# NeymarL/ChineseChess-AlphaZero

Hardware: NVIDIA B200
Metric: mcts_sims_per_sec (higher is better)
Workload: dtype f16

## Files before the change

chinesechess-alphazero_b200/csrc/cz_igemm.cuh:

```cuda
#pragma once
#include <cuda_fp16.h>
#include "cz_umma.cuh"

namespace igemm {

constexpr int kStages = 4;
constexpr int kBlockK = 64;
constexpr int kTileM = 128;
constexpr int kAStageBytes = kTileM * 128;
constexpr int kThreads = 256;

struct Args {
  int n_taps;
  int k_chunks;
  int m_tiles;
  int n_tiles;
  int box_w;
  int box_r;
  int rows;
  int n_total;
  int n_valid;
  int ldo;
  int conv;
  int relu;
  int out_f32;
  const float* bias;
  const __half* residual;
  const float* residual32;
  float* out32;
  void* out;
  uint32_t a_bytes;
  const int* n_dev;
  int rows_per_unit;
  float2* row_stats;
};

__device__ __forceinline__ int args_rows(const Args& a) { return a.n_dev ? __ldg(a.n_dev) * a.rows_per_unit : a.rows; }

template <int N_TILE>
struct Cfg {
  static constexpr int kBStageBytes = N_TILE * 128;
  static constexpr int kStageBytes = kAStageBytes + kBStageBytes;
  static constexpr int kTmemCols = (2 * N_TILE <= 32) ? 32 : (2 * N_TILE <= 64) ? 64 : (2 * N_TILE <= 128) ? 128
                                   : (2 * N_TILE <= 256) ? 256 : 512;
  static constexpr int kSmemBytes = kStages * kStageBytes + 256 + 1024;
  static_assert(2 * N_TILE <= 512, "two accumulators must fit TMEM");
  static_assert(N_TILE % 16 == 0 && N_TILE >= 16 && N_TILE <= 256, "UMMA N constraint for M=128");
};

template <int N_TILE>
__global__ void __launch_bounds__(kThreads, 1)
k_igemm(const __grid_constant__ CUtensorMap tmA, const __grid_constant__ CUtensorMap tmB, const Args a) {
  using C = Cfg<N_TILE>;
  extern __shared__ uint8_t smem_raw[];
  uint8_t* smem = reinterpret_cast<uint8_t*>((reinterpret_cast<uintptr_t>(smem_raw) + 1023) & ~(uintptr_t)1023);
  uint64_t* bars = reinterpret_cast<uint64_t*>(smem + kStages * C::kStageBytes);
  uint64_t* full = bars;
  uint64_t* empty = bars + kStages;
  uint64_t* tfull = bars + 2 * kStages;
  uint64_t* tempty = tfull + 2;
  uint32_t* tmem_slot = reinterpret_cast<uint32_t*>(tempty + 2);

  const int warp = threadIdx.x >> 5, lane = threadIdx.x & 31;

  if (warp == 0 && lane == 0) {
    umma::prefetch_tmap(&tmA);
    umma::prefetch_tmap(&tmB);
  }
  if (warp == 1 && lane == 0) {
    for (int s = 0; s < kStages; ++s) { umma::mbar_init(&full[s], 1); umma::mbar_init(&empty[s], 1); }
    for (int i = 0; i < 2; ++i) { umma::mbar_init(&tfull[i], 1); umma::mbar_init(&tempty[i], 128); }
    umma::fence_barrier_init();
    umma::fence_proxy_async();
  }
  if (warp == 2) umma::tmem_alloc<C::kTmemCols>(tmem_slot);
  umma::tc_fence_before();
  __syncthreads();
  umma::tc_fence_after();
  const uint32_t tmem_base = *tmem_slot;

  const int n_kb = a.n_taps * a.k_chunks;
  const int rows = args_rows(a);
  const int m_tiles = a.n_dev ? (rows + a.box_r * a.box_w - 1) / (a.box_r * a.box_w) : a.m_tiles;
  const int total_tiles = m_tiles * a.n_tiles;

  if (warp == 0) {
    if (lane == 0) {
      uint32_t it = 0;
      for (int tile = blockIdx.x; tile < total_tiles; tile += gridDim.x) {
        const int m_tile = tile % m_tiles, n_tile = tile / m_tiles;
        for (int tap = 0; tap < a.n_taps; ++tap) {
          const int dy = a.n_taps == 9 ? tap / 3 - 1 : 0;
          const int dx = a.n_taps == 9 ? tap % 3 - 1 : 0;
          for (int kc = 0; kc < a.k_chunks; ++kc, ++it) {
            const uint32_t s = it % kStages, ph = (it / kStages) & 1;
            umma::mbar_wait(&empty[s], ph ^ 1);
            uint8_t* sA = smem + s * C::kStageBytes;
            uint8_t* sB = sA + kAStageBytes;
            umma::mbar_expect_tx(&full[s], a.a_bytes + (uint32_t)C::kBStageBytes);
            umma::tma_load_3d(sA, &tmA, &full[s], kc * kBlockK, dx, m_tile * a.box_r + dy);
            umma::tma_load_2d(sB, &tmB, &full[s], kc * kBlockK, tap * a.n_total + n_tile * N_TILE);
          }
        }
      }
    }
  } else if (warp == 1) {
    if (lane == 0) {
      constexpr uint32_t idesc = umma::idesc_f16(kTileM, N_TILE);
      uint32_t it = 0, tcount = 0;
      for (int tile = blockIdx.x; tile < total_tiles; tile += gridDim.x, ++tcount) {
        const uint32_t acc = tcount & 1, aph = (tcount >> 1) & 1;
        umma::mbar_wait(&tempty[acc], aph ^ 1);
        umma::tc_fence_after();
        const uint32_t d_tmem = tmem_base + acc * N_TILE;
        for (int kb = 0; kb < n_kb; ++kb, ++it) {
          const uint32_t s = it % kStages, ph = (it / kStages) & 1;
          umma::mbar_wait(&full[s], ph);
          umma::tc_fence_after();
          const uint32_t sA = umma::smem_u32(smem + s * C::kStageBytes);
          const uint64_t da = umma::smem_desc_sw128(sA);
          const uint64_t db = umma::smem_desc_sw128(sA + kAStageBytes);
#pragma unroll
          for (int k = 0; k < kBlockK / 16; ++k)
            umma::mma_f16_ss(d_tmem, da + (uint64_t)(k * 2), db + (uint64_t)(k * 2), idesc, (kb | k) != 0);
          umma::mma_commit(&empty[s]);
        }
        umma::mma_commit(&tfull[acc]);
      }
    }
  } else if (warp >= 4) {
    const int q = warp - 4;
    const int m = q * 32 + lane;
    uint32_t tcount = 0;
    for (int tile = blockIdx.x; tile < total_tiles; tile += gridDim.x, ++tcount) {
      const int m_tile = tile % m_tiles, n_tile = tile / m_tiles;
      const uint32_t acc = tcount & 1, aph = (tcount >> 1) & 1;
      umma::mbar_wait(&tfull[acc], aph);
      umma::tc_fence_after();
      long long grow;
      bool valid, zero = false;
      if (a.conv) {
        const int srow = m_tile * a.box_r + m / 9;
        valid = m < a.box_r * 9 && srow < rows;
        zero = (srow % 11) == 10;
        grow = (long long)m_tile * a.box_r * 9 + m;
      } else {
        grow = (long long)m_tile * kTileM + m;
        valid = grow < rows;
      }
      const uint32_t t_row = tmem_base + ((uint32_t)(q * 32) << 16) + acc * N_TILE;
      float row_max = -INFINITY, row_sum = 0.f;
      if (a.row_stats) {
#pragma unroll 1
        for (int c0 = 0; c0 < N_TILE; c0 += 32) {
          uint32_t v[32];
          umma::tmem_ld_32x32(t_row + c0, v);
          const int n0 = n_tile * N_TILE + c0;
#pragma unroll
          for (int j = 0; j < 32; ++j)
            if (n0 + j < a.n_valid) row_max = fmaxf(row_max, __uint_as_float(v[j]) + (a.bias ? __ldg(a.bias + n0 + j) : 0.f));
        }
      }
#pragma unroll 1
      for (int c0 = 0; c0 < N_TILE; c0 += 32) {
        uint32_t v[32];
        umma::tmem_ld_32x32(t_row + c0, v);
        const int n0 = n_tile * N_TILE + c0;
        if (valid && n0 < a.n_valid) {
          float f[32];
#pragma unroll
          for (int j = 0; j < 32; ++j) f[j] = __uint_as_float(v[j]);
          if (a.bias) {
            const float4* bp4 = reinterpret_cast<const float4*>(a.bias + n0);
#pragma unroll
            for (int j = 0; j < 32; j += 4) { const float4 b4 = __ldg(bp4 + j / 4); f[j] += b4.x; f[j + 1] += b4.y; f[j + 2] += b4.z; f[j + 3] += b4.w; }
          }
          if (a.out_f32) {
            float* o = reinterpret_cast<float*>(a.out) + grow * a.ldo + n0;
            if (a.row_stats) {
#pragma unroll
              for (int j = 0; j < 32; ++j)
                if (n0 + j < a.n_valid) row_sum += __expf(f[j] - row_max);
            }
            if (n0 + 32 <= a.n_valid && (a.ldo & 3) == 0) {
#pragma unroll
              for (int j = 0; j < 32; j += 4) {
                float4 x = make_float4(f[j], f[j + 1], f[j + 2], f[j + 3]);
                if (a.relu) { x.x = fmaxf(x.x, 0.f); x.y = fmaxf(x.y, 0.f); x.z = fmaxf(x.z, 0.f); x.w = fmaxf(x.w, 0.f); }
                *reinterpret_cast<float4*>(o + j) = x;
              }
            } else if (n0 + 32 <= a.n_valid) {
#pragma unroll
              for (int j = 0; j < 32; ++j) o[j] = a.relu ? fmaxf(f[j], 0.f) : f[j];
            } else {
              for (int j = 0; j < 32 && n0 + j < a.n_valid; ++j) o[j] = a.relu ? fmaxf(f[j], 0.f) : f[j];
            }
          } else {
            __half* o = reinterpret_cast<__half*>(a.out) + grow * a.ldo + n0;
            if (a.residual) {
              const uint4* rp = reinterpret_cast<const uint4*>(a.residual + grow * a.ldo + n0);
#pragma unroll
              for (int g = 0; g < 4; ++g) {
                const uint4 rv = __ldg(rp + g);
                const __half2* h = reinterpret_cast<const __half2*>(&rv);
#pragma unroll
                for (int j = 0; j < 4; ++j) {
                  const float2 x = __half22float2(h[j]);
                  f[g * 8 + 2 * j] += x.x;
                  f[g * 8 + 2 * j + 1] += x.y;
                }
              }
            }
            uint4* op = reinterpret_cast<uint4*>(o);
#pragma unroll
            for (int g = 0; g < 4; ++g) {
              uint4 ov;
              __half2* h = reinterpret_cast<__half2*>(&ov);
#pragma unroll
              for (int j = 0; j < 4; ++j) {
                float x0 = f[g * 8 + 2 * j], x1 = f[g * 8 + 2 * j + 1];
                if (a.relu) { x0 = fmaxf(x0, 0.f); x1 = fmaxf(x1, 0.f); }
                if (zero) { x0 = 0.f; x1 = 0.f; }
                h[j] = __floats2half2_rn(x0, x1);
              }
              op[g] = ov;
            }
          }
        }
      }
      if (a.row_stats && valid) a.row_stats[grow * a.n_tiles + n_tile] = make_float2(row_max, row_sum);
      umma::tc_fence_before();
      umma::mbar_arrive(&tempty[acc]);
    }
  }

  umma::tc_fence_before();
  __syncthreads();
  if (warp == 2) {
    umma::tc_fence_after();
    umma::tmem_dealloc<C::kTmemCols>(tmem_base);
  }
}

constexpr int kStages2 = 5;
constexpr int kEpiWarps2 = 8;
constexpr int kStageRow = 36;
constexpr int kEpiStageBytes = kEpiWarps2 * 32 * kStageRow * 4;

template <int N_TILE>
struct Cfg2 {
  static constexpr int kBHalfBytes = (N_TILE / 2) * 128;
  static constexpr int kStageBytes = kAStageBytes + kBHalfBytes;
  static constexpr int kTmemCols = Cfg<N_TILE>::kTmemCols;
  static constexpr int kSmemBytes = kStages2 * kStageBytes + kEpiStageBytes + 256 + 1024;
  static_assert(N_TILE % 32 == 0 && N_TILE <= 256, "UMMA N constraint for M=256 and an even split of B");
};

constexpr int kThreads2 = 384;

template <int N_TILE>
__global__ void __cluster_dims__(2, 1, 1) __launch_bounds__(kThreads2, 1)
k_igemm2(const __grid_constant__ CUtensorMap tmA, const __grid_constant__ CUtensorMap tmB, const Args a) {
  using C = Cfg2<N_TILE>;
  extern __shared__ uint8_t smem_raw[];
  uint8_t* smem = reinterpret_cast<uint8_t*>((reinterpret_cast<uintptr_t>(smem_raw) + 1023) & ~(uintptr_t)1023);
  float* epi_stage = reinterpret_cast<float*>(smem + kStages2 * C::kStageBytes);
  uint64_t* bars = reinterpret_cast<uint64_t*>(smem + kStages2 * C::kStageBytes + kEpiStageBytes);
  uint64_t* full = bars;
  uint64_t* empty = bars + kStages2;
  uint64_t* tfull = bars + 2 * kStages2;
  uint64_t* tempty = tfull + 2;
  uint32_t* tmem_slot = reinterpret_cast<uint32_t*>(tempty + 2);

  const int warp = threadIdx.x >> 5, lane = threadIdx.x & 31;
  const uint32_t rank = umma::cluster_ctarank();
  const bool leader = rank == 0;

  if (warp == 0 && lane == 0) {
    umma::prefetch_tmap(&tmA);
    umma::prefetch_tmap(&tmB);
  }
  if (warp == 1 && lane == 0) {
    for (int s = 0; s < kStages2; ++s) { umma::mbar_init(&full[s], 1); umma::mbar_init(&empty[s], 1); }
    for (int i = 0; i < 2; ++i) { umma::mbar_init(&tfull[i], 1); umma::mbar_init(&tempty[i], 512); }
    umma::fence_barrier_init();
    umma::fence_proxy_async();
  }
  if (warp == 2) umma::tmem_alloc2<C::kTmemCols>(tmem_slot);
  umma::tc_fence_before();
  __syncthreads();
  umma::cluster_sync_all();
  umma::tc_fence_after();
  const uint32_t tmem_base = *tmem_slot;

  const int n_kb = a.n_taps * a.k_chunks;
  const int rows = args_rows(a);
  const int m_tiles = a.n_dev ? (rows + kTileM - 1) / kTileM : a.m_tiles;
  const int pairs = (m_tiles + 1) / 2;
  const int n_clusters = gridDim.x / 2, cluster_id = blockIdx.x / 2;

  if (warp == 0) {
    if (lane == 0) {
      uint32_t it = 0;
      for (int pair = cluster_id; pair < pairs; pair += n_clusters) {
        const int m_tile = 2 * pair + (int)rank;
        const int pix0 = m_tile * kTileM, img0 = pix0 / 90, row0 = (pix0 % 90) / 9, col0 = pix0 % 9;
        for (int tap = 0; tap < a.n_taps; ++tap) {
          const int dy = tap / 3 - 1, dx = tap % 3 - 1;
          for (int kc = 0; kc < a.k_chunks; ++kc, ++it) {
            const uint32_t s = it % kStages2, ph = (it / kStages2) & 1;
            umma::mbar_wait(&empty[s], ph ^ 1);
            uint8_t* sA = smem + s * C::kStageBytes;
            uint8_t* sB = sA + kAStageBytes;
            if (leader) umma::mbar_expect_tx(&full[s], 2u * (a.a_bytes + (uint32_t)C::kBHalfBytes));
            if (a.conv == 2)
              umma::tma2_load_im2col_4d(sA, &tmA, &full[s], kc * kBlockK, col0 - 1, row0 - 1, img0, (uint16_t)(dx + 1), (uint16_t)(dy + 1));
            else
              umma::tma2_load_3d(sA, &tmA, &full[s], kc * kBlockK, dx, m_tile * a.box_r + dy);
            umma::tma2_load_2d(sB, &tmB, &full[s], kc * kBlockK, tap * a.n_total + (int)rank * (N_TILE / 2));
          }
        }
      }
    }
  } else if (warp == 1) {
    if (leader && lane == 0) {
      constexpr uint32_t idesc = umma::idesc_f16(256, N_TILE);
      uint32_t it = 0, tcount = 0;
      for (int pair = cluster_id; pair < pairs; pair += n_clusters, ++tcount) {
        const uint32_t acc = tcount & 1, aph = (tcount >> 1) & 1;
        umma::mbar_wait(&tempty[acc], aph ^ 1);
        umma::tc_fence_after();
        const uint32_t d_tmem = tmem_base + acc * N_TILE;
        for (int kb = 0; kb < n_kb; ++kb, ++it) {
          const uint32_t s = it % kStages2, ph = (it / kStages2) & 1;
          umma::mbar_wait(&full[s], ph);
          umma::tc_fence_after();
          const uint32_t sA = umma::smem_u32(smem + s * C::kStageBytes);
          const uint64_t da = umma::smem_desc_sw128(sA);
          const uint64_t db = umma::smem_desc_sw128(sA + kAStageBytes);
#pragma unroll
          for (int k = 0; k < kBlockK / 16; ++k)
            umma::mma2_f16_ss(d_tmem, da + (uint64_t)(k * 2), db + (uint64_t)(k * 2), idesc, (kb | k) != 0);
          umma::mma2_commit_multicast(&empty[s]);
        }
        umma::mma2_commit_multicast(&tfull[acc]);
      }
    }
  } else if (warp >= 4) {
    const int q = warp & 3;
    const int half = (warp - 4) >> 2;
    float* S = epi_stage + (warp - 4) * 32 * kStageRow;
    const uint32_t tempty_remote[2] = {umma::mapa_shared(&tempty[0], 0), umma::mapa_shared(&tempty[1], 0)};
    constexpr int kChunks = N_TILE / 64;
    const int r4 = lane >> 3, c4 = (lane & 7) * 4;
    const int r8 = lane >> 2, c8 = (lane & 3) * 8;
    const int cbeg = half * (N_TILE / 2);
    uint32_t tcount = 0;
    auto prefetch_skip = [&](int pr) {
      if (warp != 4 || pr >= pairs || !(a.residual32 || a.residual)) return;
      const long long row0 = (long long)(2 * pr + (int)rank) * kTileM;
      const long long nrow = rows - row0 < kTileM ? rows - row0 : kTileM;
      if (nrow <= 0) return;
      const size_t esz = a.residual32 ? 4 : 2;
      const char* base = (a.residual32 ? reinterpret_cast<const char*>(a.residual32) : reinterpret_cast<const char*>(a.residual)) +
                         (size_t)row0 * a.ldo * esz;
      const size_t total = (size_t)nrow * a.ldo * esz;
      for (size_t off = (size_t)lane * 16384; off < total; off += 32 * 16384)
        umma::l2_prefetch_bulk(base + off, (uint32_t)(total - off < 16384 ? total - off : 16384));
    };
    prefetch_skip(cluster_id);
    for (int pair = cluster_id; pair < pairs; pair += n_clusters, ++tcount) {
      const int m_tile = 2 * pair + (int)rank;
      const uint32_t acc = tcount & 1, aph = (tcount >> 1) & 1;
      const long long rbase = (long long)m_tile * kTileM + q * 32;
      prefetch_skip(pair + n_clusters);
      const float* r32 = a.residual32 ? a.residual32 + rbase * a.ldo + cbeg : nullptr;
      const __half* r16 = (!a.residual32 && a.residual) ? a.residual + rbase * a.ldo + cbeg : nullptr;
      float4 nf[8];
      uint4 nh[4];
      auto fetch = [&](int ch) {
        if (r32) {
#pragma unroll
          for (int k = 0; k < 8; ++k)
            nf[k] = (rbase + r4 + 4 * k < rows) ? __ldg(reinterpret_cast<const float4*>(r32 + (size_t)(r4 + 4 * k) * a.ldo + ch * 32 + c4))
                                                  : make_float4(0.f, 0.f, 0.f, 0.f);
        } else if (r16) {
#pragma unroll
          for (int k = 0; k < 4; ++k)
            nh[k] = (rbase + r8 + 8 * k < rows) ? __ldg(reinterpret_cast<const uint4*>(r16 + (size_t)(r8 + 8 * k) * a.ldo + ch * 32 + c8))
                                                  : make_uint4(0u, 0u, 0u, 0u);
        }
      };
      fetch(0);
      umma::mbar_wait(&tfull[acc], aph);
      umma::tc_fence_after();
      const uint32_t t_row = tmem_base + ((uint32_t)(q * 32) << 16) + acc * N_TILE + cbeg;
#pragma unroll 1
      for (int ch = 0; ch < kChunks; ++ch) {
        const int c0 = cbeg + ch * 32;
        if (r32) {
#pragma unroll
          for (int k = 0; k < 8; ++k) *reinterpret_cast<float4*>(S + (r4 + 4 * k) * kStageRow + c4) = nf[k];
        } else if (r16) {
#pragma unroll
          for (int k = 0; k < 4; ++k) {
            const __half2* h = reinterpret_cast<const __half2*>(&nh[k]);
            const float2 f0 = __half22float2(h[0]), f1 = __half22float2(h[1]), f2 = __half22float2(h[2]), f3 = __half22float2(h[3]);
            float* d = S + (r8 + 8 * k) * kStageRow + c8;
            *reinterpret_cast<float4*>(d) = make_float4(f0.x, f0.y, f1.x, f1.y);
            *reinterpret_cast<float4*>(d + 4) = make_float4(f2.x, f2.y, f3.x, f3.y);
          }
        }
        if (ch + 1 < kChunks) fetch(ch + 1);
        uint32_t v[32];
        umma::tmem_ld_32x32(t_row + ch * 32, v);
        __syncwarp();
        const float4* bp = reinterpret_cast<const float4*>(a.bias + c0);
        float* own = S + lane * kStageRow;
#pragma unroll
        for (int g = 0; g < 8; ++g) {
          const float4 b = __ldg(bp + g);
          float4 x = make_float4(__uint_as_float(v[4 * g]) + b.x, __uint_as_float(v[4 * g + 1]) + b.y,
                                 __uint_as_float(v[4 * g + 2]) + b.z, __uint_as_float(v[4 * g + 3]) + b.w);
          if (r32 || r16) { const float4 rr = *reinterpret_cast<const float4*>(own + 4 * g); x.x += rr.x; x.y += rr.y; x.z += rr.z; x.w += rr.w; }
          if (a.relu) { x.x = fmaxf(x.x, 0.f); x.y = fmaxf(x.y, 0.f); x.z = fmaxf(x.z, 0.f); x.w = fmaxf(x.w, 0.f); }
          *reinterpret_cast<float4*>(own + 4 * g) = x;
        }
        __syncwarp();
        if (a.out32) {
          float* o32 = a.out32 + rbase * a.ldo + c0;
#pragma unroll
          for (int k = 0; k < 8; ++k)
            if (rbase + r4 + 4 * k < rows)
              *reinterpret_cast<float4*>(o32 + (size_t)(r4 + 4 * k) * a.ldo + c4) = *reinterpret_cast<const float4*>(S + (r4 + 4 * k) * kStageRow + c4);
        }
        {
          __half* o16 = reinterpret_cast<__half*>(a.out) + rbase * a.ldo + c0;
#pragma unroll
          for (int k = 0; k < 4; ++k) {
            const float* sp = S + (r8 + 8 * k) * kStageRow + c8;
            const float4 x0 = *reinterpret_cast<const float4*>(sp), x1 = *reinterpret_cast<const float4*>(sp + 4);
            uint4 ov;
            __half2* oh = reinterpret_cast<__half2*>(&ov);
            oh[0] = __floats2half2_rn(x0.x, x0.y); oh[1] = __floats2half2_rn(x0.z, x0.w);
            oh[2] = __floats2half2_rn(x1.x, x1.y); oh[3] = __floats2half2_rn(x1.z, x1.w);
            if (rbase + r8 + 8 * k < rows) *reinterpret_cast<uint4*>(o16 + (size_t)(r8 + 8 * k) * a.ldo + c8) = ov;
          }
        }
        __syncwarp();
      }
      umma::tc_fence_before();
      umma::mbar_arrive_cluster(tempty_remote[acc]);
    }
  }

  umma::tc_fence_before();
  __syncthreads();
  umma::cluster_sync_all();
  if (warp == 2) {
    umma::tc_fence_after();
    umma::tmem_dealloc2<C::kTmemCols>(tmem_base);
  }
}

}
```

chinesechess-alphazero_b200/csrc/cz_igemm3.cuh:

```cuda
#pragma once
#include "cz_igemm.cuh"

namespace igemm {

constexpr int kMaxStages3 = 9;
constexpr int kSmemLimit3 = 232448;
constexpr int kChunkCols3 = 16;
constexpr int kHBytes3 = 32 * kChunkCols3 * 2;
constexpr int kNH3 = 2;
constexpr int kMaxNF3 = 4;

struct Args3 {
  Args a;
  int stages;
  int skip_mode;
  int out32;
  int fbytes;
  int nf;
  int split_producer;
  int n_split;
};
__host__ __device__ constexpr int epi3_warp_bytes(int fbytes, int nf) { return nf * fbytes + kNH3 * kHBytes3; }

template <int N_TILE, int MT = 1>
struct Cfg3 {
  static constexpr int kBHalfBytes = (N_TILE / 2) * 128;
  static constexpr int kStageBytes = MT * kAStageBytes + kBHalfBytes;
  static constexpr int kTmemCols = (2 * MT * N_TILE <= 32) ? 32 : (2 * MT * N_TILE <= 64) ? 64 : (2 * MT * N_TILE <= 128) ? 128
                                   : (2 * MT * N_TILE <= 256) ? 256 : 512;
  static_assert(2 * MT * N_TILE <= 512, "accumulators (double-buffered) must fit TMEM");
  static constexpr int smem_bytes(int stages, int fbytes, int nf) { return stages * kStageBytes + kEpiWarps2 * epi3_warp_bytes(fbytes, nf) + 512 + 1024; }
  static int max_stages(int fbytes, int nf) {
    int s = (kSmemLimit3 - 512 - 1024 - kEpiWarps2 * epi3_warp_bytes(fbytes, nf)) / kStageBytes;
    return s > kMaxStages3 ? kMaxStages3 : s;
  }
  static_assert(N_TILE % 64 == 0 && N_TILE <= 256, "column halves must be multiples of 32");
};

__device__ __forceinline__ void tmem_ld_32x16(uint32_t taddr, uint32_t (&v)[16]) {
  asm volatile(
      "tcgen05.ld.sync.aligned.32x32b.x16.b32 "
      "{%0, %1, %2, %3, %4, %5, %6, %7, %8, %9, %10, %11, %12, %13, %14, %15}, [%16];"
      : "=r"(v[0]), "=r"(v[1]), "=r"(v[2]), "=r"(v[3]), "=r"(v[4]), "=r"(v[5]), "=r"(v[6]), "=r"(v[7]),
        "=r"(v[8]), "=r"(v[9]), "=r"(v[10]), "=r"(v[11]), "=r"(v[12]), "=r"(v[13]), "=r"(v[14]), "=r"(v[15])
      : "r"(taddr)
      : "memory");
  asm volatile("tcgen05.wait::ld.sync.aligned;" ::: "memory");
}

__device__ __forceinline__ void tma_store_2d(const CUtensorMap* t, const void* src, int c0, int c1) {
  asm volatile("cp.async.bulk.tensor.2d.global.shared::cta.bulk_group [%0, {%2, %3}], [%1];"
               ::"l"(reinterpret_cast<uint64_t>(t)), "r"(umma::smem_u32(src)), "r"(c0), "r"(c1) : "memory");
}
__device__ __forceinline__ void bulk_commit() { asm volatile("cp.async.bulk.commit_group;" ::: "memory"); }
template <int N>
__device__ __forceinline__ void bulk_wait_read() { asm volatile("cp.async.bulk.wait_group.read %0;" ::"n"(N) : "memory"); }
template <int N>
__device__ __forceinline__ void bulk_wait_all() { asm volatile("cp.async.bulk.wait_group %0;" ::"n"(N) : "memory"); }

template <int N_TILE, int MT = 1, int PAIRS = 1>
__global__ void __cluster_dims__(2 * PAIRS, 1, 1) __launch_bounds__(kThreads2, 1)
k_igemm3(const __grid_constant__ CUtensorMap tmA, const __grid_constant__ CUtensorMap tmB, const __grid_constant__ CUtensorMap tmOut16,
         const __grid_constant__ CUtensorMap tmSkip, const __grid_constant__ CUtensorMap tmOut32, const Args3 p) {
  using C = Cfg3<N_TILE, MT>;
  const Args& a = p.a;
  const int n_stages = p.stages;
  extern __shared__ uint8_t smem_raw[];
  uint8_t* smem = reinterpret_cast<uint8_t*>((reinterpret_cast<uintptr_t>(smem_raw) + 1023) & ~(uintptr_t)1023);
  uint8_t* epi = smem + n_stages * C::kStageBytes;
  const int warp_bytes = epi3_warp_bytes(p.fbytes, p.nf);
  uint64_t* bars = reinterpret_cast<uint64_t*>(epi + kEpiWarps2 * warp_bytes);
  uint64_t* full = bars;
  uint64_t* empty = bars + kMaxStages3;
  uint64_t* tfull = bars + 2 * kMaxStages3;
  uint64_t* tempty = tfull + 2;
  uint64_t* skipbar = tempty + 2;
  uint32_t* tmem_slot = reinterpret_cast<uint32_t*>(skipbar + kMaxNF3 * kEpiWarps2);

  const int warp = threadIdx.x >> 5, lane = threadIdx.x & 31;
  const uint32_t crank = umma::cluster_ctarank();
  const uint32_t rank = crank & 1u;
  const uint32_t pp = crank >> 1;
  const uint32_t lrank = crank & ~1u;
  const bool leader = rank == 0;

  if (warp == 0 && lane == 0) {
    umma::prefetch_tmap(&tmA);
    umma::prefetch_tmap(&tmB);
    umma::prefetch_tmap(&tmOut16);
    if (p.skip_mode) umma::prefetch_tmap(&tmSkip);
    if (p.out32) umma::prefetch_tmap(&tmOut32);
  }
  if (warp == 1 && lane == 0) {
    for (int s = 0; s < n_stages; ++s) { umma::mbar_init(&full[s], 1); umma::mbar_init(&empty[s], PAIRS); }
    for (int i = 0; i < 2; ++i) { umma::mbar_init(&tfull[i], 1); umma::mbar_init(&tempty[i], 512); }
    for (int i = 0; i < kMaxNF3 * kEpiWarps2; ++i) umma::mbar_init(&skipbar[i], 1);
    umma::fence_barrier_init();
    umma::fence_proxy_async();
  }
  if (warp == 2) umma::tmem_alloc2<C::kTmemCols>(tmem_slot);
  umma::griddep_launch_dependents();
  umma::tc_fence_before();
  __syncthreads();
  umma::cluster_sync_all();
  umma::tc_fence_after();
  const uint32_t tmem_base = *tmem_slot;
  umma::griddep_wait();

  const int n_kb = a.n_taps * a.k_chunks;
  const int rows = args_rows(a);
  const int m_tiles = a.n_dev ? (rows + kTileM - 1) / kTileM : a.m_tiles;
  const int pairs = (m_tiles + 2 * MT - 1) / (2 * MT);
  const int ns = p.n_split > 1 ? p.n_split : 1;
  const int items = pairs * ns;
  const int items_c = (items + PAIRS - 1) / PAIRS;
  const int n_clusters = gridDim.x / (2 * PAIRS), cluster_id = blockIdx.x / (2 * PAIRS);

  if (warp == 0 || (warp == 3 && p.split_producer)) {
    if (lane == 0) {
      const bool do_a = warp == 0, do_b = warp == 3 || !p.split_producer;
      uint32_t s = 0, ph = 0;
      for (int it = cluster_id; it < items_c; it += n_clusters) {
        const int item = it * PAIRS + (int)pp;
        const int pair = item / ns, n0 = (item % ns) * N_TILE;
        const int m_tile = MT * (2 * pair + (int)rank);
        for (int tap = 0; tap < a.n_taps; ++tap) {
          const int dy = tap / 3 - 1, dx = tap % 3 - 1;
          for (int kc = 0; kc < a.k_chunks; ++kc) {
            umma::mbar_wait(&empty[s], ph ^ 1);
            uint8_t* sA = smem + s * C::kStageBytes;
            uint8_t* sB = sA + MT * kAStageBytes;
            if (leader && do_a) umma::mbar_expect_tx(&full[s], 2u * ((uint32_t)MT * a.a_bytes + (uint32_t)C::kBHalfBytes));
            if (do_a) {
#pragma unroll
              for (int mt = 0; mt < MT; ++mt) {
                const int pix0 = (m_tile + mt) * kTileM, img0 = pix0 / 90, row0 = (pix0 % 90) / 9, col0 = pix0 % 9;
                umma::tma2_load_im2col_4d_r(sA + mt * kAStageBytes, &tmA, &full[s], kc * kBlockK, col0 - 1, row0 - 1, img0, (uint16_t)(dx + 1), (uint16_t)(dy + 1), lrank);
              }
            }
            if (do_b) {
              if (PAIRS == 1) umma::tma2_load_2d(sB, &tmB, &full[s], kc * kBlockK, tap * a.n_total + n0 + (int)rank * (N_TILE / 2));
              else if (pp == 0)
                umma::tma2_load_2d_mc(sB, &tmB, &full[s], kc * kBlockK, tap * a.n_total + n0 + (int)rank * (N_TILE / 2),
                                      (uint16_t)((1u << rank) | (1u << (rank + 2))));
            }
            if (++s == (uint32_t)n_stages) { s = 0; ph ^= 1; }
          }
        }
      }
    }
  } else if (warp == 1) {
    if (leader && lane == 0) {
      constexpr uint32_t idesc = umma::idesc_f16(256, N_TILE);
      uint32_t s = 0, ph = 0, tcount = 0;
      for (int it = cluster_id; it < items_c; it += n_clusters, ++tcount) {
        const uint32_t acc = tcount & 1, aph = (tcount >> 1) & 1;
        umma::mbar_wait(&tempty[acc], aph ^ 1);
        umma::tc_fence_after();
        const uint32_t d_tmem = tmem_base + acc * (MT * N_TILE);
        for (int kb = 0; kb < n_kb; ++kb) {
          umma::mbar_wait(&full[s], ph);
          umma::tc_fence_after();
          const uint32_t sA = umma::smem_u32(smem + s * C::kStageBytes);
          const uint64_t db = umma::smem_desc_sw128(sA + MT * kAStageBytes);
#pragma unroll
          for (int mt = 0; mt < MT; ++mt) {
            const uint64_t da = umma::smem_desc_sw128(sA + mt * kAStageBytes);
#pragma unroll
            for (int k = 0; k < kBlockK / 16; ++k)
              umma::mma2_f16_ss(d_tmem + mt * N_TILE, da + (uint64_t)(k * 2), db + (uint64_t)(k * 2), idesc, (kb | k) != 0);
          }
          umma::mma2_commit_mask(&empty[s], PAIRS == 1 ? (uint16_t)3 : (uint16_t)0xF);
          if (++s == (uint32_t)n_stages) { s = 0; ph ^= 1; }
        }
        umma::mma2_commit_mask(&tfull[acc], (uint16_t)(3u << (2 * pp)));
      }
    }
  } else if (warp >= 4) {
    const int ew = warp - 4;
    const int q = warp & 3;
    const int half = ew >> 2;
    constexpr int kChunks = (N_TILE / 2) / kChunkCols3;
    const int cbeg = half * (N_TILE / 2);
    const int fb = p.fbytes, nf = p.nf;
    uint8_t* F = epi + ew * warp_bytes;
    uint8_t* H = F + nf * fb;
    uint64_t* sbar = skipbar + kMaxNF3 * ew;
    const uint32_t tempty_remote[2] = {umma::mapa_shared(&tempty[0], lrank), umma::mapa_shared(&tempty[1], lrank)};
    const int r3 = (lane >> 1) & 3;
    const int r1 = (lane >> 2) & 1;
    const bool has_skip = p.skip_mode != 0, skip32 = p.skip_mode == 2;
    const uint32_t skip_bytes = skip32 ? 2048u : 1024u;
    auto prefetch_skip = [&](int item) {
      if (ew != 0 || item >= items || !has_skip || ns > 1) return;
      const int pr = item;
      const long long row0 = (long long)MT * (2 * pr + (int)rank) * kTileM;
      const long long nrow = rows - row0 < MT * kTileM ? rows - row0 : MT * kTileM;
      if (nrow <= 0) return;
      const size_t esz = skip32 ? 4 : 2;
      const char* base = (skip32 ? reinterpret_cast<const char*>(a.residual32) : reinterpret_cast<const char*>(a.residual)) + (size_t)row0 * a.ldo * esz;
      const size_t total = (size_t)nrow * a.ldo * esz;
      for (size_t off = (size_t)lane * 16384; off < total; off += 32 * 16384)
        umma::l2_prefetch_bulk(base + off, (uint32_t)(total - off < 16384 ? total - off : 16384));
    };
    int my_tiles = 0;
    for (int it = cluster_id; it < items_c; it += n_clusters) ++my_tiles;
    const uint32_t total_chunks = (uint32_t)my_tiles * (MT * kChunks);
    auto request_skip = [&](uint32_t g) {
      if (!has_skip || g >= total_chunks) return;
      const int t = (int)(g / (MT * kChunks)), rem = (int)(g % (MT * kChunks)), mt = rem / kChunks, ch = rem % kChunks;
      const int item = (cluster_id + t * n_clusters) * PAIRS + (int)pp;
      const int row = (MT * (2 * (item / ns) + (int)rank) + mt) * kTileM + q * 32;
      const uint32_t slot = g % (uint32_t)nf;
      umma::mbar_expect_tx(&sbar[slot], skip_bytes);
      umma::tma_load_2d(F + slot * fb, &tmSkip, &sbar[slot], (item % ns) * N_TILE + cbeg + ch * kChunkCols3, row);
    };
    uint32_t tcount = 0, g = 0;
    prefetch_skip(cluster_id * PAIRS + (int)pp);
    if (lane == 0)
      for (int k = 0; k < nf - 2; ++k) request_skip((uint32_t)k);
    for (int it = cluster_id; it < items_c; it += n_clusters, ++tcount) {
      const uint32_t acc = tcount & 1, aph = (tcount >> 1) & 1;
      const int item = it * PAIRS + (int)pp;
      const int pair = item / ns, n0 = (item % ns) * N_TILE;
      prefetch_skip(item + n_clusters * PAIRS);
      umma::mbar_wait(&tfull[acc], aph);
      umma::tc_fence_after();
#pragma unroll 1
      for (int mt = 0; mt < MT; ++mt) {
      const int m_tile = MT * (2 * pair + (int)rank) + mt;
      const int rbase = m_tile * kTileM + q * 32;
      const uint32_t t_row = tmem_base + ((uint32_t)(q * 32) << 16) + (acc * MT + mt) * N_TILE + cbeg;
#pragma unroll 1
      for (int ch = 0; ch < kChunks; ++ch, ++g) {
        const uint32_t slot = g % (uint32_t)nf, sph = (g / (uint32_t)nf) & 1, hb = g & 1;
        const int c0 = n0 + cbeg + ch * kChunkCols3;
        if (lane == 0) {
          bulk_wait_read<1>();
          request_skip(g + (uint32_t)nf - 2);
        }
        uint32_t v[16];
        tmem_ld_32x16(t_row + ch * kChunkCols3, v);
        __syncwarp();
        if (has_skip) umma::mbar_wait(&sbar[slot], sph);
        uint8_t* frow = F + slot * fb + lane * 64;
        uint8_t* hrow = H + hb * kHBytes3 + lane * 32;
        const float4* bp = reinterpret_cast<const float4*>(a.bias + c0);
#pragma unroll
        for (int gq = 0; gq < 4; gq += 2) {
          float4 x0, x1;
          {
            const float4 b0 = __ldg(bp + gq), b1 = __ldg(bp + gq + 1);
            x0 = make_float4(__uint_as_float(v[4 * gq]) + b0.x, __uint_as_float(v[4 * gq + 1]) + b0.y,
                             __uint_as_float(v[4 * gq + 2]) + b0.z, __uint_as_float(v[4 * gq + 3]) + b0.w);
            x1 = make_float4(__uint_as_float(v[4 * gq + 4]) + b1.x, __uint_as_float(v[4 * gq + 5]) + b1.y,
                             __uint_as_float(v[4 * gq + 6]) + b1.z, __uint_as_float(v[4 * gq + 7]) + b1.w);
          }
          if (skip32) {
            const float4 s0 = *reinterpret_cast<const float4*>(frow + ((gq ^ r3) << 4));
            const float4 s1 = *reinterpret_cast<const float4*>(frow + (((gq + 1) ^ r3) << 4));
            x0.x += s0.x; x0.y += s0.y; x0.z += s0.z; x0.w += s0.w;
            x1.x += s1.x; x1.y += s1.y; x1.z += s1.z; x1.w += s1.w;
          } else if (has_skip) {
            const uint4 sv = *reinterpret_cast<const uint4*>(F + slot * fb + lane * 32 + (((gq >> 1) ^ r1) << 4));
            const __half2* h = reinterpret_cast<const __half2*>(&sv);
            const float2 f0 = __half22float2(h[0]), f1 = __half22float2(h[1]), f2 = __half22float2(h[2]), f3 = __half22float2(h[3]);
            x0.x += f0.x; x0.y += f0.y; x0.z += f1.x; x0.w += f1.y;
            x1.x += f2.x; x1.y += f2.y; x1.z += f3.x; x1.w += f3.y;
          }
          if (a.relu) {
            x0.x = fmaxf(x0.x, 0.f); x0.y = fmaxf(x0.y, 0.f); x0.z = fmaxf(x0.z, 0.f); x0.w = fmaxf(x0.w, 0.f);
            x1.x = fmaxf(x1.x, 0.f); x1.y = fmaxf(x1.y, 0.f); x1.z = fmaxf(x1.z, 0.f); x1.w = fmaxf(x1.w, 0.f);
          }
          if (p.out32) {
            *reinterpret_cast<float4*>(frow + ((gq ^ r3) << 4)) = x0;
            *reinterpret_cast<float4*>(frow + (((gq + 1) ^ r3) << 4)) = x1;
          }
          uint4 ov;
          __half2* oh = reinterpret_cast<__half2*>(&ov);
          oh[0] = __floats2half2_rn(x0.x, x0.y); oh[1] = __floats2half2_rn(x0.z, x0.w);
          oh[2] = __floats2half2_rn(x1.x, x1.y); oh[3] = __floats2half2_rn(x1.z, x1.w);
          *reinterpret_cast<uint4*>(hrow + (((gq >> 1) ^ r1) << 4)) = ov;
        }
        umma::fence_proxy_async();
        __syncwarp();
        if (lane == 0) {
          if (p.out32) tma_store_2d(&tmOut32, F + slot * fb, c0, rbase);
          tma_store_2d(&tmOut16, H + hb * kHBytes3, c0, rbase);
          bulk_commit();
        }
      }
      }
      umma::tc_fence_before();
      umma::mbar_arrive_cluster(tempty_remote[acc]);
    }
    if (lane == 0) bulk_wait_all<0>();
  }

  umma::tc_fence_before();
  __syncthreads();
  umma::cluster_sync_all();
  if (warp == 2) {
    umma::tc_fence_after();
    umma::tmem_dealloc2<C::kTmemCols>(tmem_base);
  }
}

}
```

chinesechess-alphazero_b200/csrc/cz_nn.cu:

```cuda
#include <cuda.h>
#include <cuda_fp16.h>
#include <cuda_runtime.h>
#include <math.h>
#include <stdio.h>
#include <stdlib.h>
#include <string.h>
#include <string>
#include <vector>

#include "cz_err.h"
#include "cz_igemm.cuh"
#include "cz_igemm3.cuh"
#include "cz_nn.cuh"

namespace cznn {

#define CZ_CUDA(x)                                                                           \
  do {                                                                                       \
    cudaError_t e__ = (x);                                                                   \
    if (e__ != cudaSuccess) return cz_fail(CZ_ERR_CUDA, "%s: %s", #x, cudaGetErrorString(e__)); \
  } while (0)

constexpr int kLabels = CZ_N_LABELS;
constexpr int kPolN = 2304;
constexpr float kBnEps = 1e-3f;

typedef CUresult (*EncodeTiledFn)(CUtensorMap*, CUtensorMapDataType, cuuint32_t, void*, const cuuint64_t*,
                                  const cuuint64_t*, const cuuint32_t*, const cuuint32_t*, CUtensorMapInterleave,
                                  CUtensorMapSwizzle, CUtensorMapL2promotion, CUtensorMapFloatOOBfill);
typedef CUresult (*EncodeIm2colFn)(CUtensorMap*, CUtensorMapDataType, cuuint32_t, void*, const cuuint64_t*, const cuuint64_t*,
                                   const int*, const int*, cuuint32_t, cuuint32_t, const cuuint32_t*, CUtensorMapInterleave,
                                   CUtensorMapSwizzle, CUtensorMapL2promotion, CUtensorMapFloatOOBfill);
static EncodeTiledFn g_encode = nullptr;
static EncodeIm2colFn g_encode_im2col = nullptr;

static int load_encode() {
  if (g_encode) return 0;
  void* fn = nullptr;
  cudaDriverEntryPointQueryResult qres;
  cudaError_t e = cudaGetDriverEntryPoint("cuTensorMapEncodeTiled", &fn, cudaEnableDefault, &qres);
  if (e != cudaSuccess || !fn) return cz_fail(CZ_ERR_CUDA, "cuTensorMapEncodeTiled not available: %s", cudaGetErrorString(e));
  g_encode = (EncodeTiledFn)fn;
  fn = nullptr;
  e = cudaGetDriverEntryPoint("cuTensorMapEncodeIm2col", &fn, cudaEnableDefault, &qres);
  if (e == cudaSuccess && fn) g_encode_im2col = (EncodeIm2colFn)fn;
  return 0;
}

static int make_map_im2col(CUtensorMap* m, const void* base, int c, long long n_images) {
  if (load_encode()) return CZ_ERR_CUDA;
  if (!g_encode_im2col) return cz_fail(CZ_ERR_UNSUPPORTED, "cuTensorMapEncodeIm2col not available");
  cuuint64_t dims[4] = {(cuuint64_t)c, 9, 10, (cuuint64_t)n_images};
  cuuint64_t strides[3] = {(cuuint64_t)c * 2, (cuuint64_t)c * 2 * 9, (cuuint64_t)c * 2 * 90};
  int lower[2] = {-1, -1}, upper[2] = {-1, -1};
  cuuint32_t es[4] = {1, 1, 1, 1};
  CUresult r = g_encode_im2col(m, CU_TENSOR_MAP_DATA_TYPE_FLOAT16, 4, const_cast<void*>(base), dims, strides, lower, upper, 64, 128,
                               es, CU_TENSOR_MAP_INTERLEAVE_NONE, CU_TENSOR_MAP_SWIZZLE_128B, CU_TENSOR_MAP_L2_PROMOTION_L2_256B,
                               CU_TENSOR_MAP_FLOAT_OOB_FILL_NONE);
  if (r != CUDA_SUCCESS) return cz_fail(CZ_ERR_CUDA, "cuTensorMapEncodeIm2col failed: %d", (int)r);
  return 0;
}

static int make_map_3d(CUtensorMap* m, const void* base, int c, int w, long long rows, int box_w, int box_r) {
  if (load_encode()) return CZ_ERR_CUDA;
  cuuint64_t dims[3] = {(cuuint64_t)c, (cuuint64_t)w, (cuuint64_t)rows};
  cuuint64_t strides[2] = {(cuuint64_t)c * 2, (cuuint64_t)c * 2 * w};
  cuuint32_t box[3] = {64, (cuuint32_t)box_w, (cuuint32_t)box_r};
  cuuint32_t es[3] = {1, 1, 1};
  CUresult r = g_encode(m, CU_TENSOR_MAP_DATA_TYPE_FLOAT16, 3, const_cast<void*>(base), dims, strides, box, es,
                        CU_TENSOR_MAP_INTERLEAVE_NONE, CU_TENSOR_MAP_SWIZZLE_128B, CU_TENSOR_MAP_L2_PROMOTION_L2_256B,
                        CU_TENSOR_MAP_FLOAT_OOB_FILL_NONE);
  if (r != CUDA_SUCCESS) return cz_fail(CZ_ERR_CUDA, "cuTensorMapEncodeTiled(3d) failed: %d", (int)r);
  return 0;
}
static int make_map_2d(CUtensorMap* m, const void* base, int k, long long rows, int box_rows) {
  if (load_encode()) return CZ_ERR_CUDA;
  cuuint64_t dims[2] = {(cuuint64_t)k, (cuuint64_t)rows};
  cuuint64_t strides[1] = {(cuuint64_t)k * 2};
  cuuint32_t box[2] = {64, (cuuint32_t)box_rows};
  cuuint32_t es[2] = {1, 1};
  CUresult r = g_encode(m, CU_TENSOR_MAP_DATA_TYPE_FLOAT16, 2, const_cast<void*>(base), dims, strides, box, es,
                        CU_TENSOR_MAP_INTERLEAVE_NONE, CU_TENSOR_MAP_SWIZZLE_128B, CU_TENSOR_MAP_L2_PROMOTION_L2_256B,
                        CU_TENSOR_MAP_FLOAT_OOB_FILL_NONE);
  if (r != CUDA_SUCCESS) return cz_fail(CZ_ERR_CUDA, "cuTensorMapEncodeTiled(2d) failed: %d", (int)r);
  return 0;
}

static int make_map_tile32(CUtensorMap* m, const void* base, int c, long long rows, bool f32) {
  if (load_encode()) return CZ_ERR_CUDA;
  const cuuint64_t es = f32 ? 4 : 2;
  cuuint64_t dims[2] = {(cuuint64_t)c, (cuuint64_t)rows};
  cuuint64_t strides[1] = {(cuuint64_t)c * es};
  cuuint32_t box[2] = {igemm::kChunkCols3, 32};
  cuuint32_t est[2] = {1, 1};
  CUresult r = g_encode(m, f32 ? CU_TENSOR_MAP_DATA_TYPE_FLOAT32 : CU_TENSOR_MAP_DATA_TYPE_FLOAT16, 2, const_cast<void*>(base), dims, strides,
                        box, est, CU_TENSOR_MAP_INTERLEAVE_NONE, f32 ? CU_TENSOR_MAP_SWIZZLE_64B : CU_TENSOR_MAP_SWIZZLE_32B,
                        CU_TENSOR_MAP_L2_PROMOTION_L2_256B, CU_TENSOR_MAP_FLOAT_OOB_FILL_NONE);
  if (r != CUDA_SUCCESS) return cz_fail(CZ_ERR_CUDA, "cuTensorMapEncodeTiled(tile32) failed: %d", (int)r);
  return 0;
}

static int g_num_sms = 0;
static int num_sms() {
  if (!g_num_sms) {
    int dev = 0;
    cudaGetDevice(&dev);
    cudaDeviceGetAttribute(&g_num_sms, cudaDevAttrMultiProcessorCount, dev);
    if (g_num_sms <= 0) g_num_sms = 148;
  }
  return g_num_sms;
}

template <int N_TILE>
static int launch_igemm_t(const CUtensorMap& tmA, const CUtensorMap& tmB, const igemm::Args& a, cudaStream_t st) {
  using C = igemm::Cfg<N_TILE>;
  static bool attr_set = false;
  if (!attr_set) {
    CZ_CUDA(cudaFuncSetAttribute(igemm::k_igemm<N_TILE>, cudaFuncAttributeMaxDynamicSharedMemorySize, C::kSmemBytes));
    attr_set = true;
  }
  const int tiles = a.m_tiles * a.n_tiles;
  if (tiles <= 0) return 0;
  const int grid = tiles < num_sms() ? tiles : num_sms();
  igemm::k_igemm<N_TILE><<<grid, igemm::kThreads, C::kSmemBytes, st>>>(tmA, tmB, a);
  CZ_CUDA(cudaGetLastError());
  return 0;
}

template <int N_TILE>
static int launch_igemm2_t(const CUtensorMap& tmA, const CUtensorMap& tmB_half, const igemm::Args& a, cudaStream_t st) {
  using C = igemm::Cfg2<N_TILE>;
  static bool attr_set = false;
  if (!attr_set) {
    CZ_CUDA(cudaFuncSetAttribute(igemm::k_igemm2<N_TILE>, cudaFuncAttributeMaxDynamicSharedMemorySize, C::kSmemBytes));
    attr_set = true;
  }
  const int pairs = (a.m_tiles + 1) / 2;
  if (pairs <= 0) return 0;
  const int clusters = pairs < num_sms() / 2 ? pairs : num_sms() / 2;
  igemm::k_igemm2<N_TILE><<<2 * clusters, igemm::kThreads2, C::kSmemBytes, st>>>(tmA, tmB_half, a);
  CZ_CUDA(cudaGetLastError());
  return 0;
}
static int launch_igemm2(int n_tile, const CUtensorMap& tmA, const CUtensorMap& tmB_half, const igemm::Args& a, cudaStream_t st) {
  switch (n_tile) {
    case 64: return launch_igemm2_t<64>(tmA, tmB_half, a, st);
    case 128: return launch_igemm2_t<128>(tmA, tmB_half, a, st);
    case 192: return launch_igemm2_t<192>(tmA, tmB_half, a, st);
    case 256: return launch_igemm2_t<256>(tmA, tmB_half, a, st);
  }
  return cz_fail(CZ_ERR_UNSUPPORTED, "igemm2: unsupported N tile %d", n_tile);
}
static int epilogue_choice() {
  static int v = -1;
  if (v < 0) { const char* e = getenv("CZ_EPI"); v = (e && e[0] == '2') ? 2 : (e && e[0] == '3') ? 3 : 0; }
  return v;
}
static bool use_tma_epilogue() { return epilogue_choice() != 2; }
static bool use_tma_epilogue_for(int c, bool fp32_stream) {
  if (epilogue_choice() == 2) return false;
  if (epilogue_choice() == 3) return true;
  return !(c == 256 && fp32_stream);
}
static int g_cluster4 = 0;
template <int N_TILE, int MT, int PAIRS = 1>
static int launch_igemm3_t(const CUtensorMap& tmA, const CUtensorMap& tmB_half, const CUtensorMap& tmOut16, const CUtensorMap& tmSkip,
                           const CUtensorMap& tmOut32, const igemm::Args& a, int skip_mode, bool out32, cudaStream_t st, int n_split = 1) {
  using C = igemm::Cfg3<N_TILE, MT>;
  static bool attr_set = false;
  static int max_clusters = 0;
  if (!attr_set) {
    CZ_CUDA(cudaFuncSetAttribute(igemm::k_igemm3<N_TILE, MT, PAIRS>, cudaFuncAttributeMaxDynamicSharedMemorySize, igemm::kSmemLimit3));
    attr_set = true;
    max_clusters = num_sms() / (2 * PAIRS);
    if (PAIRS > 1) {
      cudaLaunchConfig_t oc;
      memset(&oc, 0, sizeof(oc));
      oc.gridDim = dim3(2 * PAIRS * max_clusters); oc.blockDim = dim3(igemm::kThreads2); oc.dynamicSmemBytes = igemm::kSmemLimit3;
      int nc = 0;
      if (cudaOccupancyMaxActiveClusters(&nc, igemm::k_igemm3<N_TILE, MT, PAIRS>, &oc) == cudaSuccess && nc > 0 && nc < max_clusters) max_clusters = nc;
      else (void)cudaGetLastError();
      fprintf(stderr, "[cczero] 4-CTA clusters of k_igemm3<%d, %d>: %d resident at once (%d of %d SMs)\n", N_TILE, MT, max_clusters,
              4 * max_clusters, num_sms());
    }
  }
  igemm::Args3 p;
  p.a = a;
  p.skip_mode = skip_mode; p.out32 = out32 ? 1 : 0; p.n_split = n_split;
  p.fbytes = (skip_mode == 2 || out32) ? 2048 : (skip_mode == 1 ? 1024 : 0);
  { static int nf = -1; if (nf < 0) { const char* e = getenv("CZ_NF"); nf = e ? atoi(e) : 3; if (nf < 3) nf = 3; if (nf > igemm::kMaxNF3) nf = igemm::kMaxNF3; } p.nf = nf; }
  { static int sp = -1; if (sp < 0) { const char* e = getenv("CZ_SPLIT_PROD"); sp = (e && e[0] == '1') ? 1 : 0; } p.split_producer = sp; }
  p.stages = C::max_stages(p.fbytes, p.nf);
  { static int cap = -1; if (cap < 0) { const char* e = getenv("CZ_STAGES"); cap = e ? atoi(e) : 0; } if (cap > 1 && cap < p.stages) p.stages = cap; }
  if (p.stages < 2) return cz_fail(CZ_ERR_UNSUPPORTED, "igemm3: no room for the operand ring");
  const int pairs = ((a.n_dev ? (a.rows + igemm::kTileM - 1) / igemm::kTileM : a.m_tiles) + 2 * MT - 1) / (2 * MT);
  if (pairs <= 0) return 0;
  const int items = (pairs * (n_split > 1 ? n_split : 1) + PAIRS - 1) / PAIRS;
  const int clusters = items < max_clusters ? items : max_clusters;
  static int pdl = -1;
  if (pdl < 0) { const char* e = getenv("CZ_PDL"); pdl = (e && e[0] == '0') ? 0 : 1; }
  if (pdl) {
    cudaLaunchConfig_t lc;
    memset(&lc, 0, sizeof(lc));
    lc.gridDim = dim3(2 * PAIRS * clusters); lc.blockDim = dim3(igemm::kThreads2);
    lc.dynamicSmemBytes = C::smem_bytes(p.stages, p.fbytes, p.nf); lc.stream = st;
    cudaLaunchAttribute at[1];
    at[0].id = cudaLaunchAttributeProgrammaticStreamSerialization;
    at[0].val.programmaticStreamSerializationAllowed = 1;
    lc.attrs = at; lc.numAttrs = 1;
    CZ_CUDA(cudaLaunchKernelEx(&lc, igemm::k_igemm3<N_TILE, MT, PAIRS>, tmA, tmB_half, tmOut16, tmSkip, tmOut32, p));
  } else {
    igemm::k_igemm3<N_TILE, MT, PAIRS><<<2 * PAIRS * clusters, igemm::kThreads2, C::smem_bytes(p.stages, p.fbytes, p.nf), st>>>(tmA, tmB_half, tmOut16, tmSkip, tmOut32, p);
  }
  CZ_CUDA(cudaGetLastError());
  return 0;
}
static int launch_igemm3(int n_tile, const CUtensorMap& tmA, const CUtensorMap& tmB_half, const CUtensorMap& tmOut16, const CUtensorMap& tmSkip,
                         const CUtensorMap& tmOut32, const igemm::Args& a, int skip_mode, bool out32, cudaStream_t st) {
  static int mt2 = -1;
  if (mt2 < 0) { const char* e = getenv("CZ_MT"); mt2 = (e && e[0] == '1') ? 0 : 1; }
  switch (n_tile) {
    case 64: return mt2 ? launch_igemm3_t<64, 2>(tmA, tmB_half, tmOut16, tmSkip, tmOut32, a, skip_mode, out32, st)
                        : launch_igemm3_t<64, 1>(tmA, tmB_half, tmOut16, tmSkip, tmOut32, a, skip_mode, out32, st);
    case 128: return mt2 ? launch_igemm3_t<128, 2>(tmA, tmB_half, tmOut16, tmSkip, tmOut32, a, skip_mode, out32, st)
                         : launch_igemm3_t<128, 1>(tmA, tmB_half, tmOut16, tmSkip, tmOut32, a, skip_mode, out32, st);
    case 192: return launch_igemm3_t<192, 1>(tmA, tmB_half, tmOut16, tmSkip, tmOut32, a, skip_mode, out32, st);
    case 256: {
      if (g_cluster4) return launch_igemm3_t<256, 1, 2>(tmA, tmB_half, tmOut16, tmSkip, tmOut32, a, skip_mode, out32, st);
      return launch_igemm3_t<256, 1>(tmA, tmB_half, tmOut16, tmSkip, tmOut32, a, skip_mode, out32, st);
    }
  }
  return cz_fail(CZ_ERR_UNSUPPORTED, "igemm3: unsupported N tile %d", n_tile);
}
static bool use_n_split(int n_boards, int c) {
  static int on = -1;
  if (on < 0) { const char* e = getenv("CZ_NSPLIT"); on = (e && e[0] == '0') ? 0 : 1; }
  if (!on || c <= 64) return false;
  const int pairs = ((n_boards * 90 + igemm::kTileM - 1) / igemm::kTileM + 1) / 2;
  return pairs * (c / 64) <= num_sms() / 2;
}
static int launch_igemm3_split(int c, const CUtensorMap& tmA, const CUtensorMap& tmB_32, const CUtensorMap& tmOut16, const CUtensorMap& tmSkip,
                               const CUtensorMap& tmOut32, const igemm::Args& a, int skip_mode, bool out32, cudaStream_t st) {
  return launch_igemm3_t<64, 1>(tmA, tmB_32, tmOut16, tmSkip, tmOut32, a, skip_mode, out32, st, c / 64);
}
static bool use_im2col() {
  static int v = -1;
  if (v < 0) { const char* e = getenv("CZ_CONV_STRIP"); v = (e && e[0] == '1') ? 0 : 1; }
  return v == 1;
}
static bool use_pair_kernel() {
  static int v = -1;
  if (v < 0) { const char* e = getenv("CZ_IGEMM_1CTA"); v = (e && e[0] == '1') ? 0 : 1; }
  return v == 1;
}

static int launch_igemm(int n_tile, const CUtensorMap& tmA, const CUtensorMap& tmB, const igemm::Args& a, cudaStream_t st) {
  switch (n_tile) {
    case 64: return launch_igemm_t<64>(tmA, tmB, a, st);
    case 128: return launch_igemm_t<128>(tmA, tmB, a, st);
    case 192: return launch_igemm_t<192>(tmA, tmB, a, st);
    case 256: return launch_igemm_t<256>(tmA, tmB, a, st);
  }
  return cz_fail(CZ_ERR_UNSUPPORTED, "igemm: unsupported N tile %d (filters must be 64/128/192/256)", n_tile);
}

static igemm::Args conv_args(int n_boards, int c, const float* bias, const __half* residual, __half* out, int relu) {
  igemm::Args a;
  memset(&a, 0, sizeof(a));
  a.n_taps = 9; a.k_chunks = c / 64; a.box_w = 9; a.box_r = 14;
  a.rows = n_boards * 11; a.m_tiles = (a.rows + 13) / 14; a.n_tiles = 1;
  a.n_total = c; a.n_valid = c; a.ldo = c; a.conv = 1; a.relu = relu; a.out_f32 = 0;
  a.bias = bias; a.residual = residual; a.out = out; a.a_bytes = 64 * 9 * 14 * 2;
  return a;
}

static igemm::Args conv_args_dense(int n_boards, int c, const float* bias, const __half* residual, __half* out, int relu) {
  igemm::Args a = conv_args(n_boards, c, bias, residual, out, relu);
  a.conv = 2; a.rows = n_boards * 90; a.m_tiles = (a.rows + 127) / 128; a.a_bytes = 128 * 128;
  return a;
}

static igemm::Args dense_args(int m, int n_valid, int n_pad, int k_pad, int n_tile, const float* bias, float* out, int ldo) {
  igemm::Args a;
  memset(&a, 0, sizeof(a));
  a.n_taps = 1; a.k_chunks = k_pad / 64; a.box_w = 1; a.box_r = 128;
  a.rows = m; a.m_tiles = (m + 127) / 128; a.n_tiles = n_pad / n_tile;
  a.n_total = n_pad; a.n_valid = n_valid; a.ldo = ldo; a.conv = 0; a.relu = 0; a.out_f32 = 1;
  a.bias = bias; a.residual = nullptr; a.out = out; a.a_bytes = 64 * 128 * 2;
  return a;
}

__device__ __forceinline__ int plane_of(uint8_t c) { return c == 0 ? -1 : ((c & 8) ? c - 2 : c - 1); }

__global__ void k_conv_first(const uint8_t* __restrict__ boards, const __half* __restrict__ w,
                             const float* __restrict__ shift, __half* __restrict__ out, float* __restrict__ out32, int c_out,
                             int board_pixels, int in_planes, int board_stride, const int* __restrict__ n_dev) {
  if ((int)blockIdx.x >= __ldg(n_dev)) return;
  __shared__ int8_t pl[2][90];
  __shared__ uint16_t rows[90][52];
  __shared__ uint8_t cnt[90];
  const int b = blockIdx.x, t = threadIdx.x;
  const int n_boards = in_planes / 14;
  if (t < 90) {
    const int r = t / 9, col = t % 9;
    for (int h = 0; h < n_boards; ++h)
      pl[h][t] = (int8_t)plane_of(boards[(size_t)b * board_stride + h * CZ_BOARD_STRIDE + (9 - r) * 9 + col]);
  }
  __syncthreads();
  const int per = (90 + (int)gridDim.y - 1) / (int)gridDim.y, p0 = (int)blockIdx.y * per, p1 = p0 + per < 90 ? p0 + per : 90;
  if (t < p1 - p0) {
    const int r = (p0 + t) / 9, col = (p0 + t) % 9;
    int n = 0;
    for (int kh = 0; kh < 5; ++kh) {
      const int rr = r + kh - 2;
      if (rr < 0 || rr > 9) continue;
      for (int kw = 0; kw < 5; ++kw) {
        const int cc = col + kw - 2;
        if (cc < 0 || cc > 8) continue;
        for (int h = 0; h < n_boards; ++h) {
          const int p = pl[h][rr * 9 + cc];
          if (p >= 0) rows[t][n++] = (uint16_t)((kh * 5 + kw) * in_planes + h * 14 + p);
        }
      }
    }
    cnt[t] = (uint8_t)n;
  }
  __syncthreads();
  const int pairs = c_out / 2;
  const int c = 2 * (t % pairs), grp = t / pairs, n_groups = blockDim.x / pairs;
  if (grp >= n_groups) return;
  const float2 sh = *reinterpret_cast<const float2*>(shift + c);
  __half* o = out + (size_t)b * board_pixels * c_out;
  const __half2* w2 = reinterpret_cast<const __half2*>(w + c);
  const int stride2 = c_out / 2;
  for (int pix = p0 + grp; pix < p1; pix += n_groups) {
    float a0 = sh.x, a1 = sh.y;
    const int n = cnt[pix - p0];
    for (int k = 0; k < n; ++k) {
      const float2 v = __half22float2(__ldg(w2 + (size_t)rows[pix - p0][k] * stride2));
      a0 += v.x; a1 += v.y;
    }
    a0 = fmaxf(a0, 0.f); a1 = fmaxf(a1, 0.f);
    *reinterpret_cast<__half2*>(o + (size_t)pix * c_out + c) = __floats2half2_rn(a0, a1);
    if (out32) *reinterpret_cast<float2*>(out32 + ((size_t)b * board_pixels + pix) * c_out + c) = make_float2(a0, a1);
  }
  if (blockIdx.y == 0)
  for (int col = 90 + grp; col < board_pixels; col += n_groups)
    *reinterpret_cast<__half2*>(o + (size_t)col * c_out + c) = __floats2half2_rn(0.f, 0.f);
}

__global__ void k_planes_to_boards(const float* __restrict__ planes, uint8_t* __restrict__ boards, int n, int in_planes) {
  const int b = blockIdx.x;
  if (b >= n) return;
  const int t = threadIdx.x;
  if (t < 96) {
    for (int h = 0; h < in_planes / 14; ++h) {
      uint8_t code = 0;
      if (t < 90) {
        const int y = t / 9, x = t % 9, r = 9 - y;
        for (int p = 0; p < 14; ++p)
          if (planes[((size_t)b * in_planes + h * 14 + p) * 90 + r * 9 + x] > 0.5f) code = (uint8_t)(p < 7 ? p + 1 : p + 2);
      }
      boards[((size_t)b * (in_planes / 14) + h) * CZ_BOARD_STRIDE + t] = code;
    }
  }
}

constexpr int kHeadPos = 4;
constexpr int kMaxHeadOut = 36;
static size_t heads_smem_bytes(int c_in, int n_out) { return ((size_t)kHeadPos * n_out * 90 + (size_t)(c_in / 8) * n_out * 8 + kHeadPos * 8) * sizeof(float); }
__global__ void __launch_bounds__(256) k_heads(const __half* __restrict__ act, const float* __restrict__ act32, int c_in,
                                                const int* __restrict__ n_dev, int board_pixels, int pol_c, int val_c, int pol_k1,
                                                const float* __restrict__ wh,
                                                const float* __restrict__ shifth,
                                                const float* __restrict__ wv1,
                                                const float* __restrict__ bv1,
                                                const float* __restrict__ wv2,
                                                const float* __restrict__ bv2,
                                                int hidden, __half* __restrict__ pol_feat, float* __restrict__ value,
                                                int hp) {
  extern __shared__ __align__(16) float hsm[];
  const int n_out = pol_c + val_c;
  float* feat = hsm;
  float* wsm = feat + kHeadPos * n_out * 90;
  float* red = wsm + (c_in / 8) * n_out * 8;
  const int tid = threadIdx.x, warp = tid >> 5, lane = tid & 31;
  const int b0 = blockIdx.x * hp;
  const int n_pos = __ldg(n_dev);
  if (b0 >= n_pos) return;
  const int npos = n_pos - b0 < hp ? n_pos - b0 : hp;
  for (int i = tid; i < n_out * c_in; i += 256) { const int o = i / c_in, c = i % c_in; wsm[((c >> 3) * n_out + o) * 8 + (c & 7)] = __ldg(wh + i); }
  __syncthreads();
  for (int item = tid; item < npos * 90; item += 256) {
    const int p = item / 90, pix = item % 90;
    const size_t row = ((size_t)(b0 + p) * board_pixels + pix) * c_in;
    for (int o0 = 0; o0 < n_out; o0 += 6) {
      float s[6] = {0.f, 0.f, 0.f, 0.f, 0.f, 0.f};
#pragma unroll 4
      for (int g = 0; g < c_in / 8; ++g) {
        float x[8];
        if (act32) {
          const float4* a4 = reinterpret_cast<const float4*>(act32 + row + g * 8);
          const float4 u = __ldg(a4), w4 = __ldg(a4 + 1);
          x[0] = u.x; x[1] = u.y; x[2] = u.z; x[3] = u.w; x[4] = w4.x; x[5] = w4.y; x[6] = w4.z; x[7] = w4.w;
        } else {
          const uint4 v = __ldg(reinterpret_cast<const uint4*>(act + row + g * 8));
          const __half2* h = reinterpret_cast<const __half2*>(&v);
#pragma unroll
          for (int j = 0; j < 4; ++j) { const float2 f = __half22float2(h[j]); x[2 * j] = f.x; x[2 * j + 1] = f.y; }
        }
#pragma unroll
        for (int o = 0; o < 6; ++o) {
          if (o0 + o < n_out) {
            const float* wp = wsm + (g * n_out + o0 + o) * 8;
            const float4 wa = *reinterpret_cast<const float4*>(wp), wb = *reinterpret_cast<const float4*>(wp + 4);
            s[o] += x[0] * wa.x + x[1] * wa.y + x[2] * wa.z + x[3] * wa.w + x[4] * wb.x + x[5] * wb.y + x[6] * wb.z + x[7] * wb.w;
          }
        }
      }
#pragma unroll
      for (int o = 0; o < 6; ++o)
        if (o0 + o < n_out) feat[(p * n_out + o0 + o) * 90 + pix] = fmaxf(s[o] + __ldg(shifth + o0 + o), 0.f);
    }
  }
  __syncthreads();
  const int pol_in = pol_c * 90, pol_k = 3 * pol_k1;
  for (int i = tid; i < npos * pol_k1; i += 256) {
    const int p = i / pol_k1, k = i % pol_k1;
    const float f = k < pol_in ? feat[(p * n_out + k / 90) * 90 + k % 90] : 0.f;
    const __half hi = __float2half_rn(f);
    const __half lo = __float2half_rn(f - __half2float(hi));
    __half* row = pol_feat + (size_t)(b0 + p) * pol_k;
    row[k] = hi; row[pol_k1 + k] = lo; row[2 * pol_k1 + k] = hi;
  }
  float h[kHeadPos];
#pragma unroll
  for (int p = 0; p < kHeadPos; ++p) h[p] = 0.f;
  if (tid < hidden) {
    float acc[kHeadPos];
    const float bb = bv1[tid];
#pragma unroll
    for (int p = 0; p < kHeadPos; ++p) acc[p] = bb;
#pragma unroll 10
    for (int i = 0; i < val_c * 90; ++i) {
      const float wv = __ldg(wv1 + (size_t)i * hidden + tid);
#pragma unroll
      for (int p = 0; p < kHeadPos; ++p) acc[p] += feat[(p * n_out + pol_c + i / 90) * 90 + i % 90] * wv;
    }
    const float w2 = wv2[tid];
#pragma unroll
    for (int p = 0; p < kHeadPos; ++p) h[p] = fmaxf(acc[p], 0.f) * w2;
  }
#pragma unroll
  for (int p = 0; p < kHeadPos; ++p) {
    float v = h[p];
    for (int m = 16; m; m >>= 1) v += __shfl_xor_sync(0xffffffffu, v, m);
    if (lane == 0) red[p * 8 + warp] = v;
  }
  __syncthreads();
  if (tid < npos) {
    float sum = bv2[0];
    for (int i = 0; i < 8; ++i) sum += red[tid * 8 + i];
    value[b0 + tid] = tanhf(sum);
  }
}

struct RowStat { float mx, inv; };
__device__ __forceinline__ RowStat combine_stats(const float2* __restrict__ st, int n_tiles) {
  float mx = -INFINITY;
  for (int t = 0; t < n_tiles; ++t) mx = fmaxf(mx, __ldg(&st[t].x));
  float s = 0.f;
  for (int t = 0; t < n_tiles; ++t) { const float2 v = __ldg(st + t); s = __fmaf_rn(v.y, expf(v.x - mx), s); }
  RowStat r; r.mx = mx; r.inv = __frcp_rn(s);
  return r;
}
__device__ __forceinline__ float policy_prob(float logit, const RowStat& r) { return __fmul_rn(expf(logit - r.mx), r.inv); }

__global__ void __launch_bounds__(256) k_softmax(const float* __restrict__ logits, int ldl, const float2* __restrict__ stats, int n_tiles,
                                                  float* __restrict__ policy) {
  const int b = blockIdx.x;
  const RowStat rs = combine_stats(stats + (size_t)b * n_tiles, n_tiles);
  const float* l = logits + (size_t)b * ldl;
  for (int i = threadIdx.x; i < kLabels; i += 256) policy[(size_t)b * kLabels + i] = policy_prob(l[i], rs);
}

__global__ void __launch_bounds__(128) k_legal_priors(const float* __restrict__ logits, int ldl, const float2* __restrict__ stats, int n_tiles,
                                                       const int16_t* __restrict__ labels, const int32_t* __restrict__ counts,
                                                       const int* __restrict__ n_dev, float* __restrict__ out) {
  const int leaf = blockIdx.x * 4 + (threadIdx.x >> 5), lane = threadIdx.x & 31;
  if (leaf >= __ldg(n_dev)) return;
  const RowStat rs = combine_stats(stats + (size_t)leaf * n_tiles, n_tiles);
  const float* l = logits + (size_t)leaf * ldl;
  const int L = counts[leaf];
  for (int i = lane; i < L; i += 32) {
    const int lab = labels[(size_t)leaf * CZ_MAX_MOVES + i];
    out[(size_t)leaf * CZ_MAX_MOVES + i] = lab >= 0 ? policy_prob(l[lab], rs) : 0.f;
  }
}
__global__ void k_set_int(int* p, int v) { *p = v; }

__global__ void k_bn_fold(const float* gamma, const float* beta, const float* mean, const float* var, float* scale,
                          float* shift, int c) {
  const int i = blockIdx.x * blockDim.x + threadIdx.x;
  if (i < c) {
    const float s = gamma[i] / sqrtf(var[i] + kBnEps);
    scale[i] = s;
    shift[i] = beta[i] - mean[i] * s;
  }
}
__global__ void k_prep_hwio(const float* w, const float* scale, __half* out, long long n, int co) {
  const long long i = (long long)blockIdx.x * blockDim.x + threadIdx.x;
  if (i < n) out[i] = __float2half_rn(w[i] * scale[i % co]);
}
__global__ void k_prep_conv3(const float* w, const float* scale, __half* out, int c) {
  const long long i = (long long)blockIdx.x * blockDim.x + threadIdx.x;
  const long long n = 9LL * c * c;
  if (i < n) {
    const int ci = (int)(i % c), co = (int)((i / c) % c), tap = (int)(i / ((long long)c * c));
    out[i] = __float2half_rn(w[((long long)tap * c + ci) * c + co] * scale[co]);
  }
}
__global__ void k_prep_1x1(const float* w, const float* scale, float* out, int ci_n, int co_n) {
  const int i = blockIdx.x * blockDim.x + threadIdx.x;
  if (i < ci_n * co_n) {
    const int ci = i % ci_n, co = i / ci_n;
    out[(size_t)co * ci_n + ci] = w[(size_t)ci * co_n + co] * scale[co];
  }
}
__global__ void k_prep_policy(const float* w, __half* out, int pol_in, int pol_k1) {
  const long long i = (long long)blockIdx.x * blockDim.x + threadIdx.x;
  if (i < (long long)kPolN * pol_k1) {
    const int k = (int)(i % pol_k1), n = (int)(i / pol_k1);
    const float f = (k < pol_in && n < kLabels) ? w[(size_t)k * kLabels + n] : 0.f;
    const __half hi = __float2half_rn(f);
    const __half lo = __float2half_rn(f - __half2float(hi));
    __half* row = out + (size_t)n * 3 * pol_k1;
    row[k] = hi; row[pol_k1 + k] = hi; row[2 * pol_k1 + k] = lo;
  }
}
__global__ void k_copy_pad(const float* src, float* dst, int n_src, int n_dst) {
  const int i = blockIdx.x * blockDim.x + threadIdx.x;
  if (i < n_dst) dst[i] = i < n_src ? src[i] : 0.f;
}

struct Carver {
  uint8_t* base; size_t off, cap;
  void* take(size_t bytes) {
    off = (off + 1023) & ~(size_t)1023;
    void* p = base ? base + off : nullptr;
    off += bytes;
    return p;
  }
};

struct NetWeights {
  __half* w_first; float* shift_first;
  __half* w_conv;  float* shift_conv;
  float *wh, *shifth, *wv1, *bv1, *wv2, *bv2;
  __half* w_pol; float* b_pol;
  CUtensorMap map_wpol;
  std::vector<CUtensorMap> map_w, map_w_half, map_w_32;
  bool ready;
};

struct NnRuntime {
  int filters, blocks, value_fc, max_batch;
  int pol_c, val_c, pol_k1;
  NetWeights nets[2]; int n_nets, cur;
  cudaStream_t stream;
  bool ready;
  uint64_t launches;
  __half *x, *t, *y, *pol_feat;
  float *x32, *y32;
  float* logits;
  float2* stats;
  int* n_scalar;
  bool heads_attr;
  bool capturing;
  size_t prof_open;
  uint8_t* boards_tmp;
  int in_planes;
  __half* w_first; float* shift_first;
  __half* w_conv;  float* shift_conv;
  float *wh, *shifth, *wv1, *bv1, *wv2, *bv2;
  __half* w_pol; float* b_pol;
  float* scratch;
  CUtensorMap map_x, map_t, map_y, map_pf, map_wpol;
  std::vector<CUtensorMap> map_w;
  std::vector<CUtensorMap> map_w_half;
  std::vector<CUtensorMap> map_w_32;
  bool fp32_skip;
  int board_pixels;
  CUtensorMap imap_x, imap_t, imap_y;
  CUtensorMap omap_x, omap_t, omap_y;
  CUtensorMap fmap_x32, fmap_y32;
  bool profile;
  std::vector<cudaEvent_t> ev;
  size_t ev_used;
  std::vector<double> ev_flops;
  double prof_ms, prof_flops; uint64_t prof_launches;
};

static void store_net(NnRuntime* r, int k) {
  NetWeights& n = r->nets[k];
  n.w_first = r->w_first; n.shift_first = r->shift_first; n.w_conv = r->w_conv; n.shift_conv = r->shift_conv;
  n.wh = r->wh; n.shifth = r->shifth; n.wv1 = r->wv1; n.bv1 = r->bv1; n.wv2 = r->wv2; n.bv2 = r->bv2;
  n.w_pol = r->w_pol; n.b_pol = r->b_pol; n.map_wpol = r->map_wpol; n.map_w = r->map_w; n.map_w_half = r->map_w_half; n.map_w_32 = r->map_w_32;
  n.ready = r->ready;
}
static void select_net(NnRuntime* r, int k) {
  if (r->cur == k) return;
  store_net(r, r->cur);
  const NetWeights& n = r->nets[k];
  r->w_first = n.w_first; r->shift_first = n.shift_first; r->w_conv = n.w_conv; r->shift_conv = n.shift_conv;
  r->wh = n.wh; r->shifth = n.shifth; r->wv1 = n.wv1; r->bv1 = n.bv1; r->wv2 = n.wv2; r->bv2 = n.bv2;
  r->w_pol = n.w_pol; r->b_pol = n.b_pol; r->map_wpol = n.map_wpol; r->map_w = n.map_w; r->map_w_half = n.map_w_half; r->map_w_32 = n.map_w_32;
  r->ready = n.ready;
  r->cur = k;
}

static void prof_collect(NnRuntime* r) {
  for (size_t i = 0; i + 1 < r->ev_used; i += 2) {
    float ms = 0.f;
    if (cudaEventElapsedTime(&ms, r->ev[i], r->ev[i + 1]) == cudaSuccess) {
      r->prof_ms += ms; r->prof_flops += r->ev_flops[i / 2]; r->prof_launches += (uint64_t)(2 * r->blocks);
    }
  }
  r->ev_used = 0;
}

static void layout(NnRuntime* r, Carver& cv) {
  const int c = r->filters;
  const size_t act = (size_t)r->max_batch * 11 * 9 * c * sizeof(__half);
  r->x = (__half*)cv.take(act);
  r->t = (__half*)cv.take(act);
  r->y = (__half*)cv.take(act);
  r->x32 = (float*)cv.take(act * 2);
  r->y32 = (float*)cv.take(act * 2);
  r->pol_feat = (__half*)cv.take(((size_t)r->max_batch + 128) * 3 * r->pol_k1 * sizeof(__half));
  r->logits = (float*)cv.take((size_t)r->max_batch * kPolN * sizeof(float));
  r->stats = (float2*)cv.take((size_t)r->max_batch * (kPolN / 256) * sizeof(float2));
  r->n_scalar = (int*)cv.take(64);
  r->boards_tmp = (uint8_t*)cv.take((size_t)r->max_batch * 2 * CZ_BOARD_STRIDE);
  for (int net = 0; net < r->n_nets; ++net) {
  r->w_first = (__half*)cv.take((size_t)25 * 28 * c * sizeof(__half));
  r->shift_first = (float*)cv.take(c * sizeof(float));
  r->w_conv = (__half*)cv.take((size_t)2 * r->blocks * 9 * c * c * sizeof(__half));
  r->shift_conv = (float*)cv.take((size_t)2 * r->blocks * c * sizeof(float));
  r->wh = (float*)cv.take((size_t)(r->pol_c + r->val_c) * c * sizeof(float));
  r->shifth = (float*)cv.take((size_t)(r->pol_c + r->val_c + 4) * sizeof(float));
  r->wv1 = (float*)cv.take((size_t)r->val_c * 90 * r->value_fc * sizeof(float));
  r->bv1 = (float*)cv.take(r->value_fc * sizeof(float));
  r->wv2 = (float*)cv.take(r->value_fc * sizeof(float));
  r->bv2 = (float*)cv.take(4 * sizeof(float));
  r->w_pol = (__half*)cv.take((size_t)kPolN * 3 * r->pol_k1 * sizeof(__half));
  r->b_pol = (float*)cv.take(kPolN * sizeof(float));
  r->ready = false;
  r->cur = net;
  store_net(r, net);
  }
  if (r->n_nets > 1) { r->cur = r->n_nets - 1; select_net(r, 0); }
  r->cur = 0;
  r->scratch = (float*)cv.take((size_t)(2 * 256 + 2 * kMaxHeadOut) * sizeof(float));
}

static void set_heads(NnRuntime* r, int pol_c, int val_c) {
  r->pol_c = pol_c > 0 ? pol_c : 4; r->val_c = val_c > 0 ? val_c : 2;
  r->pol_k1 = (r->pol_c * 90 + 63) / 64 * 64;
}
size_t nn_workspace_bytes(int filters, int blocks, int value_fc, int max_batch, int n_nets, int pol_c, int val_c) {
  NnRuntime tmp;
  tmp.filters = filters; tmp.blocks = blocks; tmp.value_fc = value_fc; tmp.max_batch = max_batch; tmp.n_nets = n_nets; tmp.cur = 0;
  set_heads(&tmp, pol_c, val_c);
  Carver cv{nullptr, 0, 0};
  layout(&tmp, cv);
  return cv.off + 4096;
}

NnRuntime* nn_create(int device, int filters, int blocks, int value_fc, int max_batch, void* workspace, size_t bytes,
                     void* stream, int fp32_skip_mode, int n_nets, int in_planes, int pol_c, int val_c) {
  (void)device;
  if (filters % 64 != 0 || filters < 64 || filters > 256) { cz_fail(CZ_ERR_UNSUPPORTED, "nn: filters must be 64..256 step 64"); return nullptr; }
  if (value_fc > 256 || value_fc < 1) { cz_fail(CZ_ERR_UNSUPPORTED, "nn: value_fc_size must be <= 256"); return nullptr; }
  if (n_nets < 1 || n_nets > 2) { cz_fail(CZ_ERR_ARG, "nn: 1 or 2 networks"); return nullptr; }
  if (pol_c < 0 || val_c < 0 || pol_c > 32 || val_c > 4 || (pol_c > 0 ? pol_c : 4) + (val_c > 0 ? val_c : 2) > kMaxHeadOut) {
    cz_fail(CZ_ERR_UNSUPPORTED, "nn: head widths up to 32 policy / 4 value channels"); return nullptr;
  }
  if (bytes < nn_workspace_bytes(filters, blocks, value_fc, max_batch, n_nets, pol_c, val_c)) { cz_fail(CZ_ERR_ARG, "nn: workspace too small"); return nullptr; }
  NnRuntime* r = new NnRuntime();
  set_heads(r, pol_c, val_c);
  r->heads_attr = false;
  r->filters = filters; r->blocks = blocks; r->value_fc = value_fc; r->max_batch = max_batch; r->n_nets = n_nets; r->cur = 0;
  r->stream = (cudaStream_t)stream; r->ready = false; r->launches = 0;
  r->in_planes = in_planes == 28 ? 28 : 14;
  r->fp32_skip = fp32_skip_mode == 1 || (fp32_skip_mode == 0 && blocks >= 10);
  { const char* e = getenv("CZ_FP32_SKIP"); if (e && e[0] == '1') r->fp32_skip = true; if (e && e[0] == '0') r->fp32_skip = false; }
  { const char* e = getenv("CZ_CLUSTER4"); g_cluster4 = (e && e[0] == '1') ? 1 : 0; }
  r->profile = false; r->ev_used = 0; r->prof_ms = 0; r->prof_flops = 0; r->prof_launches = 0; r->capturing = false;
  Carver cv{(uint8_t*)workspace, 0, bytes};
  layout(r, cv);
  const int c = filters;
  const long long rows = (long long)max_batch * 11;
  int rc = 0;
  r->board_pixels = (use_im2col() && use_pair_kernel()) ? 90 : 99;
  if (r->board_pixels == 90) {
    rc |= make_map_im2col(&r->imap_x, r->x, c, max_batch);
    rc |= make_map_im2col(&r->imap_t, r->t, c, max_batch);
    rc |= make_map_im2col(&r->imap_y, r->y, c, max_batch);
    rc |= make_map_tile32(&r->omap_x, r->x, c, (long long)max_batch * 90, false);
    rc |= make_map_tile32(&r->omap_t, r->t, c, (long long)max_batch * 90, false);
    rc |= make_map_tile32(&r->omap_y, r->y, c, (long long)max_batch * 90, false);
    rc |= make_map_tile32(&r->fmap_x32, r->x32, c, (long long)max_batch * 90, true);
    rc |= make_map_tile32(&r->fmap_y32, r->y32, c, (long long)max_batch * 90, true);
  }
  rc |= make_map_3d(&r->map_x, r->x, c, 9, rows, 9, 14);
  rc |= make_map_3d(&r->map_t, r->t, c, 9, rows, 9, 14);
  rc |= make_map_3d(&r->map_y, r->y, c, 9, rows, 9, 14);
  rc |= make_map_3d(&r->map_pf, r->pol_feat, 3 * r->pol_k1, 1, (long long)max_batch + 128, 1, 128);
  for (int net = n_nets - 1; net >= 0; --net) {
    select_net(r, net);
    rc |= make_map_2d(&r->map_wpol, r->w_pol, 3 * r->pol_k1, kPolN, 256);
    r->map_w.resize(2 * blocks);
    r->map_w_half.resize(2 * blocks);
    r->map_w_32.resize(2 * blocks);
    for (int i = 0; i < 2 * blocks; ++i) {
      rc |= make_map_2d(&r->map_w[i], r->w_conv + (size_t)i * 9 * c * c, c, 9LL * c, c);
      rc |= make_map_2d(&r->map_w_half[i], r->w_conv + (size_t)i * 9 * c * c, c, 9LL * c, c / 2);
      rc |= make_map_2d(&r->map_w_32[i], r->w_conv + (size_t)i * 9 * c * c, c, 9LL * c, 32);
    }
    store_net(r, net);
  }
  if (rc) { delete r; return nullptr; }
  cudaMemsetAsync(r->x, 0, (size_t)max_batch * 11 * 9 * c * 2, r->stream);
  cudaMemsetAsync(r->t, 0, (size_t)max_batch * 11 * 9 * c * 2, r->stream);
  cudaMemsetAsync(r->y, 0, (size_t)max_batch * 11 * 9 * c * 2, r->stream);
  cudaMemsetAsync(r->pol_feat, 0, ((size_t)max_batch + 128) * 3 * r->pol_k1 * 2, r->stream);
  return r;
}

void nn_destroy(NnRuntime* r) {
  if (!r) return;
  for (cudaEvent_t e : r->ev) cudaEventDestroy(e);
  delete r;
}
void nn_profile(NnRuntime* r, bool on) { if (r) { r->profile = on; } }
int nn_profile_read(NnRuntime* r, double* ms, uint64_t* launches, double* flops) {
  if (!r) return cz_fail(CZ_ERR_STATE, "no network");
  CZ_CUDA(cudaStreamSynchronize(r->stream));
  prof_collect(r);
  if (ms) *ms = r->prof_ms;
  if (launches) *launches = r->prof_launches;
  if (flops) *flops = r->prof_flops;
  r->prof_ms = 0; r->prof_flops = 0; r->prof_launches = 0;
  return 0;
}
bool nn_ready(const NnRuntime* r) {
  if (!r) return false;
  for (int k = 0; k < r->n_nets; ++k)
    if (!(k == r->cur ? r->ready : r->nets[k].ready)) return false;
  return true;
}
uint64_t nn_launches(const NnRuntime* r) { return r ? r->launches : 0; }

struct WeightSet {
  const cz_tensor_desc* d; int n;
  const cz_tensor_desc* find(const std::string& layer, const std::string& weight) const {
    for (int i = 0; i < n; ++i) {
      std::string nm = d[i].name ? d[i].name : "";
      const size_t slash = nm.find('/');
      if (slash == std::string::npos) continue;
      std::string l = nm.substr(0, slash), w = nm.substr(slash + 1);
      const size_t colon = w.find(':');
      if (colon != std::string::npos) w = w.substr(0, colon);
      const size_t s2 = w.find('/');
      if (s2 != std::string::npos) w = w.substr(s2 + 1);
      if (w != weight) continue;
      if (l == layer || (l.size() > layer.size() && l.compare(0, layer.size(), layer) == 0 && l[layer.size()] == '-')) return &d[i];
    }
    return nullptr;
  }
};

#define NEED(var, layer, weight, count)                                                                      \
  const cz_tensor_desc* var = ws.find(layer, weight);                                                        \
  if (!var || var->numel != (long long)(count))                                                              \
    return cz_fail(CZ_ERR_ARG, "cz_nn_set_weights: missing or mis-sized tensor %s/%s (want %lld)", std::string(layer).c_str(), weight, (long long)(count));

static int fold_bn(NnRuntime* r, const WeightSet& ws, const std::string& layer, int c, float* scale, float* shift) {
  NEED(g, layer, "gamma", c);
  NEED(b, layer, "beta", c);
  NEED(m, layer, "moving_mean", c);
  NEED(v, layer, "moving_variance", c);
  k_bn_fold<<<(c + 127) / 128, 128, 0, r->stream>>>((const float*)g->dev, (const float*)b->dev, (const float*)m->dev,
                                                     (const float*)v->dev, scale, shift, c);
  r->launches++;
  return 0;
}

int nn_set_weights(NnRuntime* r, int net, const cz_tensor_desc* descs, int n) {
  if (!r) return cz_fail(CZ_ERR_STATE, "cz_nn_set_weights: engine was created without a network (nn_filters = 0)");
  if (net < 0 || net >= r->n_nets) return cz_fail(CZ_ERR_ARG, "cz_nn_set_weights: network %d of %d", net, r->n_nets);
  select_net(r, net);
  WeightSet ws{descs, n};
  const int c = r->filters;
  cudaStream_t st = r->stream;
  float* scale = r->scratch;
  {
    NEED(k, "input_conv", "kernel", 25LL * r->in_planes * c);
    if (fold_bn(r, ws, "input_batchnorm", c, scale, r->shift_first)) return CZ_ERR_ARG;
    const long long nn = 25LL * r->in_planes * c;
    k_prep_hwio<<<(unsigned)((nn + 255) / 256), 256, 0, st>>>((const float*)k->dev, scale, r->w_first, nn, c);
  }
  for (int i = 0; i < r->blocks; ++i) {
    for (int j = 0; j < 2; ++j) {
      const std::string conv = "res" + std::to_string(i + 1) + "_conv" + std::to_string(j + 1);
      const std::string bn = "res" + std::to_string(i + 1) + "_batchnorm" + std::to_string(j + 1);
      NEED(k, conv, "kernel", 9LL * c * c);
      const int li = 2 * i + j;
      if (fold_bn(r, ws, bn, c, scale, r->shift_conv + (size_t)li * c)) return CZ_ERR_ARG;
      const long long nn = 9LL * c * c;
      k_prep_conv3<<<(unsigned)((nn + 255) / 256), 256, 0, st>>>((const float*)k->dev, scale, r->w_conv + (size_t)li * nn, c);
    }
  }
  {
    const int pc = r->pol_c, vc = r->val_c;
    NEED(kp, "policy_conv", "kernel", (long long)pc * c);
    if (fold_bn(r, ws, "policy_batchnorm", pc, scale, r->shifth)) return CZ_ERR_ARG;
    k_prep_1x1<<<(pc * c + 255) / 256, 256, 0, st>>>((const float*)kp->dev, scale, r->wh, c, pc);
    NEED(kv, "value_conv", "kernel", (long long)vc * c);
    float* scale_v = r->scratch + 2 * 256 + kMaxHeadOut;
    if (fold_bn(r, ws, "value_batchnorm", vc, scale_v, r->shifth + pc)) return CZ_ERR_ARG;
    k_prep_1x1<<<(vc * c + 255) / 256, 256, 0, st>>>((const float*)kv->dev, scale_v, r->wh + (size_t)pc * c, c, vc);
  }
  {
    NEED(k, "policy_out", "kernel", (long long)r->pol_c * 90 * kLabels);
    NEED(b, "policy_out", "bias", kLabels);
    const long long nn = (long long)kPolN * r->pol_k1;
    k_prep_policy<<<(unsigned)((nn + 255) / 256), 256, 0, st>>>((const float*)k->dev, r->w_pol, r->pol_c * 90, r->pol_k1);
    k_copy_pad<<<(kPolN + 255) / 256, 256, 0, st>>>((const float*)b->dev, r->b_pol, kLabels, kPolN);
  }
  {
    const int h = r->value_fc;
    NEED(k1, "value_dense", "kernel", (long long)r->val_c * 90 * h);
    NEED(b1, "value_dense", "bias", h);
    NEED(k2, "value_out", "kernel", h);
    NEED(b2, "value_out", "bias", 1);
    CZ_CUDA(cudaMemcpyAsync(r->wv1, k1->dev, (size_t)r->val_c * 90 * h * 4, cudaMemcpyDeviceToDevice, st));
    CZ_CUDA(cudaMemcpyAsync(r->bv1, b1->dev, (size_t)h * 4, cudaMemcpyDeviceToDevice, st));
    CZ_CUDA(cudaMemcpyAsync(r->wv2, k2->dev, (size_t)h * 4, cudaMemcpyDeviceToDevice, st));
    CZ_CUDA(cudaMemcpyAsync(r->bv2, b2->dev, 4, cudaMemcpyDeviceToDevice, st));
  }
  r->launches += 6 + 2 * r->blocks;
  CZ_CUDA(cudaGetLastError());
  CZ_CUDA(cudaStreamSynchronize(st));
  r->ready = true;
  return 0;
}

static int conv_first_threads(int c) {
  const int pairs = c / 2;
  int g = 256 / pairs;
  if (g < 1) g = 1;
  while (pairs * g < 96) ++g;
  return pairs * g;
}
static int fw_first(NnRuntime* r, const uint8_t* boards, int n, const int* n_dev) {
  const int c = r->filters;
  const bool s32 = r->board_pixels == 90 && r->fp32_skip;
  int slices = (2 * num_sms() + n - 1) / n;
  if (slices > 15) slices = 15;
  k_conv_first<<<dim3(n, slices), conv_first_threads(c), 0, r->stream>>>(boards, r->w_first, r->shift_first, r->x, s32 ? r->x32 : nullptr, c, r->board_pixels,
                                                            r->in_planes, (r->in_planes / 14) * CZ_BOARD_STRIDE, n_dev);
  r->launches++;
  CZ_CUDA(cudaGetLastError());
  return 0;
}
static int fw_tower(NnRuntime* r, int n, const int* n_dev) {
  const int c = r->filters;
  cudaStream_t st = r->stream;
  const bool dense = r->board_pixels == 90;
  const bool s32 = dense && r->fp32_skip;
  float *x32 = s32 ? r->x32 : nullptr, *y32 = s32 ? r->y32 : nullptr;
  CUtensorMap *ix = &r->imap_x, *iy = &r->imap_y;
  CUtensorMap *ox = &r->omap_x, *oy = &r->omap_y;
  CUtensorMap *fx = &r->fmap_x32, *fy = &r->fmap_y32;
  __half *x = r->x, *y = r->y;
  CUtensorMap *mx = &r->map_x, *my = &r->map_y;
  const bool epi3 = dense && use_tma_epilogue();
  for (int i = 0; i < r->blocks; ++i) {
    const size_t wsz = (size_t)c;
    igemm::Args a1 = conv_args(n, c, r->shift_conv + (size_t)(2 * i) * wsz, nullptr, r->t, 1);
    igemm::Args a2 = conv_args(n, c, r->shift_conv + (size_t)(2 * i + 1) * wsz, x, y, 1);
    if (dense) {
      igemm::Args d1 = conv_args_dense(n, c, a1.bias, nullptr, r->t, 1);
      igemm::Args d2 = conv_args_dense(n, c, a2.bias, x, y, 1);
      d1.n_dev = n_dev; d1.rows_per_unit = 90; d2.n_dev = n_dev; d2.rows_per_unit = 90;
      d2.residual32 = x32; d2.out32 = y32;
      { float* t32 = x32; x32 = y32; y32 = t32; }
      if (epi3 && use_n_split(n, c)) {
        if (launch_igemm3_split(c, *ix, r->map_w_32[2 * i], r->omap_t, r->omap_t, r->omap_t, d1, 0, false, st)) return CZ_ERR_CUDA;
        if (launch_igemm3_split(c, r->imap_t, r->map_w_32[2 * i + 1], *oy, s32 ? *fx : *ox, *fy, d2, s32 ? 2 : 1, s32, st)) return CZ_ERR_CUDA;
      } else {
      if (epi3 && use_tma_epilogue_for(c, false)) {
        if (launch_igemm3(c, *ix, r->map_w_half[2 * i], r->omap_t, r->omap_t, r->omap_t, d1, 0, false, st)) return CZ_ERR_CUDA;
      } else if (launch_igemm2(c, *ix, r->map_w_half[2 * i], d1, st)) return CZ_ERR_CUDA;
      if (epi3 && use_tma_epilogue_for(c, s32)) {
        if (launch_igemm3(c, r->imap_t, r->map_w_half[2 * i + 1], *oy, s32 ? *fx : *ox, *fy, d2, s32 ? 2 : 1, s32, st)) return CZ_ERR_CUDA;
      } else if (launch_igemm2(c, r->imap_t, r->map_w_half[2 * i + 1], d2, st)) return CZ_ERR_CUDA;
      }
      CUtensorMap* ti = ix; ix = iy; iy = ti;
      ti = ox; ox = oy; oy = ti;
      ti = fx; fx = fy; fy = ti;
    } else {
      if (launch_igemm(c, *mx, r->map_w[2 * i], a1, st)) return CZ_ERR_CUDA;
      if (launch_igemm(c, r->map_t, r->map_w[2 * i + 1], a2, st)) return CZ_ERR_CUDA;
    }
    r->launches += 2;
    __half* tx = x; x = y; y = tx;
    CUtensorMap* tm = mx; mx = my; my = tm;
  }
  return 0;
}
static int fw_heads(NnRuntime* r, int n, const int* n_dev, float* value) {
  const int c = r->filters;
  const bool s32 = r->board_pixels == 90 && r->fp32_skip;
  const bool odd = (r->blocks & 1) != 0;
  const __half* x = odd ? r->y : r->x;
  const float* x32 = s32 ? (odd ? r->y32 : r->x32) : nullptr;
  const size_t hsm = heads_smem_bytes(c, r->pol_c + r->val_c);
  if (hsm > 48 * 1024 && !r->heads_attr) {
    CZ_CUDA(cudaFuncSetAttribute(k_heads, cudaFuncAttributeMaxDynamicSharedMemorySize, (int)hsm));
    r->heads_attr = true;
  }
  const int hp = n <= 2 * num_sms() ? 1 : kHeadPos;
  k_heads<<<(n + hp - 1) / hp, 256, hsm, r->stream>>>(x, x32, c, n_dev, r->board_pixels, r->pol_c, r->val_c, r->pol_k1, r->wh, r->shifth,
                                                      r->wv1, r->bv1, r->wv2, r->bv2, r->value_fc, r->pol_feat, value, hp);
  igemm::Args ap = dense_args(n, kLabels, kPolN, 3 * r->pol_k1, 256, r->b_pol, r->logits, kPolN);
  ap.n_dev = n_dev; ap.rows_per_unit = 1; ap.row_stats = r->stats;
  if (launch_igemm(256, r->map_pf, r->map_wpol, ap, r->stream)) return CZ_ERR_CUDA;
  r->launches += 2;
  CZ_CUDA(cudaGetLastError());
  return 0;
}
void nn_prof_begin(NnRuntime* r, double flops) {
  r->prof_open = (size_t)-1;
  if (!r->profile) return;
  if (r->ev_used + 2 > 4096) { cudaStreamSynchronize(r->stream); prof_collect(r); }
  while (r->ev.size() < r->ev_used + 2) { cudaEvent_t e; cudaEventCreate(&e); r->ev.push_back(e); }
  r->prof_open = r->ev_used; r->ev_used += 2;
  if (r->ev_flops.size() < r->ev_used / 2) r->ev_flops.resize(r->ev_used / 2);
  r->ev_flops[r->prof_open / 2] = flops > 0 ? flops : 0.0;
  cudaEventRecord(r->ev[r->prof_open], r->stream);
}
void nn_prof_end(NnRuntime* r) {
  if (r->prof_open != (size_t)-1) cudaEventRecord(r->ev[r->prof_open + 1], r->stream);
  r->prof_open = (size_t)-1;
}
static int forward_tower(NnRuntime* r, const uint8_t* boards, int n_max, const int* n_dev, float* value) {
  int rc = fw_first(r, boards, n_max, n_dev);
  if (rc) return rc;
  nn_prof_begin(r, 2.0 * 90.0 * 9.0 * r->filters * r->filters * (double)n_max * 2.0 * r->blocks);
  rc = fw_tower(r, n_max, n_dev);
  nn_prof_end(r);
  if (rc) return rc;
  return fw_heads(r, n_max, n_dev, value);
}

static int forward_chunk(NnRuntime* r, const uint8_t* boards, int n, float* policy, float* value) {
  k_set_int<<<1, 1, 0, r->stream>>>(r->n_scalar, n);
  if (r->board_pixels != 90) {
  }
  const int rc = forward_tower(r, boards, n, r->n_scalar, value);
  if (rc) return rc;
  k_softmax<<<n, 256, 0, r->stream>>>(r->logits, kPolN, r->stats, kPolN / 256, policy);
  r->launches += 2;
  CZ_CUDA(cudaGetLastError());
  return 0;
}

int nn_forward_boards(NnRuntime* r, int net, const uint8_t* boards, int batch, float* policy, float* value) {
  if (!r || net < 0 || net >= r->n_nets) return cz_fail(CZ_ERR_STATE, "no such network");
  select_net(r, net);
  if (!r->ready) return cz_fail(CZ_ERR_STATE, "network weights not set (cz_nn_set_weights)");
  for (int off = 0; off < batch; off += r->max_batch) {
    const int n = batch - off < r->max_batch ? batch - off : r->max_batch;
    const int rc = forward_chunk(r, boards + (size_t)off * (r->in_planes / 14) * CZ_BOARD_STRIDE, n, policy + (size_t)off * kLabels, value + off);
    if (rc) return rc;
  }
  return 0;
}

int nn_forward_planes(NnRuntime* r, int net, const float* planes, int batch, float* policy, float* value) {
  if (!r || net < 0 || net >= r->n_nets) return cz_fail(CZ_ERR_STATE, "no such network");
  select_net(r, net);
  if (!r->ready) return cz_fail(CZ_ERR_STATE, "network weights not set (cz_nn_set_weights)");
  for (int off = 0; off < batch; off += r->max_batch) {
    const int n = batch - off < r->max_batch ? batch - off : r->max_batch;
    k_planes_to_boards<<<n, 96, 0, r->stream>>>(planes + (size_t)off * r->in_planes * 90, r->boards_tmp, n, r->in_planes);
    r->launches++;
    const int rc = forward_chunk(r, r->boards_tmp, n, policy + (size_t)off * kLabels, value + off);
    if (rc) return rc;
  }
  return 0;
}

int nn_forward_leaves(NnRuntime* r, int net, int part, const uint8_t* boards, int n_max, const int* n_dev, const int16_t* labels,
                      const int32_t* label_counts, float* legal_p, float* value) {
  if (!r || net < 0 || net >= r->n_nets) return cz_fail(CZ_ERR_STATE, "no such network");
  if (n_max > r->max_batch) return cz_fail(CZ_ERR_ARG, "nn_forward_leaves: %d leaves > max batch %d", n_max, r->max_batch);
  if (r->board_pixels != 90) return cz_fail(CZ_ERR_UNSUPPORTED, "nn_forward_leaves needs the dense (im2col) layout");
  select_net(r, net);
  if (!r->ready) return cz_fail(CZ_ERR_STATE, "network weights not set (cz_nn_set_weights)");
  int rc = 0;
  if (part & 1) rc = fw_first(r, boards, n_max, n_dev);
  if (!rc && (part & 2)) rc = fw_tower(r, n_max, n_dev);
  if (!rc && (part & 4)) rc = fw_heads(r, n_max, n_dev, value);
  if (rc) return rc;
  if (part & 4) k_legal_priors<<<(n_max + 3) / 4, 128, 0, r->stream>>>(r->logits, kPolN, r->stats, kPolN / 256, labels, label_counts, n_dev, legal_p);
  if (part & 4) r->launches++;
  CZ_CUDA(cudaGetLastError());
  return 0;
}
void nn_set_capturing(NnRuntime* r, bool on) { if (r) r->capturing = on; }
bool nn_profiling(const NnRuntime* r) { return r && r->profile; }
void nn_set_stream(NnRuntime* r, void* stream) { if (r) r->stream = (cudaStream_t)stream; }
int nn_launches_per_forward(const NnRuntime* r) { return r ? 1 + 2 * r->blocks + 3 : 0; }
double nn_tower_flops_per_position(const NnRuntime* r) { return r ? 2.0 * 90.0 * 9.0 * r->filters * r->filters * 2.0 * r->blocks : 0.0; }

}

extern "C" {

int cz_igemm_conv3x3(const void* act_in, const void* w, const float* bias, const void* residual, void* act_out,
                     int n_boards, int c, int relu, void* stream) {
  using namespace cznn;
  if (c % 64 || c < 64 || c > 256 || n_boards <= 0) return cz_fail(CZ_ERR_ARG, "cz_igemm_conv3x3: bad shape");
  CUtensorMap ma, mb;
  if (make_map_3d(&ma, act_in, c, 9, (long long)n_boards * 11, 9, 14)) return CZ_ERR_CUDA;
  igemm::Args a = conv_args(n_boards, c, bias, (const __half*)residual, (__half*)act_out, relu);
  if (make_map_2d(&mb, w, c, 9LL * c, c)) return CZ_ERR_CUDA;
  return launch_igemm(c, ma, mb, a, (cudaStream_t)stream);
}

int cz_igemm_conv3x3_dense(const void* act_in, const void* w, const float* bias, const void* residual, void* act_out,
                           int n_boards, int c, int relu, void* stream) {
  using namespace cznn;
  if (c % 64 || c < 64 || c > 256 || n_boards <= 0) return cz_fail(CZ_ERR_ARG, "cz_igemm_conv3x3_dense: bad shape");
  CUtensorMap ma, mb;
  if (make_map_im2col(&ma, act_in, c, n_boards)) return CZ_ERR_CUDA;
  if (make_map_2d(&mb, w, c, 9LL * c, c / 2)) return CZ_ERR_CUDA;
  igemm::Args a = conv_args_dense(n_boards, c, bias, (const __half*)residual, (__half*)act_out, relu);
  if (use_tma_epilogue()) {
    CUtensorMap mo, ms;
    if (make_map_tile32(&mo, act_out, c, (long long)n_boards * 90, false)) return CZ_ERR_CUDA;
    if (make_map_tile32(&ms, residual ? residual : act_out, c, (long long)n_boards * 90, false)) return CZ_ERR_CUDA;
    return launch_igemm3(c, ma, mb, mo, ms, mo, a, residual ? 1 : 0, false, (cudaStream_t)stream);
  }
  return launch_igemm2(c, ma, mb, a, (cudaStream_t)stream);
}

int cz_igemm_dense(const void* a_dev, const void* w_dev, const float* bias, float* out, int m, int n_valid, int n_pad,
                   int k, int n_tile, int ldo, void* stream) {
  using namespace cznn;
  if (k % 64 || n_pad % n_tile || m <= 0) return cz_fail(CZ_ERR_ARG, "cz_igemm_dense: bad shape");
  CUtensorMap ma, mb;
  if (make_map_3d(&ma, a_dev, k, 1, (long long)m, 1, 128)) return CZ_ERR_CUDA;
  if (make_map_2d(&mb, w_dev, k, n_pad, n_tile)) return CZ_ERR_CUDA;
  igemm::Args a = dense_args(m, n_valid, n_pad, k, n_tile, bias, out, ldo);
  return launch_igemm(n_tile, ma, mb, a, (cudaStream_t)stream);
}

}
```

chinesechess-alphazero_b200/csrc/cz_nn.cuh:

```cuda
#pragma once
#include <stdint.h>
#include <stddef.h>
#include "../../include/cczero_b200.h"

namespace cznn {

struct NnRuntime;

size_t nn_workspace_bytes(int filters, int blocks, int value_fc, int max_batch, int n_nets, int pol_c, int val_c);
NnRuntime* nn_create(int device, int filters, int blocks, int value_fc, int max_batch, void* workspace, size_t bytes,
                     void* stream, int fp32_skip_mode, int n_nets, int in_planes , int pol_c, int val_c);
void nn_destroy(NnRuntime*);
int nn_set_weights(NnRuntime*, int net, const cz_tensor_desc* descs, int n);
bool nn_ready(const NnRuntime*);
int nn_forward_boards(NnRuntime*, int net, const uint8_t* boards_dev, int batch, float* policy_dev, float* value_dev);
int nn_forward_planes(NnRuntime*, int net, const float* planes_dev, int batch, float* policy_dev, float* value_dev);
int nn_forward_leaves(NnRuntime*, int net, int part, const uint8_t* boards_dev, int n_max, const int* n_dev, const int16_t* labels_dev,
                      const int32_t* label_counts_dev, float* legal_p_dev, float* value_dev);
void nn_set_capturing(NnRuntime*, bool on);
bool nn_profiling(const NnRuntime*);
void nn_prof_begin(NnRuntime*, double flops);
void nn_prof_end(NnRuntime*);
int nn_launches_per_forward(const NnRuntime*);
double nn_tower_flops_per_position(const NnRuntime*);
void nn_set_stream(NnRuntime*, void* stream);
uint64_t nn_launches(const NnRuntime*);
void nn_profile(NnRuntime*, bool on);
int nn_profile_read(NnRuntime*, double* ms, uint64_t* launches, double* flops);

}
```

chinesechess-alphazero_b200/csrc/cz_tree_api.cu:

```cuda
#include "../../include/cczero_b200.h"
#include "cz_tree.cuh"
#include "cz_selfplay.cuh"
#include "cz_rt.h"
#include "cz_err.h"
#if !defined(CZ_EMUL)
#include "cz_nn.cuh"
#endif
#include <stdlib.h>
#include <new>
#include <vector>

using namespace cz;

namespace {

constexpr int kWarps = 4;

CZ_D TreeSmem* tree_smem() { return reinterpret_cast<TreeSmem*>(czs::dyn_smem()) + czs::warp_in_block(); }
CZ_D int my_game() { return czs::block_idx() * czs::warps_per_block() + czs::warp_in_block(); }

CZ_KERNEL(k_begin)(EngineDev E, int sims_override, int raw_tasks) {
  const int g = my_game();
  if (g >= E.n_games) return;
  game_begin(E, g, sims_override, raw_tasks != 0, tree_smem());
// ... 735 lines not shown
  }
  cudaEventRecord(ready[0], T);
  cudaStreamWaitEvent(N, ready[0], 0);
  const char* msg;
  if (czrt_last_error(&msg)) return cz_fail(CZ_ERR_CUDA, "cz_search: %s", msg);
  return 0;
}
}
#endif

#if !defined(CZ_EMUL)
namespace {
struct Range { int gb, ge; uint8_t* dense; int16_t* labels; int32_t* nlab; float* legal_p; float* value; };
Range range_of(cz_engine* e, int h) {
  const int G = e->cfg.n_games, K = e->cfg.leaves_per_round;
  const int mid = e->n_ranges == 2 ? (G + 1) / 2 : G;
  Range r;
  r.gb = h == 0 ? 0 : mid; r.ge = h == 0 ? mid : G;
  const size_t off = (size_t)r.gb * K;
  r.dense = e->d.leaf_dense + off * e->d.lb_stride;
  r.labels = e->d.leaf_labels + off * MAX_MOVES; r.nlab = e->d.leaf_nlab + off;
  r.legal_p = e->legal_p + off * MAX_MOVES; r.value = e->value_buf + off;
  return r;
}
int enqueue_part(cz_engine* e, int h, int part) {
  const Range r = range_of(e, h);
  const int n_max = (r.ge - r.gb) * e->cfg.leaves_per_round;
  const int* n_dev = e->d.totals + 4 * h;
  if (part == 1) {
    RANGE_LAUNCH(e, e->stream, r.gb, r.ge, k_apply_wave, e->d, r.gb, r.ge, (const float*)r.legal_p, (const float*)r.value);
    k_scan_block<<<1, 1024, 0, e->stream>>>(e->d, r.gb, r.ge, h);
    RANGE_LAUNCH(e, e->stream, r.gb, r.ge, k_gather, e->d, r.gb, r.ge, r.dense, r.labels, r.nlab);
  }
  const int rc = cznn::nn_forward_leaves(e->nn, e->cfg.arena ? h : 0, part, r.dense, n_max, n_dev, r.labels, r.nlab, r.legal_p, r.value);
  if (rc) return rc;
  if (part == 4 && h == e->n_ranges - 1)
    CZ_LAUNCH(k_loop_flag, 1, 1, 0, e->stream, e->d, e->n_ranges, (volatile int32_t*)e->d_flags, e->while_handle, e->capture_cond);
  return 0;
}
int build_while_graph(cz_engine* e) {
  cudaGraph_t g = nullptr;
  if (cudaGraphCreate(&g, 0) != cudaSuccess) return cz_fail(CZ_ERR_CUDA, "cudaGraphCreate failed");
  cudaGraphConditionalHandle handle;
  if (cudaGraphConditionalHandleCreate(&handle, g, 1, cudaGraphCondAssignDefault) != cudaSuccess) {
    cudaGraphDestroy(g);
    return cz_fail(CZ_ERR_CUDA, "cudaGraphConditionalHandleCreate failed: %s", cudaGetErrorString(cudaGetLastError()));
  }
  cudaGraphNodeParams np = {cudaGraphNodeTypeConditional};
  np.conditional.handle = handle;
  np.conditional.type = cudaGraphCondTypeWhile;
  np.conditional.size = 1;
  cudaGraphNode_t node;
  if (cudaGraphAddNode(&node, g, nullptr, 0, &np) != cudaSuccess) {
    cudaGraphDestroy(g);
    return cz_fail(CZ_ERR_CUDA, "cudaGraphAddNode(conditional) failed: %s", cudaGetErrorString(cudaGetLastError()));
  }
  cudaGraph_t body = np.conditional.phGraph_out[0];
  e->while_handle = (unsigned long long)handle;
  e->capture_cond = 1;
  cznn::nn_set_capturing(e->nn, true);
  int rc = 0;
  if (cudaStreamBeginCaptureToGraph(e->stream, body, nullptr, nullptr, 0, cudaStreamCaptureModeThreadLocal) != cudaSuccess) {
    rc = cz_fail(CZ_ERR_CUDA, "cudaStreamBeginCaptureToGraph failed: %s", cudaGetErrorString(cudaGetLastError()));
  } else {
    for (int h = 0; h < e->n_ranges && !rc; ++h)
      for (int part = 1; part <= 4 && !rc; part <<= 1) rc = enqueue_part(e, h, part);
    cudaGraph_t out = nullptr;
    const cudaError_t err = cudaStreamEndCapture(e->stream, &out);
    if (!rc && err != cudaSuccess) rc = cz_fail(CZ_ERR_CUDA, "capture of the loop body failed: %s", cudaGetErrorString(err));
  }
  cznn::nn_set_capturing(e->nn, false);
  e->capture_cond = 0;
  if (!rc && cudaGraphInstantiate(&e->g_while, g, 0) != cudaSuccess)
    rc = cz_fail(CZ_ERR_CUDA, "instantiate of the WHILE graph failed: %s", cudaGetErrorString(cudaGetLastError()));
  cudaGraphDestroy(g);
  return rc;
}
int capture_part(cz_engine* e, int h, int part, cudaGraphExec_t* out) {
  cznn::nn_set_capturing(e->nn, true);
  if (cudaStreamBeginCapture(e->stream, cudaStreamCaptureModeThreadLocal) != cudaSuccess) {
    cznn::nn_set_capturing(e->nn, false);
    return cz_fail(CZ_ERR_CUDA, "cudaStreamBeginCapture failed: %s", cudaGetErrorString(cudaGetLastError()));
  }
  const int rc = enqueue_part(e, h, part);
  cudaGraph_t g = nullptr;
  cudaError_t err = cudaStreamEndCapture(e->stream, &g);
  cznn::nn_set_capturing(e->nn, false);
  if (rc) { if (g) cudaGraphDestroy(g); return rc; }
  if (err != cudaSuccess || !g) return cz_fail(CZ_ERR_CUDA, "graph capture (range %d part %d) failed: %s", h, part, cudaGetErrorString(err));
  err = cudaGraphInstantiate(out, g, 0);
  cudaGraphDestroy(g);
  if (err != cudaSuccess) return cz_fail(CZ_ERR_CUDA, "graph instantiate (range %d part %d) failed: %s", h, part, cudaGetErrorString(err));
  return 0;
}
int build_graphs(cz_engine* e) {
  for (int h = 0; h < e->n_ranges; ++h) {
    int rc;
    if ((rc = capture_part(e, h, 1, &e->g_pre[h])) || (rc = capture_part(e, h, 2, &e->g_tower[h])) || (rc = capture_part(e, h, 4, &e->g_post[h])))
      return rc;
  }
  e->graphs_built = true;
  return 0;
}
int launches_per_iteration(cz_engine* e) { return 3 + cznn::nn_launches_per_forward(e->nn); }

int search_graph_loop(cz_engine* e) {
  CZ_LAUNCH(k_loop_reset, 1, 1, 0, e->stream, e->d);
  e->h_flags[0] = 0; e->h_flags[1] = 1;
  const bool prof = cznn::nn_profiling(e->nn);
  if (e->graphs_built && e->g_while && !prof) {
    if (cudaGraphLaunch(e->g_while, e->stream) != cudaSuccess)
      return cz_fail(CZ_ERR_CUDA, "cz_search: WHILE graph launch failed: %s", cudaGetErrorString(cudaGetLastError()));
    if (cudaStreamSynchronize(e->stream) != cudaSuccess) return cz_fail(CZ_ERR_CUDA, "cz_search: device failure in the loop graph");
    e->launches += (uint64_t)e->h_flags[0] * ((uint64_t)e->n_ranges * launches_per_iteration(e) + 1);
    const char* m;
    if (czrt_last_error(&m)) return cz_fail(CZ_ERR_CUDA, "cz_search: %s", m);
    return 0;
  }
  const int kDepth = e->cfg.n_games * e->cfg.leaves_per_round >= 1024 ? 4 : 2;
  int launched = 0;
  for (;;) {
    for (int h = 0; h < e->n_ranges; ++h) {
      if (!e->graphs_built) {
        int rc;
        if ((rc = enqueue_part(e, h, 1))) return rc;
        if (prof) cznn::nn_prof_begin(e->nn, -1.0);
        rc = enqueue_part(e, h, 2);
        if (prof) cznn::nn_prof_end(e->nn);
        if (rc || (rc = enqueue_part(e, h, 4))) return rc;
      } else {
        if (cudaGraphLaunch(e->g_pre[h], e->stream) != cudaSuccess) return cz_fail(CZ_ERR_CUDA, "cz_search: graph launch failed: %s", cudaGetErrorString(cudaGetLastError()));
        if (prof) cznn::nn_prof_begin(e->nn, -1.0);
        cudaGraphLaunch(e->g_tower[h], e->stream);
        if (prof) cznn::nn_prof_end(e->nn);
        cudaGraphLaunch(e->g_post[h], e->stream);
      }
    }
    if (!e->graphs_built) {
      int rc = build_graphs(e);
      if (!rc && e->loop_mode == 2) rc = build_while_graph(e);
      if (rc) return rc;
    }
    ++launched;
    e->launches += (uint64_t)e->n_ranges * launches_per_iteration(e) + 1;

    int done;
    unsigned spins = 0;
    while (launched - (done = e->h_flags[0]) >= kDepth) {
      if (++spins >= 1000000u) {
        spins = 0;
        const cudaError_t q = cudaStreamQuery(e->stream);
        if (q != cudaSuccess && q != cudaErrorNotReady) return cz_fail(CZ_ERR_CUDA, "cz_search: %s", cudaGetErrorString(q));
        if (q == cudaSuccess && e->h_flags[0] == done) return cz_fail(CZ_ERR_CUDA, "cz_search: the loop flag of iteration %d never arrived", done + 1);
      }
    }
    if (done > 0 && e->h_flags[1] == 0) break;
  }
  if (cudaStreamSynchronize(e->stream) != cudaSuccess) return cz_fail(CZ_ERR_CUDA, "cz_search: device failure");
  const char* msg;
  if (czrt_last_error(&msg)) return cz_fail(CZ_ERR_CUDA, "cz_search: %s", msg);
  return 0;
}
}
#endif

int cz_search(cz_engine* e, const cz_root_opts* opts) {
#if defined(CZ_EMUL)
  (void)e; (void)opts;
  return cz_fail(CZ_ERR_UNSUPPORTED, "cz_search: the CPU emulation build has no network; use the wave/apply API");
#else
  if (!e) return cz_fail(CZ_ERR_ARG, "cz_search: null engine");
  if (!e->nn || !cznn::nn_ready(e->nn)) return cz_fail(CZ_ERR_STATE, "cz_search: network weights not set");
  int rc = cz_search_begin(e, opts);
  if (rc) return rc;
  if (e->graph_loop) return search_graph_loop(e);
  const char* force = getenv("CZ_FORCE_PIPELINE");
  if (e->tree_stream && ((long long)e->cfg.n_games * e->cfg.leaves_per_round >= 8192 || e->cfg.arena || (force && force[0] == '1')))
    return search_pipelined(e);
  if (e->cfg.arena) return cz_fail(CZ_ERR_STATE, "cz_search: arena mode needs the two-range pipeline (CZ_NO_PIPELINE is set)");
  for (;;) {
    int32_t n = 0, busy = 0;
    if ((rc = cz_search_wave(e, &n, &busy))) return rc;
    if (n > 0) {
      if ((rc = cznn::nn_forward_boards(e->nn, 0, e->d.leaf_dense, n, e->policy_buf, e->value_buf))) return rc;
      if ((rc = cz_search_apply(e, e->policy_buf, e->value_buf))) return rc;
    }
    if (!busy) break;
  }
  return 0;
#endif
}

int cz_search_run(cz_engine* e) {
#if defined(CZ_EMUL)
  (void)e;
  return cz_fail(CZ_ERR_UNSUPPORTED, "cz_search_run: the CPU emulation build has no network; use the wave/apply API");
#else
  if (!e) return cz_fail(CZ_ERR_ARG, "cz_search_run: null engine");
  if (!e->nn || !cznn::nn_ready(e->nn)) return cz_fail(CZ_ERR_STATE, "cz_search_run: network weights not set");
  if (e->last_leaves != 0) return cz_fail(CZ_ERR_STATE, "cz_search_run: %d leaves of a host-driven wave were not applied", e->last_leaves);
  if (e->graph_loop) return search_graph_loop(e);
  if (e->cfg.arena) return cz_fail(CZ_ERR_UNSUPPORTED, "cz_search_run: the host-driven loop (CZ_SEARCH_LOOP=host) serves arena engines through cz_search only");
  for (;;) {
    int32_t n = 0, busy = 0;
    int rc;
    if ((rc = cz_search_wave(e, &n, &busy))) return rc;
    if (n > 0) {
      if ((rc = cznn::nn_forward_boards(e->nn, 0, e->d.leaf_dense, n, e->policy_buf, e->value_buf))) return rc;
      if ((rc = cz_search_apply(e, e->policy_buf, e->value_buf))) return rc;
    }
    if (!busy) break;
  }
  return 0;
#endif
}

int cz_get_root(cz_engine* e, int game, cz_root_info* out) {
  if (!e || !out || game < 0 || game >= e->cfg.n_games) return cz_fail(CZ_ERR_ARG, "cz_get_root: bad argument");
  CZ_LAUNCH(k_root_info, 1, 1, sizeof(TreeSmem), e->stream, e->d, game, e->root_info_dev);
  if (launch_ok(e, "cz_get_root")) return CZ_ERR_CUDA;
  czrt_copy(out, e->root_info_dev, sizeof(cz_root_info), e->stream);
  return czrt_sync(e->stream) ? cz_fail(CZ_ERR_CUDA, "cz_get_root: device failure") : 0;
}

int cz_get_pv(cz_engine* e, int game, int32_t max_len, cz_pv_info* out) {
  if (!e || !out || game < 0 || game >= e->cfg.n_games || max_len < 0 || max_len > CZ_MAX_PV)
    return cz_fail(CZ_ERR_ARG, "cz_get_pv: bad argument");
  CZ_LAUNCH(k_pv, 1, 1, sizeof(TreeSmem), e->stream, e->d, game, max_len, e->pv_dev);
  if (launch_ok(e, "cz_get_pv")) return CZ_ERR_CUDA;
  czrt_copy(out, e->pv_dev, sizeof(cz_pv_info), e->stream);
  return czrt_sync(e->stream) ? cz_fail(CZ_ERR_CUDA, "cz_get_pv: device failure") : 0;
}

int cz_get_search_stats(cz_engine* e, uint64_t* out) {
  if (!e || !out) return cz_fail(CZ_ERR_ARG, "cz_get_search_stats: bad argument");
  CZ_LAUNCH(k_stat_reduce, 1, 1, 0, e->stream, e->d, e->stat_out);
  if (launch_ok(e, "cz_get_search_stats")) return CZ_ERR_CUDA;
  unsigned long long h[6];
  czrt_copy(h, e->stat_out, sizeof(h), e->stream);
  if (czrt_sync(e->stream)) return cz_fail(CZ_ERR_CUDA, "cz_get_search_stats: device failure");
  for (int k = 0; k < 6; ++k) out[k] = h[k];
  return 0;
}

int cz_get_counters(cz_engine* e, uint64_t* out) {
  if (!e || !out) return cz_fail(CZ_ERR_ARG, "cz_get_counters: bad argument");
  unsigned long long dc[8];
  CZ_LAUNCH(k_err_reduce, 1, 1, 0, e->stream, e->d);
  czrt_copy(dc, e->d.counters, sizeof(dc), e->stream);
  if (czrt_sync(e->stream)) return cz_fail(CZ_ERR_CUDA, "cz_get_counters: device failure");
  out[0] = e->total_sims; out[1] = dc[1]; out[2] = dc[2]; out[3] = dc[3]; out[4] = dc[4];
  out[5] = dc[5]; out[6] = dc[6]; out[7] = dc[7];
  return 0;
}

int cz_launch_count(cz_engine* e, uint64_t* n) {
  if (!e || !n) return cz_fail(CZ_ERR_ARG, "cz_launch_count: bad argument");
  uint64_t v = e->launches;
#if !defined(CZ_EMUL)
  v += cznn::nn_launches(e->nn);
#endif
  *n = v;
  return 0;
}

int cz_nn_set_weights_net(cz_engine* e, int32_t net, const cz_tensor_desc* descs, int32_t n) {
#if defined(CZ_EMUL)
  (void)e; (void)net; (void)descs; (void)n;
  return cz_fail(CZ_ERR_UNSUPPORTED, "cz_nn_set_weights: no tensor cores in the CPU emulation build");
#else
  if (!e || !descs) return cz_fail(CZ_ERR_ARG, "cz_nn_set_weights: bad argument");
  return cznn::nn_set_weights(e->nn, net, descs, n);
#endif
}

int cz_nn_set_weights(cz_engine* e, const cz_tensor_desc* descs, int32_t n) { return cz_nn_set_weights_net(e, 0, descs, n); }

int cz_nn_forward(cz_engine* e, const float* planes_dev, int32_t batch, float* policy_dev, float* value_dev) {
#if defined(CZ_EMUL)
  (void)e; (void)planes_dev; (void)batch; (void)policy_dev; (void)value_dev;
  return cz_fail(CZ_ERR_UNSUPPORTED, "cz_nn_forward: no tensor cores in the CPU emulation build");
#else
  if (!e || !planes_dev || !policy_dev || !value_dev || batch < 0) return cz_fail(CZ_ERR_ARG, "cz_nn_forward: bad argument");
  return cznn::nn_forward_planes(e->nn, 0, planes_dev, batch, policy_dev, value_dev);
#endif
}

int cz_nn_forward_boards(cz_engine* e, const uint8_t* boards_dev, int32_t batch, float* policy_dev, float* value_dev) {
#if defined(CZ_EMUL)
  (void)e; (void)boards_dev; (void)batch; (void)policy_dev; (void)value_dev;
  return cz_fail(CZ_ERR_UNSUPPORTED, "cz_nn_forward_boards: no tensor cores in the CPU emulation build");
#else
  if (!e || !boards_dev || !policy_dev || !value_dev || batch < 0) return cz_fail(CZ_ERR_ARG, "cz_nn_forward_boards: bad argument");
  return cznn::nn_forward_boards(e->nn, 0, boards_dev, batch, policy_dev, value_dev);
#endif
}

int cz_noise_sample(cz_engine* e, int game, int n_moves, int count, double* out_dev) {
  if (!e || !out_dev || count < 0 || n_moves < 1 || game < 0 || game >= e->cfg.n_games) return cz_fail(CZ_ERR_ARG, "cz_noise_sample: bad argument");
  CZ_LAUNCH(k_noise_sample, 64, 1, 0, e->stream, e->d, game, n_moves, count, out_dev);
  return launch_ok(e, "cz_noise_sample");
}

int cz_nn_profile(cz_engine* e, int enable, double* ms, uint64_t* launches, double* flops) {
#if defined(CZ_EMUL)
  (void)e; (void)enable; (void)ms; (void)launches; (void)flops;
  return cz_fail(CZ_ERR_UNSUPPORTED, "cz_nn_profile: no network in the CPU emulation build");
#else
  if (!e || !e->nn) return cz_fail(CZ_ERR_STATE, "cz_nn_profile: engine has no network");
  cznn::nn_profile(e->nn, enable != 0);
  double fl = 0.0;
  const int rc = cznn::nn_profile_read(e->nn, ms, launches, &fl);
  if (rc) return rc;
  unsigned long long pos = 0;
  czrt_copy(&pos, e->d.counters, sizeof(pos), e->stream);
  if (czrt_sync(e->stream)) return cz_fail(CZ_ERR_CUDA, "cz_nn_profile: device failure");
  fl += (double)(pos - e->prof_pos0) * cznn::nn_tower_flops_per_position(e->nn);
  e->prof_pos0 = pos;
  if (flops) *flops = fl;
  return 0;
#endif
}

}

#include "cz_selfplay_api.inc"
```

chinesechess-alphazero_b200/csrc/cz_umma.cuh:

```cuda
#pragma once
#include <cuda.h>
#include <cuda_runtime.h>
#include <stdint.h>

namespace umma {

__device__ __forceinline__ uint32_t smem_u32(const void* p) { return (uint32_t)__cvta_generic_to_shared(p); }

__device__ __forceinline__ void mbar_init(uint64_t* bar, uint32_t count) {
  asm volatile("mbarrier.init.shared::cta.b64 [%0], %1;" ::"r"(smem_u32(bar)), "r"(count) : "memory");
}
__device__ __forceinline__ void fence_barrier_init() {
  asm volatile("fence.mbarrier_init.release.cluster;" ::: "memory");
}
__device__ __forceinline__ void fence_proxy_async() { asm volatile("fence.proxy.async.shared::cta;" ::: "memory"); }
__device__ __forceinline__ void mbar_expect_tx(uint64_t* bar, uint32_t bytes) {
  asm volatile("mbarrier.arrive.expect_tx.shared::cta.b64 _, [%0], %1;" ::"r"(smem_u32(bar)), "r"(bytes) : "memory");
}
__device__ __forceinline__ void mbar_arrive(uint64_t* bar) {
  asm volatile("mbarrier.arrive.shared::cta.b64 _, [%0];" ::"r"(smem_u32(bar)) : "memory");
}
__device__ __forceinline__ void mbar_wait(uint64_t* bar, uint32_t parity) {
  const uint32_t addr = smem_u32(bar);
  uint32_t ok;
  do {
    asm volatile(
        "{\n\t.reg .pred p;\n\t"
        "mbarrier.try_wait.parity.shared::cta.b64 p, [%1], %2;\n\t"
        "selp.u32 %0, 1, 0, p;\n\t}"
        : "=r"(ok)
        : "r"(addr), "r"(parity)
        : "memory");
  } while (!ok);
}

__device__ __forceinline__ void prefetch_tmap(const CUtensorMap* t) {
  asm volatile("prefetch.tensormap [%0];" ::"l"(reinterpret_cast<uint64_t>(t)) : "memory");
}
__device__ __forceinline__ void tma_load_2d(void* dst, const CUtensorMap* t, uint64_t* bar, int c0, int c1) {
  asm volatile(
      "cp.async.bulk.tensor.2d.shared::cluster.global.mbarrier::complete_tx::bytes [%0], [%1, {%3, %4}], [%2];"
      ::"r"(smem_u32(dst)), "l"(reinterpret_cast<uint64_t>(t)), "r"(smem_u32(bar)), "r"(c0), "r"(c1)
      : "memory");
}
__device__ __forceinline__ void tma_load_3d(void* dst, const CUtensorMap* t, uint64_t* bar, int c0, int c1, int c2) {
  asm volatile(
      "cp.async.bulk.tensor.3d.shared::cluster.global.mbarrier::complete_tx::bytes [%0], [%1, {%3, %4, %5}], [%2];"
      ::"r"(smem_u32(dst)), "l"(reinterpret_cast<uint64_t>(t)), "r"(smem_u32(bar)), "r"(c0), "r"(c1), "r"(c2)
      : "memory");
}

__device__ __forceinline__ void tc_fence_before() { asm volatile("tcgen05.fence::before_thread_sync;" ::: "memory"); }
__device__ __forceinline__ void tc_fence_after() { asm volatile("tcgen05.fence::after_thread_sync;" ::: "memory"); }

template <int kCols>
__device__ __forceinline__ void tmem_alloc(uint32_t* slot_in_smem) {
  asm volatile("tcgen05.alloc.cta_group::1.sync.aligned.shared::cta.b32 [%0], %1;" ::"r"(smem_u32(slot_in_smem)), "n"(kCols)
               : "memory");
  asm volatile("tcgen05.relinquish_alloc_permit.cta_group::1.sync.aligned;" ::: "memory");
}
template <int kCols>
__device__ __forceinline__ void tmem_dealloc(uint32_t taddr) {
  asm volatile("tcgen05.dealloc.cta_group::1.sync.aligned.b32 %0, %1;" ::"r"(taddr), "n"(kCols) : "memory");
}

__device__ __forceinline__ uint64_t smem_desc_sw128(uint32_t saddr) {
  uint64_t d = 0;
  d |= (uint64_t)((saddr >> 4) & 0x3FFF);
  d |= (uint64_t)1 << 16;
  d |= (uint64_t)(1024 >> 4) << 32;
  d |= (uint64_t)1 << 46;
  d |= (uint64_t)2 << 61;
  return d;
}

__host__ __device__ constexpr uint32_t idesc_f16(int m, int n) {
  return (1u << 4) | (0u << 7) | (0u << 10) | ((uint32_t)(n >> 3) << 17) | ((uint32_t)(m >> 4) << 24);
}

__device__ __forceinline__ void mma_f16_ss(uint32_t tmem_d, uint64_t desc_a, uint64_t desc_b, uint32_t idesc, uint32_t accumulate) {
  asm volatile(
      "{\n\t.reg .pred p;\n\t"
      "setp.ne.b32 p, %4, 0;\n\t"
      "tcgen05.mma.cta_group::1.kind::f16 [%0], %1, %2, %3, p;\n\t}"
      ::"r"(tmem_d), "l"(desc_a), "l"(desc_b), "r"(idesc), "r"(accumulate)
      : "memory");
}
__device__ __forceinline__ void mma_commit(uint64_t* bar) {
  asm volatile("tcgen05.commit.cta_group::1.mbarrier::arrive::one.shared::cluster.b64 [%0];" ::"r"(smem_u32(bar)) : "memory");
}

__device__ __forceinline__ void tmem_ld_32x32(uint32_t taddr, uint32_t (&v)[32]) {
  asm volatile(
      "tcgen05.ld.sync.aligned.32x32b.x32.b32 "
      "{%0, %1, %2, %3, %4, %5, %6, %7, %8, %9, %10, %11, %12, %13, %14, %15, "
      "%16, %17, %18, %19, %20, %21, %22, %23, %24, %25, %26, %27, %28, %29, %30, %31}, [%32];"
      : "=r"(v[0]), "=r"(v[1]), "=r"(v[2]), "=r"(v[3]), "=r"(v[4]), "=r"(v[5]), "=r"(v[6]), "=r"(v[7]),
        "=r"(v[8]), "=r"(v[9]), "=r"(v[10]), "=r"(v[11]), "=r"(v[12]), "=r"(v[13]), "=r"(v[14]), "=r"(v[15]),
        "=r"(v[16]), "=r"(v[17]), "=r"(v[18]), "=r"(v[19]), "=r"(v[20]), "=r"(v[21]), "=r"(v[22]), "=r"(v[23]),
        "=r"(v[24]), "=r"(v[25]), "=r"(v[26]), "=r"(v[27]), "=r"(v[28]), "=r"(v[29]), "=r"(v[30]), "=r"(v[31])
      : "r"(taddr)
      : "memory");
  asm volatile("tcgen05.wait::ld.sync.aligned;" ::: "memory");
}

__device__ __forceinline__ uint32_t cluster_ctarank() {
  uint32_t r;
  asm volatile("mov.u32 %0, %%cluster_ctarank;" : "=r"(r));
  return r;
}
__device__ __forceinline__ void griddep_launch_dependents() { asm volatile("griddepcontrol.launch_dependents;" ::: "memory"); }
__device__ __forceinline__ void griddep_wait() { asm volatile("griddepcontrol.wait;" ::: "memory"); }
__device__ __forceinline__ void cluster_sync_all() {
  asm volatile("barrier.cluster.arrive.release.aligned;" ::: "memory");
  asm volatile("barrier.cluster.wait.acquire.aligned;" ::: "memory");
}
__device__ __forceinline__ uint32_t mapa_shared(const void* p, uint32_t rank) {
  uint32_t r;
  asm volatile("mapa.shared::cluster.u32 %0, %1, %2;" : "=r"(r) : "r"(smem_u32(p)), "r"(rank));
  return r;
}
__device__ __forceinline__ void l2_prefetch_bulk(const void* gptr, uint32_t bytes) {
  asm volatile("cp.async.bulk.prefetch.L2.global [%0], %1;" ::"l"(gptr), "r"(bytes) : "memory");
}

__device__ __forceinline__ void mbar_arrive_cluster(uint32_t cluster_addr) {
  asm volatile("mbarrier.arrive.relaxed.cluster.shared::cluster.b64 _, [%0];" ::"r"(cluster_addr) : "memory");
}
__device__ __forceinline__ void mbar_wait_cluster(uint64_t* bar, uint32_t parity) {
  const uint32_t addr = smem_u32(bar);
  uint32_t ok;
  do {
    asm volatile(
        "{\n\t.reg .pred p;\n\t"
        "mbarrier.try_wait.parity.acquire.cluster.shared::cta.b64 p, [%1], %2;\n\t"
        "selp.u32 %0, 1, 0, p;\n\t}"
        : "=r"(ok)
        : "r"(addr), "r"(parity)
        : "memory");
  } while (!ok);
}
__device__ __forceinline__ void tma2_load_2d(void* dst, const CUtensorMap* t, uint64_t* bar, int c0, int c1) {
  asm volatile(
      "cp.async.bulk.tensor.2d.cta_group::2.shared::cluster.global.mbarrier::complete_tx::bytes [%0], [%1, {%3, %4}], [%2];"
      ::"r"(smem_u32(dst)), "l"(reinterpret_cast<uint64_t>(t)), "r"(mapa_shared(bar, 0)), "r"(c0), "r"(c1)
      : "memory");
}
__device__ __forceinline__ void tma2_load_3d(void* dst, const CUtensorMap* t, uint64_t* bar, int c0, int c1, int c2) {
  asm volatile(
      "cp.async.bulk.tensor.3d.cta_group::2.shared::cluster.global.mbarrier::complete_tx::bytes [%0], [%1, {%3, %4, %5}], [%2];"
      ::"r"(smem_u32(dst)), "l"(reinterpret_cast<uint64_t>(t)), "r"(mapa_shared(bar, 0)), "r"(c0), "r"(c1), "r"(c2)
      : "memory");
}
__device__ __forceinline__ void tma2_load_im2col_4d(void* dst, const CUtensorMap* t, uint64_t* bar, int c, int w, int h, int n,
                                                    uint16_t ow, uint16_t oh) {
  asm volatile(
      "cp.async.bulk.tensor.4d.im2col.cta_group::2.shared::cluster.global.mbarrier::complete_tx::bytes [%0], [%1, {%3, %4, %5, %6}], [%2], {%7, %8};"
      ::"r"(smem_u32(dst)), "l"(reinterpret_cast<uint64_t>(t)), "r"(mapa_shared(bar, 0)), "r"(c), "r"(w), "r"(h), "r"(n), "h"(ow), "h"(oh)
      : "memory");
}
__device__ __forceinline__ void tma2_load_2d_r(void* dst, const CUtensorMap* t, uint64_t* bar, int c0, int c1, uint32_t lr) {
  asm volatile(
      "cp.async.bulk.tensor.2d.cta_group::2.shared::cluster.global.mbarrier::complete_tx::bytes [%0], [%1, {%3, %4}], [%2];"
      ::"r"(smem_u32(dst)), "l"(reinterpret_cast<uint64_t>(t)), "r"(mapa_shared(bar, lr)), "r"(c0), "r"(c1)
      : "memory");
}
__device__ __forceinline__ void tma2_load_im2col_4d_r(void* dst, const CUtensorMap* t, uint64_t* bar, int c, int w, int h, int n,
                                                      uint16_t ow, uint16_t oh, uint32_t lr) {
  asm volatile(
      "cp.async.bulk.tensor.4d.im2col.cta_group::2.shared::cluster.global.mbarrier::complete_tx::bytes [%0], [%1, {%3, %4, %5, %6}], [%2], {%7, %8};"
      ::"r"(smem_u32(dst)), "l"(reinterpret_cast<uint64_t>(t)), "r"(mapa_shared(bar, lr)), "r"(c), "r"(w), "r"(h), "r"(n), "h"(ow), "h"(oh)
      : "memory");
}
__device__ __forceinline__ void tma2_load_2d_mc(void* dst, const CUtensorMap* t, uint64_t* bar, int c0, int c1, uint16_t cta_mask) {
  asm volatile(
      "cp.async.bulk.tensor.2d.cta_group::2.shared::cluster.global.mbarrier::complete_tx::bytes.multicast::cluster [%0], [%1, {%4, %5}], [%2], %3;"
      ::"r"(smem_u32(dst)), "l"(reinterpret_cast<uint64_t>(t)), "r"(smem_u32(bar) & 0xFEFFFFFFu), "h"(cta_mask), "r"(c0), "r"(c1)
      : "memory");
}
template <int kCols>
__device__ __forceinline__ void tmem_alloc2(uint32_t* slot_in_smem) {
  asm volatile("tcgen05.alloc.cta_group::2.sync.aligned.shared::cta.b32 [%0], %1;" ::"r"(smem_u32(slot_in_smem)), "n"(kCols)
               : "memory");
  asm volatile("tcgen05.relinquish_alloc_permit.cta_group::2.sync.aligned;" ::: "memory");
}
template <int kCols>
__device__ __forceinline__ void tmem_dealloc2(uint32_t taddr) {
  asm volatile("tcgen05.dealloc.cta_group::2.sync.aligned.b32 %0, %1;" ::"r"(taddr), "n"(kCols) : "memory");
}
__device__ __forceinline__ void mma2_f16_ss(uint32_t tmem_d, uint64_t desc_a, uint64_t desc_b, uint32_t idesc, uint32_t accumulate) {
  asm volatile(
      "{\n\t.reg .pred p;\n\t"
      "setp.ne.b32 p, %4, 0;\n\t"
      "tcgen05.mma.cta_group::2.kind::f16 [%0], %1, %2, %3, p;\n\t}"
      ::"r"(tmem_d), "l"(desc_a), "l"(desc_b), "r"(idesc), "r"(accumulate)
      : "memory");
}
__device__ __forceinline__ void mma2_commit_mask(uint64_t* bar, uint16_t mask) {
  asm volatile("tcgen05.commit.cta_group::2.mbarrier::arrive::one.shared::cluster.multicast::cluster.b64 [%0], %1;"
               ::"r"(smem_u32(bar)), "h"(mask) : "memory");
}
__device__ __forceinline__ void mma2_commit_multicast(uint64_t* bar) {
  const uint16_t mask = 3;
  asm volatile("tcgen05.commit.cta_group::2.mbarrier::arrive::one.shared::cluster.multicast::cluster.b64 [%0], %1;"
               ::"r"(smem_u32(bar)), "h"(mask) : "memory");
}

}
```

chinesechess-alphazero_b200/engine.py:

```python
import ctypes as C

import numpy as np
import torch

from .env import move_to_u16, state_to_board, u16_to_move
from .lib import (BOARD_STRIDE, MAX_MOVES, MAX_NO_ACT, N_LABELS, CzConfig, CzPvInfo, CzRecordHdr, CzRootInfo, CzRootOpts,
                  get_lib)


def _ptr(t):
    return C.c_void_p(t.data_ptr()) if t is not None else C.c_void_p(0)


class Engine:
    def __init__(self, lib=None, device=None, n_games=1, sims_per_move=800, leaves_per_round=8, virtual_loss=3,
                 max_nodes_per_game=None, max_edges_per_game=None, max_path=128, noise_mode=1, max_game_length=100,
                 nn_filters=0, nn_blocks=0, nn_value_fc=256, c_puct=1.5, noise_eps=0.15, dirichlet_alpha=0.2,
                 tau_decay_rate=0.9, resign_threshold=-0.98, enable_resign_rate=0.5, min_resign_turn=40, seed=0, rank=0, nn_fp32_skip=None, arena=False,
                 use_history=False, game_quota=0, playouts=None, nn_policy_channels=0, nn_value_channels=0):
        self.lib = lib or get_lib()
        if device is None:
            device = 'cuda' if self.lib.is_cuda else 'cpu'
        self.device = torch.device(device)
        if self.lib.is_cuda and self.device.type != 'cuda':
            raise ValueError("the CUDA library needs a CUDA device")
        if self.device.type == 'cuda' and self.device.index is None:
            self.device = torch.device('cuda', torch.cuda.current_device())
        if max_nodes_per_game is None:
            max_nodes_per_game = max(64, 4 * sims_per_move + 64)
        if max_edges_per_game is None:
            max_edges_per_game = max_nodes_per_game * 48
        cfg = CzConfig()
        cfg.struct_bytes = C.sizeof(CzConfig)
        cfg.device = self.device.index or 0 if self.device.type == 'cuda' else 0
        cfg.n_games, cfg.sims_per_move, cfg.leaves_per_round = n_games, sims_per_move, leaves_per_round
        cfg.virtual_loss, cfg.max_nodes_per_game, cfg.max_edges_per_game = virtual_loss, max_nodes_per_game, max_edges_per_game
        cfg.max_path, cfg.noise_mode, cfg.max_plies = max_path, noise_mode, 2 * max_game_length
        cfg.nn_filters, cfg.nn_blocks, cfg.nn_value_fc = nn_filters, nn_blocks, nn_value_fc
        cfg.c_puct, cfg.noise_eps, cfg.dirichlet_alpha = c_puct, noise_eps, dirichlet_alpha
        cfg.tau_decay_rate, cfg.resign_threshold, cfg.enable_resign_rate = tau_decay_rate, resign_threshold, enable_resign_rate
        cfg.min_resign_turn, cfg.max_game_length = min_resign_turn, max_game_length
        cfg.seed, cfg.rank = seed, rank
        cfg.arena = 1 if arena else 0
        cfg.nn_fp32_skip = 0 if nn_fp32_skip is None else (1 if nn_fp32_skip else 2)
        cfg.use_history = 1 if use_history else 0
        cfg.game_quota = int(game_quota or 0)
        cfg.playouts_lo, cfg.playouts_hi = (playouts or (0, 0))
        cfg.nn_policy_channels, cfg.nn_value_channels = int(nn_policy_channels or 0), int(nn_value_channels or 0)
        self.use_history = bool(use_history)
        self.in_planes = 28 if use_history else 14
        self.cfg = cfg
        nbytes = C.c_uint64(0)
        self.lib.call("cz_workspace_bytes", C.byref(cfg), C.byref(nbytes))
        self.workspace_bytes = nbytes.value
        self.workspace = torch.zeros(nbytes.value, dtype=torch.uint8, device=self.device)
        self._h = C.c_void_p(0)
        self.lib.call("cz_create", C.byref(cfg), _ptr(self.workspace), nbytes, self._stream(), C.byref(self._h))
        self.n_games = n_games
        self.K = leaves_per_round
        self._keep = []

    def _stream(self):
        if self.lib.is_cuda:
            return C.c_void_p(torch.cuda.current_stream(self.device).cuda_stream)
        return C.c_void_p(0)

    def close(self):
        if self._h:
            self.lib.raw("cz_destroy")(self._h)
            self._h = C.c_void_p(0)

    def __del__(self):
        try:
            self.close()
        except Exception:
            pass

    def reset(self, states=None):
        if states is None:
            self.lib.call("cz_reset_games", self._h, C.c_void_p(0))
            return
        assert len(states) == self.n_games
        b = np.ascontiguousarray(np.stack([state_to_board(s) for s in states]))
        self.lib.call("cz_reset_games", self._h, C.c_void_p(b.ctypes.data))

    def set_root(self, game, state):
        b = np.ascontiguousarray(state_to_board(state))
        self.lib.call("cz_set_root", self._h, game, C.c_void_p(b.ctypes.data))

    def make_opts(self, no_act=None, increase_temp=None, active=None, noise=None, sims_override=0, hist=None, raw_tasks=False):
        o = CzRootOpts()
        o.struct_bytes = C.sizeof(CzRootOpts)
        keep = []
        if hist is not None and any(h for h in hist):
            hb = np.zeros((self.n_games, BOARD_STRIDE), dtype=np.uint8)
            given = np.zeros(self.n_games, dtype=np.uint8)
            for g, h in enumerate(hist):
                if h:
                    given[g] = 1
                    if len(h) >= 5:
                        hb[g] = state_to_board(h[-5])
            keep += [hb, given]
            o.root_hist_host = hb.ctypes.data
            o.root_hist_given_host = given.ctypes.data
        if no_act is not None:
            a = np.full((self.n_games, MAX_NO_ACT), 0xFFFF, dtype=np.uint16)
            for g, lst in enumerate(no_act):
                for k, m in enumerate(lst or []):
                    a[g, k] = move_to_u16(m)
            keep.append(a)
            o.no_act_host = a.ctypes.data
        if increase_temp is not None:
            a = np.ascontiguousarray(np.asarray(increase_temp, dtype=np.uint8))
            keep.append(a)
            o.increase_temp_host = a.ctypes.data
        if active is not None:
            a = np.ascontiguousarray(np.asarray(active, dtype=np.uint8))
            keep.append(a)
            o.active_host = a.ctypes.data
        if noise is not None:
            t = torch.as_tensor(np.ascontiguousarray(noise, dtype=np.float64)).to(self.device)
            assert t.dim() == 2 and t.shape[0] == self.n_games
            keep.append(t)
            o.noise_dev = t.data_ptr()
            o.noise_stride = t.shape[1]
        o.sims_override = sims_override
        o.raw_tasks = 1 if raw_tasks else 0
        self._keep = keep
        return o

    def search_begin(self, opts=None):
        self.lib.call("cz_search_begin", self._h, C.byref(opts) if opts is not None else None)

    def search_wave(self):
        n, busy = C.c_int32(0), C.c_int32(0)
        self.lib.call("cz_search_wave", self._h, C.byref(n), C.byref(busy))
        return n.value, bool(busy.value)

    def leaf_planes(self, n):
        planes = torch.empty((n, self.in_planes, 10, 9), dtype=torch.float32, device=self.device)
        self.lib.call("cz_leaf_planes", self._h, _ptr(planes))
        return planes

    def leaf_boards(self, n):
        b = torch.empty((n, self.in_planes // 14 * BOARD_STRIDE), dtype=torch.uint8, device=self.device)
        self.lib.call("cz_leaf_boards", self._h, _ptr(b))
        return b

    def search_apply(self, policy, value):
        assert policy.dtype == torch.float32 and value.dtype == torch.float32
        self._apply_keep = (getattr(self, "_apply_keep", []) + [(policy, value)])[-4:]
        self.lib.call("cz_search_apply", self._h, _ptr(policy), _ptr(value))

    def leaf_labels(self, n):
        lab = torch.full((n, MAX_MOVES), -1, dtype=torch.int16, device=self.device)
        cnt = torch.zeros((n,), dtype=torch.int32, device=self.device)
        self.lib.call("cz_leaf_labels", self._h, _ptr(lab), _ptr(cnt))
        return lab, cnt

    def search_apply_legal(self, legal_p, value):
        assert legal_p.dtype == torch.float32 and value.dtype == torch.float32 and legal_p.shape[1] == MAX_MOVES
        self._apply_keep = (getattr(self, "_apply_keep", []) + [(legal_p, value)])[-4:]
        self.lib.call("cz_search_apply_legal", self._h, _ptr(legal_p), _ptr(value))

    def search_external(self, evaluate_planes, opts=None):
        self.search_begin(opts)
        stats = {"waves": 0, "positions": 0}
        while True:
            n, busy = self.search_wave()
            stats["waves"] += 1
            if n > 0:
                planes = self.leaf_planes(n).cpu().numpy()
                pol, val = evaluate_planes(planes)
                self.search_apply(torch.as_tensor(np.ascontiguousarray(pol, dtype=np.float32)).to(self.device),
                                  torch.as_tensor(np.ascontiguousarray(val, dtype=np.float32)).to(self.device))
                stats["positions"] += n
            if not busy:
                break
        return stats

    def search_more(self, n_sims):
        self.lib.call("cz_search_more", self._h, int(n_sims))

    def set_noise_table(self, noise):
        t = torch.as_tensor(np.ascontiguousarray(noise, dtype=np.float64)).to(self.device)
        assert t.dim() == 2 and t.shape[0] == self.n_games
        self._noise_keep = (getattr(self, "_noise_keep", []) + [t])[-2:]
        self.lib.call("cz_set_noise_table", self._h, _ptr(t), t.shape[1])

    def run_waves(self, evaluate_planes=None, host_loop=False):
        if evaluate_planes is None and self.lib.is_cuda and self.cfg.nn_filters > 0 and not host_loop:
            c0 = int(self.counters()[1])
            self.lib.call("cz_search_run", self._h)
            return int(self.counters()[1]) - c0
        n_pos = 0
        while True:
            n, busy = self.search_wave()
            if n > 0:
                if evaluate_planes is None:
                    pol, val = self.nn_forward_boards(self.leaf_boards(n))
                    self.search_apply(pol, val)
                else:
                    pol, val = evaluate_planes(self.leaf_planes(n).cpu().numpy())
                    self.search_apply(torch.as_tensor(np.ascontiguousarray(pol, dtype=np.float32)).to(self.device),
                                      torch.as_tensor(np.ascontiguousarray(val, dtype=np.float32)).to(self.device))
                n_pos += n
            if not busy:
                return n_pos

    def pv(self, game, max_len=20):
        info = CzPvInfo()
        self.lib.call("cz_get_pv", self._h, game, max_len, C.byref(info))
        return [u16_to_move(info.moves[i]) for i in range(info.n_moves)], (float(info.value) if info.has_value else None)

    def search_stats(self):
        a = np.zeros(6, dtype=np.uint64)
        self.lib.call("cz_get_search_stats", self._h, C.c_void_p(a.ctypes.data))
        sims, depth, imm, created, edges, nodes = (int(x) for x in a)
        return {"sims": sims, "path_edges": depth, "no_network": imm, "nodes_created": created, "edges_stored": edges, "nodes_stored": nodes}

    def search(self, opts=None):
        self.lib.call("cz_search", self._h, C.byref(opts) if opts is not None else None)

    def root(self, game):
        info = CzRootInfo()
        self.lib.call("cz_get_root", self._h, game, C.byref(info))
        L = info.n_moves
        return {
            "moves": [u16_to_move(info.moves[i]) for i in range(L)],
            "n": [info.n[i] for i in range(L)], "w": [info.w[i] for i in range(L)], "p": [info.p[i] for i in range(L)],
            "sum_n": info.sum_n, "noise_used": info.noise_used, "sims_run": info.sims_run,
        }

    def upload_roots(self, boards_pinned):
        self.lib.call("cz_set_roots", self._h, C.c_void_p(boards_pinned.data_ptr()))

    def download_roots(self, stage):
        self.lib.call("cz_get_roots", self._h, C.c_void_p(stage.boards.data_ptr()))
        stage.d2h_bytes_acc += stage.boards.numel()
        return stage.boards

    def download_root_stats(self, stage):
        self.lib.call("cz_get_root_stats", self._h, C.c_void_p(stage.n.data_ptr()), C.c_void_p(stage.moves.data_ptr()),
                      C.c_void_p(stage.counts.data_ptr()), C.c_void_p(stage.sims.data_ptr()))
        return stage.n, stage.moves, stage.counts

    def sims_run(self):
        st = getattr(self, "_sims_stage", None)
        if st is None:
            from .records import RootStage
            st = self._sims_stage = RootStage(self)
        self.download_root_stats(st)
        return st.sims.numpy()

    def compact(self):
        self.lib.call("cz_compact", self._h)

    def counters(self):
        a = np.zeros(8, dtype=np.uint64)
        self.lib.call("cz_get_counters", self._h, C.c_void_p(a.ctypes.data))
        return a

    def launch_count(self):
        n = C.c_uint64(0)
        self.lib.call("cz_launch_count", self._h, C.byref(n))
        return n.value

    def nn_profile(self, enable=True):
        ms, n, fl = C.c_double(0), C.c_uint64(0), C.c_double(0)
        self.lib.call("cz_nn_profile", self._h, int(enable), C.byref(ms), C.byref(n), C.byref(fl))
        return ms.value, n.value, fl.value

    def play_move(self):
        f = C.c_int32(0)
        self.lib.call("cz_play_move", self._h, C.byref(f))
        return f.value

    def selfplay(self, target_games=0, max_moves=0):
        g, s = C.c_int32(0), C.c_int64(0)
        self.lib.call("cz_selfplay", self._h, target_games, max_moves, C.byref(g), C.byref(s))
        return g.value, s.value

    def set_game_sims(self, sims):
        a = np.ascontiguousarray(np.asarray(sims, dtype=np.int32))
        assert a.shape == (self.n_games,)
        self.lib.call("cz_set_game_sims", self._h, C.c_void_p(a.ctypes.data))

    def any_active(self):
        return bool(self.active_flags().any())

    def active_flags(self):
        a = np.zeros(self.n_games, dtype=np.int32)
        self.lib.call("cz_get_active", self._h, C.c_void_p(a.ctypes.data))
        return a

    def drain_records(self, cap=None):
        cap = cap or max(64, 2 * self.n_games)
        row = self.cfg.max_plies + 1
        hdr = (CzRecordHdr * cap)()
        moves = np.zeros((cap, row), dtype=np.uint16)
        n = C.c_int32(0)
        self.lib.call("cz_drain_records", self._h, C.cast(hdr, C.c_void_p), C.c_void_p(moves.ctypes.data), cap, C.byref(n))
        out = []
        for i in range(n.value):
            h = hdr[i]
            out.append({"n_plies": h.n_plies, "value_red": h.value_red, "game_index": h.game_index, "flags": h.flags,
                        "moves": [u16_to_move(v) for v in moves[i, :h.n_plies]]})
        return out

    def set_weights(self, named_tensors, net=0):
        from .lib import CzTensorDesc
        arr = (CzTensorDesc * len(named_tensors))()
        keep = []
        for i, (k, t) in enumerate(named_tensors.items()):
            t = t.detach().to(self.device, torch.float32).contiguous()
            keep.append(t)
            arr[i].name = k.encode()
            arr[i].dev = t.data_ptr()
            arr[i].numel = t.numel()
        self._weights_keep = getattr(self, "_weights_keep", {})
        self._weights_keep[net] = keep
        self.lib.call("cz_nn_set_weights_net", self._h, net, arr, len(named_tensors))

    def nn_forward_planes(self, planes):
        n = planes.shape[0]
        pol = torch.empty((n, N_LABELS), dtype=torch.float32, device=self.device)
        val = torch.empty((n,), dtype=torch.float32, device=self.device)
        self.lib.call("cz_nn_forward", self._h, _ptr(planes), n, _ptr(pol), _ptr(val))
        return pol, val

    def nn_forward_boards(self, boards):
        n = boards.shape[0]
        pol = torch.empty((n, N_LABELS), dtype=torch.float32, device=self.device)
        val = torch.empty((n,), dtype=torch.float32, device=self.device)
        self.lib.call("cz_nn_forward_boards", self._h, _ptr(boards), n, _ptr(pol), _ptr(val))
        return pol, val
```

chinesechess-alphazero_b200/lib.py:

```python
import ctypes as C
import os

HERE = os.path.dirname(os.path.abspath(__file__))
CUDA_LIB_PATH = os.path.join(HERE, "libcczero_b200.so")

BOARD_STRIDE = 96
MAX_MOVES = 128
N_LABELS = 2086
MAX_NO_ACT = 16


class CzError(RuntimeError):
    pass


class CzConfig(C.Structure):
    _fields_ = [
        ("struct_bytes", C.c_int32), ("device", C.c_int32), ("n_games", C.c_int32),
        ("sims_per_move", C.c_int32), ("leaves_per_round", C.c_int32), ("virtual_loss", C.c_int32),
        ("max_nodes_per_game", C.c_int32), ("max_edges_per_game", C.c_int32), ("max_path", C.c_int32),
        ("noise_mode", C.c_int32), ("max_plies", C.c_int32), ("nn_filters", C.c_int32),
        ("nn_blocks", C.c_int32), ("nn_value_fc", C.c_int32),
        ("c_puct", C.c_double), ("noise_eps", C.c_double), ("dirichlet_alpha", C.c_double),
        ("tau_decay_rate", C.c_double), ("resign_threshold", C.c_double), ("enable_resign_rate", C.c_double),
        ("min_resign_turn", C.c_int32), ("max_game_length", C.c_int32),
        ("seed", C.c_uint64), ("rank", C.c_int32), ("arena", C.c_int32), ("nn_fp32_skip", C.c_int32), ("use_history", C.c_int32),
        ("game_quota", C.c_int32), ("playouts_lo", C.c_int32), ("playouts_hi", C.c_int32),
        ("nn_policy_channels", C.c_int32), ("nn_value_channels", C.c_int32), ("reserved0", C.c_int32),
    ]


class CzRootOpts(C.Structure):
    _fields_ = [
        ("struct_bytes", C.c_int32), ("reserved", C.c_int32),
        ("no_act_host", C.c_void_p), ("increase_temp_host", C.c_void_p), ("active_host", C.c_void_p),
        ("noise_dev", C.c_void_p), ("noise_stride", C.c_int64),
        ("sims_override", C.c_int32), ("raw_tasks", C.c_int32),
        ("root_hist_host", C.c_void_p), ("root_hist_given_host", C.c_void_p),
    ]


class CzRootInfo(C.Structure):
    _fields_ = [
        ("n_moves", C.c_int32), ("sum_n", C.c_int32), ("noise_used", C.c_int32), ("sims_run", C.c_int32),
        ("moves", C.c_uint16 * MAX_MOVES), ("n", C.c_int32 * MAX_MOVES),
        ("w", C.c_double * MAX_MOVES), ("p", C.c_float * MAX_MOVES),
    ]


MAX_PV = 32


class CzPvInfo(C.Structure):
    _fields_ = [("n_moves", C.c_int32), ("has_value", C.c_int32), ("value", C.c_float), ("moves", C.c_uint16 * MAX_PV)]


class CzRecordHdr(C.Structure):
    _fields_ = [("n_plies", C.c_int32), ("value_red", C.c_int32), ("game_index", C.c_int32), ("flags", C.c_int32)]


class CzTensorDesc(C.Structure):
    _fields_ = [("name", C.c_char_p), ("dev", C.c_void_p), ("numel", C.c_int64)]


_P = C.c_void_p
_SIGS = {
    "cz_last_error": (C.c_char_p, []),
    "cz_build_is_cuda": (C.c_int, []),
    "cz_action_labels": (C.c_int, [_P, _P]),
    "cz_env_movegen": (C.c_int, [_P, C.c_int, _P, _P, _P]),
    "cz_env_done": (C.c_int, [_P, C.c_int, C.c_int, _P, _P, _P]),
    "cz_env_step": (C.c_int, [_P, _P, C.c_int, _P, _P, _P]),
    "cz_env_encode_planes": (C.c_int, [_P, C.c_int, _P, _P]),
    "cz_env_check_catch": (C.c_int, [_P, _P, C.c_int, _P, _P, _P, _P]),
    "cz_env_keys": (C.c_int, [_P, C.c_int, _P, _P]),
    "cz_workspace_bytes": (C.c_int, [C.POINTER(CzConfig), C.POINTER(C.c_uint64)]),
    "cz_create": (C.c_int, [C.POINTER(CzConfig), _P, C.c_uint64, _P, C.POINTER(_P)]),
    "cz_destroy": (None, [_P]),
    "cz_reset_games": (C.c_int, [_P, _P]),
    "cz_set_root": (C.c_int, [_P, C.c_int, _P]),
    "cz_set_roots": (C.c_int, [_P, _P]),
    "cz_get_roots": (C.c_int, [_P, _P]),
    "cz_get_root_stats": (C.c_int, [_P, _P, _P, _P, _P]),
    "cz_compact": (C.c_int, [_P]),
    "cz_search_begin": (C.c_int, [_P, C.POINTER(CzRootOpts)]),
    "cz_search_more": (C.c_int, [_P, C.c_int32]),
    "cz_set_noise_table": (C.c_int, [_P, _P, C.c_int64]),
    "cz_get_pv": (C.c_int, [_P, C.c_int, C.c_int32, C.POINTER(CzPvInfo)]),
    "cz_search_wave": (C.c_int, [_P, C.POINTER(C.c_int32), C.POINTER(C.c_int32)]),
    "cz_leaf_planes": (C.c_int, [_P, _P]),
    "cz_leaf_boards": (C.c_int, [_P, _P]),
    "cz_search_apply": (C.c_int, [_P, _P, _P]),
    "cz_leaf_labels": (C.c_int, [_P, _P, _P]),
    "cz_search_apply_legal": (C.c_int, [_P, _P, _P]),
    "cz_search": (C.c_int, [_P, C.POINTER(CzRootOpts)]),
    "cz_search_run": (C.c_int, [_P]),
    "cz_get_root": (C.c_int, [_P, C.c_int, C.POINTER(CzRootInfo)]),
    "cz_get_counters": (C.c_int, [_P, _P]),
    "cz_get_search_stats": (C.c_int, [_P, _P]),
    "cz_play_move": (C.c_int, [_P, C.POINTER(C.c_int32)]),
    "cz_selfplay": (C.c_int, [_P, C.c_int32, C.c_int32, C.POINTER(C.c_int32), C.POINTER(C.c_int64)]),
    "cz_set_game_sims": (C.c_int, [_P, _P]),
    "cz_get_active": (C.c_int, [_P, _P]),
    "cz_record_layout": (C.c_int, [_P, _P]),
    "cz_clear_records": (C.c_int, [_P]),
    "cz_drain_records": (C.c_int, [_P, _P, _P, C.c_int32, C.POINTER(C.c_int32)]),
    "cz_record_buffer": (C.c_int, [_P, C.POINTER(_P), C.POINTER(C.c_uint64), C.POINTER(C.c_int32)]),
    "cz_nn_set_weights": (C.c_int, [_P, C.POINTER(CzTensorDesc), C.c_int32]),
    "cz_nn_set_weights_net": (C.c_int, [_P, C.c_int32, C.POINTER(CzTensorDesc), C.c_int32]),
    "cz_nn_forward": (C.c_int, [_P, _P, C.c_int32, _P, _P]),
    "cz_nn_forward_boards": (C.c_int, [_P, _P, C.c_int32, _P, _P]),
    "cz_launch_count": (C.c_int, [_P, C.POINTER(C.c_uint64)]),
    "cz_nn_profile": (C.c_int, [_P, C.c_int, C.POINTER(C.c_double), C.POINTER(C.c_uint64), C.POINTER(C.c_double)]),
    "cz_noise_sample": (C.c_int, [_P, C.c_int, C.c_int, C.c_int, _P]),
    "cz_igemm_conv3x3": (C.c_int, [_P, _P, _P, _P, _P, C.c_int, C.c_int, C.c_int, _P]),
    "cz_igemm_conv3x3_dense": (C.c_int, [_P, _P, _P, _P, _P, C.c_int, C.c_int, C.c_int, _P]),
    "cz_igemm_dense": (C.c_int, [_P, _P, _P, _P, C.c_int, C.c_int, C.c_int, C.c_int, C.c_int, C.c_int, _P]),
}
CUDA_ONLY = {"cz_igemm_conv3x3", "cz_igemm_conv3x3_dense", "cz_igemm_dense"}


class CzLib:

    def __init__(self, path):
        if not os.path.exists(path):
            raise CzError(
                f"native library missing: {path} — build it with "
                "`python chinesechess-alphazero_b200/build.py cuda` (there is no CPU fallback)")
        self.path = path
        self._dll = C.CDLL(path, mode=C.RTLD_LOCAL)
        self.missing = []
        for name, (res, args) in _SIGS.items():
            try:
                fn = getattr(self._dll, name)
            except AttributeError:
                self.missing.append(name)
                continue
            fn.restype = res
            fn.argtypes = args
        self.is_cuda = bool(self._dll.cz_build_is_cuda())

    def raw(self, name):
        return getattr(self._dll, name)

    def call(self, name, *args):
        rc = getattr(self._dll, name)(*args)
        if rc is not None and rc < 0:
            msg = self._dll.cz_last_error()
            raise CzError(f"{name} failed ({rc}): {msg.decode() if msg else ''}")
        return rc


_lib = None


def get_lib():
    global _lib
    if _lib is None:
        if not os.path.exists(CUDA_LIB_PATH):
            try:
                from . import build
                build.build_cuda()
            except Exception as e:
                raise CzError(f"native library missing and could not be built ({e}); run "
                              "`python chinesechess-alphazero_b200/build.py cuda`") from e
        _lib = CzLib(CUDA_LIB_PATH)
        if not _lib.is_cuda:
            raise CzError("libcczero_b200.so is not a CUDA build")
    return _lib
```

include/cczero_b200.h:

```cpp
#ifndef CCZERO_B200_H
#define CCZERO_B200_H
#include <stdint.h>
#ifdef __cplusplus
extern "C" {
#endif

#define CZ_BOARD_STRIDE 96
#define CZ_MAX_MOVES 128
#define CZ_N_LABELS 2086
#define CZ_MAX_NO_ACT 16

typedef enum cz_status {
  CZ_OK = 0,
  CZ_ERR_ARG = -1,
  CZ_ERR_CUDA = -2,
  CZ_ERR_STATE = -3,
  CZ_ERR_CAPACITY = -4,
  CZ_ERR_UNSUPPORTED = -5
} cz_status;

const char* cz_last_error(void);
int cz_build_is_cuda(void);

int cz_action_labels(char* labels_host, int16_t* lut_host);

int cz_env_movegen(const uint8_t* boards_dev, int n, uint16_t* moves_dev, int32_t* counts_dev, void* stream);
int cz_env_done(const uint8_t* boards_dev, int n, int need_check, int8_t* out_dev, uint16_t* final_move_dev,
                void* stream);
int cz_env_step(const uint8_t* boards_dev, const uint16_t* moves_dev, int n, uint8_t* boards_out_dev,
                uint8_t* no_eat_dev, void* stream);
int cz_env_encode_planes(const uint8_t* boards_dev, int n, float* planes_dev, void* stream);
int cz_env_check_catch(const uint8_t* boards_dev, const uint16_t* moves_dev, int n, uint8_t* will_cc_dev,
                       uint8_t* be_catched_dev, uint8_t* has_attack_dev, void* stream);
int cz_env_keys(const uint8_t* boards_dev, int n, uint64_t* keys_dev , void* stream);

typedef struct cz_engine cz_engine;

typedef struct cz_config {
  int32_t struct_bytes;
  int32_t device;
  int32_t n_games;
  int32_t sims_per_move;
  int32_t leaves_per_round;
  int32_t virtual_loss;
  int32_t max_nodes_per_game;
  int32_t max_edges_per_game;
  int32_t max_path;
  int32_t noise_mode;
  int32_t max_plies;
  int32_t nn_filters;
  int32_t nn_blocks;
  int32_t nn_value_fc;
  double c_puct;
  double noise_eps;
  double dirichlet_alpha;
  double tau_decay_rate;
  double resign_threshold;
  double enable_resign_rate;
  int32_t min_resign_turn;
  int32_t max_game_length;
  uint64_t seed;
  int32_t rank;
  int32_t arena;
  int32_t nn_fp32_skip;
  int32_t use_history;
  int32_t game_quota;
  int32_t playouts_lo;
  int32_t playouts_hi;
  int32_t nn_policy_channels;
  int32_t nn_value_channels;
  int32_t reserved0;
} cz_config;

int cz_workspace_bytes(const cz_config* cfg, uint64_t* bytes);
int cz_create(const cz_config* cfg, void* workspace_dev, uint64_t workspace_bytes, void* stream, cz_engine** out);
void cz_destroy(cz_engine* e);

int cz_reset_games(cz_engine* e, const uint8_t* boards_host);
int cz_set_root(cz_engine* e, int game, const uint8_t* board_host);

int cz_set_roots(cz_engine* e, const uint8_t* boards_host);
int cz_get_roots(cz_engine* e, uint8_t* boards_host);

typedef struct cz_root_opts {
  int32_t struct_bytes;
  int32_t reserved;
  const uint16_t* no_act_host;
  const uint8_t* increase_temp_host;
  const uint8_t* active_host;
  const double* noise_dev;
  int64_t noise_stride;
  int32_t sims_override;
  int32_t raw_tasks;
  const uint8_t* root_hist_host;
  const uint8_t* root_hist_given_host;
} cz_root_opts;

int cz_search_begin(cz_engine* e, const cz_root_opts* opts);
int cz_search_wave(cz_engine* e, int32_t* n_leaves, int32_t* any_active);
int cz_leaf_planes(cz_engine* e, float* planes_dev );
int cz_leaf_boards(cz_engine* e, uint8_t* boards_dev );
int cz_search_apply(cz_engine* e, const float* policy_dev , const float* value_dev );
int cz_leaf_labels(cz_engine* e, int16_t* labels_dev, int32_t* counts_dev);
int cz_search_apply_legal(cz_engine* e, const float* legal_p_dev, const float* value_dev);
int cz_search_more(cz_engine* e, int32_t n_sims);
int cz_set_noise_table(cz_engine* e, const double* noise_dev, int64_t noise_stride);
int cz_search(cz_engine* e, const cz_root_opts* opts);
int cz_search_run(cz_engine* e);

typedef struct cz_root_info {
  int32_t n_moves;
  int32_t sum_n;
  int32_t noise_used;
  int32_t sims_run;
  uint16_t moves[CZ_MAX_MOVES];
  int32_t n[CZ_MAX_MOVES];
  double w[CZ_MAX_MOVES];
  float p[CZ_MAX_MOVES];
} cz_root_info;
int cz_get_root(cz_engine* e, int game, cz_root_info* out_host);

#define CZ_MAX_PV 32
typedef struct cz_pv_info {
  int32_t n_moves;
  int32_t has_value;
  float value;
  uint16_t moves[CZ_MAX_PV];
} cz_pv_info;
int cz_get_pv(cz_engine* e, int game, int32_t max_len, cz_pv_info* out_host);

int cz_get_root_stats(cz_engine* e, int32_t* n_host, uint16_t* moves_host, int32_t* counts_host, int32_t* sims_run_host);

int cz_compact(cz_engine* e);

int cz_get_search_stats(cz_engine* e, uint64_t* out );

int cz_get_counters(cz_engine* e, uint64_t* out_host );

int cz_play_move(cz_engine* e, int32_t* n_finished);
int cz_selfplay(cz_engine* e, int32_t target_games, int32_t max_moves, int32_t* games_done, int64_t* sims_done);

typedef struct cz_record_hdr {
  int32_t n_plies;
  int32_t value_red;
  int32_t game_index;
  int32_t flags;
} cz_record_hdr;
int cz_drain_records(cz_engine* e, cz_record_hdr* hdr_host, uint16_t* moves_host, int32_t cap, int32_t* n);
int cz_set_game_sims(cz_engine* e, const int32_t* sims_host);
int cz_get_active(cz_engine* e, int32_t* active_host);
int cz_record_buffer(cz_engine* e, void** dev_ptr, uint64_t* bytes, int32_t* n_ready);
int cz_record_layout(cz_engine* e, int64_t* out );
int cz_clear_records(cz_engine* e);

typedef struct cz_tensor_desc {
  const char* name;
  const void* dev;
  int64_t numel;
} cz_tensor_desc;
int cz_nn_set_weights(cz_engine* e, const cz_tensor_desc* descs, int32_t n);
int cz_nn_set_weights_net(cz_engine* e, int32_t net, const cz_tensor_desc* descs, int32_t n);
int cz_nn_forward(cz_engine* e, const float* planes_dev, int32_t batch, float* policy_dev, float* value_dev);
int cz_nn_forward_boards(cz_engine* e, const uint8_t* boards_dev, int32_t batch, float* policy_dev, float* value_dev);
int cz_nn_profile(cz_engine* e, int enable, double* ms, uint64_t* launches, double* flops);
int cz_launch_count(cz_engine* e, uint64_t* n);

int cz_igemm_conv3x3(const void* act_in_dev, const void* w_dev, const float* bias_dev, const void* residual_dev,
                     void* act_out_dev, int n_boards, int c, int relu, void* stream);
int cz_igemm_conv3x3_dense(const void* act_in_dev, const void* w_dev, const float* bias_dev, const void* residual_dev,
                           void* act_out_dev, int n_boards, int c, int relu, void* stream);
int cz_noise_sample(cz_engine* e, int game, int n_moves, int count, double* out_dev);
int cz_igemm_dense(const void* a_dev, const void* w_dev, const float* bias_dev, float* out_dev, int m, int n_valid,
                   int n_pad, int k, int n_tile, int ldo, void* stream);

#ifdef __cplusplus
}
#endif
#endif
```

Before: 270,700.

## Add dynamic cluster work scheduler for 4-CTA igemm3 and PDL for igemm2

Replaces the compile-time PAIRS template with a runtime cluster-size variant (k_igemm3_mc). In that variant one CTA pulls work items from a global atomic counter and broadcasts them to all CTAs in the cluster through a shared-memory ring guarded by mbarriers, so producer, MMA and epilogue warps consume a dynamic schedule. It also adds programmatic dependent launch to igemm2 so its prologue can overlap the tail of the previous kernel. The 4-CTA path stays gated by CZ_CLUSTER4, which is off by default, and adds per-launch global atomics plus diagnostic counters.

```diff
diff --git a/chinesechess-alphazero_b200/csrc/cz_igemm.cuh b/chinesechess-alphazero_b200/csrc/cz_igemm.cuh
--- a/chinesechess-alphazero_b200/csrc/cz_igemm.cuh
+++ b/chinesechess-alphazero_b200/csrc/cz_igemm.cuh
@@ -287,11 +287,13 @@
     umma::fence_proxy_async();
   }
   if (warp == 2) umma::tmem_alloc2<C::kTmemCols>(tmem_slot);
+  umma::griddep_launch_dependents();
   umma::tc_fence_before();
   __syncthreads();
   umma::cluster_sync_all();
   umma::tc_fence_after();
   const uint32_t tmem_base = *tmem_slot;
+  umma::griddep_wait();
 
   const int n_kb = a.n_taps * a.k_chunks;
   const int rows = args_rows(a);
diff --git a/chinesechess-alphazero_b200/csrc/cz_igemm3.cuh b/chinesechess-alphazero_b200/csrc/cz_igemm3.cuh
--- a/chinesechess-alphazero_b200/csrc/cz_igemm3.cuh
+++ b/chinesechess-alphazero_b200/csrc/cz_igemm3.cuh
@@ -19,6 +19,8 @@
   int nf;
   int split_producer;
   int n_split;
+  int* work;
+  unsigned long long* diag;
 };
 __host__ __device__ constexpr int epi3_warp_bytes(int fbytes, int nf) { return nf * fbytes + kNH3 * kHBytes3; }
 
@@ -58,10 +60,11 @@
 template <int N>
 __device__ __forceinline__ void bulk_wait_all() { asm volatile("cp.async.bulk.wait_group %0;" ::"n"(N) : "memory"); }
 
-template <int N_TILE, int MT = 1, int PAIRS = 1>
-__global__ void __cluster_dims__(2 * PAIRS, 1, 1) __launch_bounds__(kThreads2, 1)
-k_igemm3(const __grid_constant__ CUtensorMap tmA, const __grid_constant__ CUtensorMap tmB, const __grid_constant__ CUtensorMap tmOut16,
-         const __grid_constant__ CUtensorMap tmSkip, const __grid_constant__ CUtensorMap tmOut32, const Args3 p) {
+constexpr int kRing3 = 3;
+
+template <int N_TILE, int MT, bool kDyn>
+__device__ __forceinline__ void igemm3_body(const CUtensorMap& tmA, const CUtensorMap& tmB, const CUtensorMap& tmOut16,
+                                            const CUtensorMap& tmSkip, const CUtensorMap& tmOut32, const Args3& p) {
   using C = Cfg3<N_TILE, MT>;
   const Args& a = p.a;
   const int n_stages = p.stages;
@@ -75,14 +78,22 @@
   uint64_t* tfull = bars + 2 * kMaxStages3;
   uint64_t* tempty = tfull + 2;
   uint64_t* skipbar = tempty + 2;
-  uint32_t* tmem_slot = reinterpret_cast<uint32_t*>(skipbar + kMaxNF3 * kEpiWarps2);
+  uint64_t* rfull = skipbar + kMaxNF3 * kEpiWarps2;
+  uint64_t* rempty = rfull + kRing3;
+  uint32_t* tmem_slot = reinterpret_cast<uint32_t*>(rempty + kRing3);
+  int* ritem = reinterpret_cast<int*>(tmem_slot + 1);
+  static_assert((2 * kMaxStages3 + 4 + kMaxNF3 * kEpiWarps2 + 2 * kRing3) * 8 + 4 + 4 * kRing3 <= 512, "barrier block");
 
   const int warp = threadIdx.x >> 5, lane = threadIdx.x & 31;
   const uint32_t crank = umma::cluster_ctarank();
+  const uint32_t ncta = kDyn ? umma::cluster_nctarank() : 2u;
+  const uint32_t npairs = ncta >> 1;
   const uint32_t rank = crank & 1u;
   const uint32_t pp = crank >> 1;
   const uint32_t lrank = crank & ~1u;
   const bool leader = rank == 0;
+  constexpr bool dyn = kDyn;
+  const uint32_t n_readers = ncta * (8u + (p.split_producer ? 2u : 1u)) + npairs;
 
   if (warp == 0 && lane == 0) {
     umma::prefetch_tmap(&tmA);
@@ -92,9 +103,11 @@
     if (p.out32) umma::prefetch_tmap(&tmOut32);
   }
   if (warp == 1 && lane == 0) {
-    for (int s = 0; s < n_stages; ++s) { umma::mbar_init(&full[s], 1); umma::mbar_init(&empty[s], PAIRS); }
+    for (int s = 0; s < n_stages; ++s) { umma::mbar_init(&full[s], 1); umma::mbar_init(&empty[s], npairs); }
     for (int i = 0; i < 2; ++i) { umma::mbar_init(&tfull[i], 1); umma::mbar_init(&tempty[i], 512); }
     for (int i = 0; i < kMaxNF3 * kEpiWarps2; ++i) umma::mbar_init(&skipbar[i], 1);
+    if (dyn)
+      for (int i = 0; i < kRing3; ++i) { umma::mbar_init(&rfull[i], 1); umma::mbar_init(&rempty[i], n_readers); }
     umma::fence_barrier_init();
     umma::fence_proxy_async();
   }
@@ -113,15 +126,45 @@
   const int pairs = (m_tiles + 2 * MT - 1) / (2 * MT);
   const int ns = p.n_split > 1 ? p.n_split : 1;
   const int items = pairs * ns;
-  const int items_c = (items + PAIRS - 1) / PAIRS;
-  const int n_clusters = gridDim.x / (2 * PAIRS), cluster_id = blockIdx.x / (2 * PAIRS);
-
-  if (warp == 0 || (warp == 3 && p.split_producer)) {
+  const int n_clusters = gridDim.x / 2, cluster_id = blockIdx.x / 2;
+
+  auto next_step = [&](uint32_t& pos) -> int {
+    if (!dyn) return cluster_id + (int)(pos++) * n_clusters;
+    const uint32_t s = pos % kRing3, ph = (pos / kRing3) & 1;
+    ++pos;
+    umma::mbar_wait_cluster(&rfull[s], ph);
+    return *reinterpret_cast<volatile int*>(&ritem[s]);
+  };
+  auto give_back = [&](uint32_t pos) {
+    if (dyn) umma::mbar_arrive_release_cluster(umma::mapa_shared(&rempty[(pos - 1) % kRing3], 0));
+  };
+  auto take = [&](uint32_t& pos) -> int { const int v = next_step(pos); give_back(pos); return v; };
+
+  if (dyn && crank == 0 && warp == 2 && lane == 0) {
+    unsigned long long handed = 0;
+    for (uint32_t pos = 0;; ++pos) {
+      const uint32_t s = pos % kRing3, ph = (pos / kRing3) & 1;
+      umma::mbar_wait_cluster(&rempty[s], ph ^ 1);
+      const int step = atomicAdd(&p.work[0], (int)npairs);
+      for (uint32_t r = 0; r < ncta; ++r) {
+        umma::st_cluster_u32(umma::mapa_shared(&ritem[s], r), (uint32_t)step);
+        umma::mbar_arrive_release_cluster(umma::mapa_shared(&rfull[s], r));
+      }
+      if (step >= items) break;
+      handed += (unsigned long long)(items - step < (int)npairs ? items - step : (int)npairs);
+    }
+    atomicAdd(&p.diag[ncta == 4 ? 0 : 1], 1ull);
+    atomicAdd(&p.diag[2], handed);
+    if (atomicAdd(&p.work[1], (int)ncta) + (int)ncta == (int)gridDim.x) {
+      atomicExch(&p.work[0], 0);
+      atomicExch(&p.work[1], 0);
+    }
+  } else if (warp == 0 || (warp == 3 && p.split_producer)) {
     if (lane == 0) {
       const bool do_a = warp == 0, do_b = warp == 3 || !p.split_producer;
-      uint32_t s = 0, ph = 0;
-      for (int it = cluster_id; it < items_c; it += n_clusters) {
-        const int item = it * PAIRS + (int)pp;
+      uint32_t s = 0, ph = 0, rpos = 0;
+      for (int step = take(rpos); step < items; step = take(rpos)) {
+        const int item = step + (int)pp;
         const int pair = item / ns, n0 = (item % ns) * N_TILE;
         const int m_tile = MT * (2 * pair + (int)rank);
         for (int tap = 0; tap < a.n_taps; ++tap) {
@@ -139,7 +182,7 @@
               }
             }
             if (do_b) {
-              if (PAIRS == 1) umma::tma2_load_2d(sB, &tmB, &full[s], kc * kBlockK, tap * a.n_total + n0 + (int)rank * (N_TILE / 2));
+              if (npairs == 1) umma::tma2_load_2d(sB, &tmB, &full[s], kc * kBlockK, tap * a.n_total + n0 + (int)rank * (N_TILE / 2));
               else if (pp == 0)
                 umma::tma2_load_2d_mc(sB, &tmB, &full[s], kc * kBlockK, tap * a.n_total + n0 + (int)rank * (N_TILE / 2),
                                       (uint16_t)((1u << rank) | (1u << (rank + 2))));
@@ -152,8 +195,9 @@
   } else if (warp == 1) {
     if (leader && lane == 0) {
       constexpr uint32_t idesc = umma::idesc_f16(256, N_TILE);
-      uint32_t s = 0, ph = 0, tcount = 0;
-      for (int it = cluster_id; it < items_c; it += n_clusters, ++tcount) {
+      const uint16_t stage_mask = ncta == 4 ? (uint16_t)0xF : (uint16_t)3;
+      uint32_t s = 0, ph = 0, tcount = 0, rpos = 0;
+      for (int step = take(rpos); step < items; step = take(rpos), ++tcount) {
         const uint32_t acc = tcount & 1, aph = (tcount >> 1) & 1;
         umma::mbar_wait(&tempty[acc], aph ^ 1);
         umma::tc_fence_after();
@@ -170,7 +214,7 @@
             for (int k = 0; k < kBlockK / 16; ++k)
               umma::mma2_f16_ss(d_tmem + mt * N_TILE, da + (uint64_t)(k * 2), db + (uint64_t)(k * 2), idesc, (kb | k) != 0);
           }
-          umma::mma2_commit_mask(&empty[s], PAIRS == 1 ? (uint16_t)3 : (uint16_t)0xF);
+          umma::mma2_commit_mask(&empty[s], stage_mask);
           if (++s == (uint32_t)n_stages) { s = 0; ph ^= 1; }
         }
         umma::mma2_commit_mask(&tfull[acc], (uint16_t)(3u << (2 * pp)));
@@ -203,27 +247,35 @@
       for (size_t off = (size_t)lane * 16384; off < total; off += 32 * 16384)
         umma::l2_prefetch_bulk(base + off, (uint32_t)(total - off < 16384 ? total - off : 16384));
     };
-    int my_tiles = 0;
-    for (int it = cluster_id; it < items_c; it += n_clusters) ++my_tiles;
-    const uint32_t total_chunks = (uint32_t)my_tiles * (MT * kChunks);
-    auto request_skip = [&](uint32_t g) {
-      if (!has_skip || g >= total_chunks) return;
-      const int t = (int)(g / (MT * kChunks)), rem = (int)(g % (MT * kChunks)), mt = rem / kChunks, ch = rem % kChunks;
-      const int item = (cluster_id + t * n_clusters) * PAIRS + (int)pp;
+    constexpr int kT = MT * kChunks;
+    auto request_skip = [&](int step, int k, uint32_t g) {
+      if (!has_skip || step >= items) return;
+      const int item = step + (int)pp, mt = k / kChunks, ch = k % kChunks;
       const int row = (MT * (2 * (item / ns) + (int)rank) + mt) * kTileM + q * 32;
       const uint32_t slot = g % (uint32_t)nf;
       umma::mbar_expect_tx(&sbar[slot], skip_bytes);
       umma::tma_load_2d(F + slot * fb, &tmSkip, &sbar[slot], (item % ns) * N_TILE + cbeg + ch * kChunkCols3, row);
     };
+    uint32_t rpos = 0;
+    auto take_warp = [&]() -> int {
+      const int v = next_step(rpos);
+      if (dyn) {
+        __syncwarp();
+        if (lane == 0) give_back(rpos);
+      }
+      return v;
+    };
+    int cur = take_warp();
+    int nxt = cur < items ? take_warp() : cur;
     uint32_t tcount = 0, g = 0;
-    prefetch_skip(cluster_id * PAIRS + (int)pp);
+    prefetch_skip(cur + (int)pp);
     if (lane == 0)
-      for (int k = 0; k < nf - 2; ++k) request_skip((uint32_t)k);
-    for (int it = cluster_id; it < items_c; it += n_clusters, ++tcount) {
+      for (int k = 0; k < nf - 2; ++k) request_skip(cur, k, (uint32_t)k);
+    for (; cur < items; ++tcount) {
       const uint32_t acc = tcount & 1, aph = (tcount >> 1) & 1;
-      const int item = it * PAIRS + (int)pp;
+      const int item = cur + (int)pp;
       const int pair = item / ns, n0 = (item % ns) * N_TILE;
-      prefetch_skip(item + n_clusters * PAIRS);
+      prefetch_skip(nxt + (int)pp);
       umma::mbar_wait(&tfull[acc], aph);
       umma::tc_fence_after();
 #pragma unroll 1
@@ -237,7 +289,9 @@
         const int c0 = n0 + cbeg + ch * kChunkCols3;
         if (lane == 0) {
           bulk_wait_read<1>();
-          request_skip(g + (uint32_t)nf - 2);
+          const int k2 = mt * kChunks + ch + nf - 2;
+          if (k2 < kT) request_skip(cur, k2, g + (uint32_t)nf - 2);
+          else request_skip(nxt, k2 - kT, g + (uint32_t)nf - 2);
         }
         uint32_t v[16];
         tmem_ld_32x16(t_row + ch * kChunkCols3, v);
@@ -293,6 +347,8 @@
       }
       umma::tc_fence_before();
       umma::mbar_arrive_cluster(tempty_remote[acc]);
+      cur = nxt;
+      if (cur < items) nxt = take_warp();
     }
     if (lane == 0) bulk_wait_all<0>();
   }
@@ -306,4 +362,17 @@
   }
 }
 
-}
+template <int N_TILE, int MT = 1>
+__global__ void __cluster_dims__(2, 1, 1) __launch_bounds__(kThreads2, 1)
+k_igemm3(const __grid_constant__ CUtensorMap tmA, const __grid_constant__ CUtensorMap tmB, const __grid_constant__ CUtensorMap tmOut16,
+         const __grid_constant__ CUtensorMap tmSkip, const __grid_constant__ CUtensorMap tmOut32, const Args3 p) {
+  igemm3_body<N_TILE, MT, false>(tmA, tmB, tmOut16, tmSkip, tmOut32, p);
+}
+template <int N_TILE>
+__global__ void __launch_bounds__(kThreads2, 1)
+k_igemm3_mc(const __grid_constant__ CUtensorMap tmA, const __grid_constant__ CUtensorMap tmB, const __grid_constant__ CUtensorMap tmOut16,
+            const __grid_constant__ CUtensorMap tmSkip, const __grid_constant__ CUtensorMap tmOut32, const Args3 p) {
+  igemm3_body<N_TILE, 1, true>(tmA, tmB, tmOut16, tmSkip, tmOut32, p);
+}
+
+}
diff --git a/chinesechess-alphazero_b200/csrc/cz_nn.cu b/chinesechess-alphazero_b200/csrc/cz_nn.cu
--- a/chinesechess-alphazero_b200/csrc/cz_nn.cu
+++ b/chinesechess-alphazero_b200/csrc/cz_nn.cu
@@ -127,6 +127,18 @@
   return 0;
 }
 
+static bool use_pdl() {
+  static int pdl = -1;
+  if (pdl < 0) { const char* e = getenv("CZ_PDL"); pdl = (e && e[0] == '0') ? 0 : 1; }
+  return pdl == 1;
+}
+static cudaLaunchAttribute pdl_attr() {
+  cudaLaunchAttribute at;
+  at.id = cudaLaunchAttributeProgrammaticStreamSerialization;
+  at.val.programmaticStreamSerializationAllowed = 1;
+  return at;
+}
+
 template <int N_TILE>
 static int launch_igemm2_t(const CUtensorMap& tmA, const CUtensorMap& tmB_half, const igemm::Args& a, cudaStream_t st) {
   using C = igemm::Cfg2<N_TILE>;
@@ -138,7 +150,16 @@
   const int pairs = (a.m_tiles + 1) / 2;
   if (pairs <= 0) return 0;
   const int clusters = pairs < num_sms() / 2 ? pairs : num_sms() / 2;
-  igemm::k_igemm2<N_TILE><<<2 * clusters, igemm::kThreads2, C::kSmemBytes, st>>>(tmA, tmB_half, a);
+  if (use_pdl()) {
+    cudaLaunchConfig_t lc;
+    memset(&lc, 0, sizeof(lc));
+    lc.gridDim = dim3(2 * clusters); lc.blockDim = dim3(igemm::kThreads2); lc.dynamicSmemBytes = C::kSmemBytes; lc.stream = st;
+    cudaLaunchAttribute at = pdl_attr();
+    lc.attrs = &at; lc.numAttrs = 1;
+    CZ_CUDA(cudaLaunchKernelEx(&lc, igemm::k_igemm2<N_TILE>, tmA, tmB_half, a));
+  } else {
+    igemm::k_igemm2<N_TILE><<<2 * clusters, igemm::kThreads2, C::kSmemBytes, st>>>(tmA, tmB_half, a);
+  }
   CZ_CUDA(cudaGetLastError());
   return 0;
 }
@@ -157,36 +178,44 @@
   return v;
 }
 static bool use_tma_epilogue() { return epilogue_choice() != 2; }
+static int g_cluster4 = 0;
 static bool use_tma_epilogue_for(int c, bool fp32_stream) {
   if (epilogue_choice() == 2) return false;
   if (epilogue_choice() == 3) return true;
   return !(c == 256 && fp32_stream);
 }
-static int g_cluster4 = 0;
-template <int N_TILE, int MT, int PAIRS = 1>
+static int cluster4_resident() {
+  static int n = -1;
+  if (n < 0) {
+    n = 0;
+    if (cudaFuncSetAttribute(igemm::k_igemm3_mc<256>, cudaFuncAttributeMaxDynamicSharedMemorySize, igemm::kSmemLimit3) == cudaSuccess) {
+      cudaLaunchConfig_t oc;
+      memset(&oc, 0, sizeof(oc));
+      oc.gridDim = dim3(num_sms() / 4 * 4); oc.blockDim = dim3(igemm::kThreads2); oc.dynamicSmemBytes = igemm::kSmemLimit3;
+      cudaLaunchAttribute at[1];
+      at[0].id = cudaLaunchAttributeClusterDimension;
+      at[0].val.clusterDim.x = 4; at[0].val.clusterDim.y = 1; at[0].val.clusterDim.z = 1;
+      oc.attrs = at; oc.numAttrs = 1;
+      if (cudaOccupancyMaxActiveClusters(&n, igemm::k_igemm3_mc<256>, &oc) != cudaSuccess) n = 0;
+    }
+    (void)cudaGetLastError();
+  }
+  return n;
+}
+template <int N_TILE, int MT>
 static int launch_igemm3_t(const CUtensorMap& tmA, const CUtensorMap& tmB_half, const CUtensorMap& tmOut16, const CUtensorMap& tmSkip,
-                           const CUtensorMap& tmOut32, const igemm::Args& a, int skip_mode, bool out32, cudaStream_t st, int n_split = 1) {
+                           const CUtensorMap& tmOut32, const igemm::Args& a, int skip_mode, bool out32, cudaStream_t st, int n_split = 1,
+                           int* sched = nullptr, unsigned long long* diag = nullptr) {
   using C = igemm::Cfg3<N_TILE, MT>;
   static bool attr_set = false;
-  static int max_clusters = 0;
   if (!attr_set) {
-    CZ_CUDA(cudaFuncSetAttribute(igemm::k_igemm3<N_TILE, MT, PAIRS>, cudaFuncAttributeMaxDynamicSharedMemorySize, igemm::kSmemLimit3));
+    CZ_CUDA(cudaFuncSetAttribute(igemm::k_igemm3<N_TILE, MT>, cudaFuncAttributeMaxDynamicSharedMemorySize, igemm::kSmemLimit3));
     attr_set = true;
-    max_clusters = num_sms() / (2 * PAIRS);
-    if (PAIRS > 1) {
-      cudaLaunchConfig_t oc;
-      memset(&oc, 0, sizeof(oc));
-      oc.gridDim = dim3(2 * PAIRS * max_clusters); oc.blockDim = dim3(igemm::kThreads2); oc.dynamicSmemBytes = igemm::kSmemLimit3;
-      int nc = 0;
-      if (cudaOccupancyMaxActiveClusters(&nc, igemm::k_igemm3<N_TILE, MT, PAIRS>, &oc) == cudaSuccess && nc > 0 && nc < max_clusters) max_clusters = nc;
-      else (void)cudaGetLastError();
-      fprintf(stderr, "[cczero] 4-CTA clusters of k_igemm3<%d, %d>: %d resident at once (%d of %d SMs)\n", N_TILE, MT, max_clusters,
-              4 * max_clusters, num_sms());
-    }
   }
   igemm::Args3 p;
   p.a = a;
   p.skip_mode = skip_mode; p.out32 = out32 ? 1 : 0; p.n_split = n_split;
+  p.work = sched; p.diag = diag;
   p.fbytes = (skip_mode == 2 || out32) ? 2048 : (skip_mode == 1 ? 1024 : 0);
   { static int nf = -1; if (nf < 0) { const char* e = getenv("CZ_NF"); nf = e ? atoi(e) : 3; if (nf < 3) nf = 3; if (nf > igemm::kMaxNF3) nf = igemm::kMaxNF3; } p.nf = nf; }
   { static int sp = -1; if (sp < 0) { const char* e = getenv("CZ_SPLIT_PROD"); sp = (e && e[0] == '1') ? 1 : 0; } p.split_producer = sp; }
@@ -195,28 +224,48 @@
   if (p.stages < 2) return cz_fail(CZ_ERR_UNSUPPORTED, "igemm3: no room for the operand ring");
   const int pairs = ((a.n_dev ? (a.rows + igemm::kTileM - 1) / igemm::kTileM : a.m_tiles) + 2 * MT - 1) / (2 * MT);
   if (pairs <= 0) return 0;
-  const int items = (pairs * (n_split > 1 ? n_split : 1) + PAIRS - 1) / PAIRS;
-  const int clusters = items < max_clusters ? items : max_clusters;
-  static int pdl = -1;
-  if (pdl < 0) { const char* e = getenv("CZ_PDL"); pdl = (e && e[0] == '0') ? 0 : 1; }
+  const int items = pairs * (n_split > 1 ? n_split : 1);
+  const bool pdl = use_pdl();
+  const size_t smem = C::smem_bytes(p.stages, p.fbytes, p.nf);
+  cudaLaunchConfig_t lc;
+  memset(&lc, 0, sizeof(lc));
+  lc.blockDim = dim3(igemm::kThreads2); lc.dynamicSmemBytes = smem; lc.stream = st;
+  cudaLaunchAttribute at[3];
+  int n_at = 0;
+  if (pdl) at[n_at++] = pdl_attr();
+  if constexpr (N_TILE == 256 && MT == 1) {
+    if (sched) {
+      static bool mc_attr = false;
+      if (!mc_attr) {
+        CZ_CUDA(cudaFuncSetAttribute(igemm::k_igemm3_mc<256>, cudaFuncAttributeMaxDynamicSharedMemorySize, igemm::kSmemLimit3));
+        mc_attr = true;
+      }
+      const int full = num_sms() / 4 * 4, want = (2 * items + 3) / 4 * 4;
+      lc.gridDim = dim3(want < full ? want : full);
+      at[n_at].id = cudaLaunchAttributeClusterDimension;
+      at[n_at].val.clusterDim.x = 2; at[n_at].val.clusterDim.y = 1; at[n_at].val.clusterDim.z = 1; ++n_at;
+      at[n_at].id = cudaLaunchAttributePreferredClusterDimension;
+      at[n_at].val.preferredClusterDim.x = 4; at[n_at].val.preferredClusterDim.y = 1; at[n_at].val.preferredClusterDim.z = 1; ++n_at;
+      lc.attrs = at; lc.numAttrs = n_at;
+      CZ_CUDA(cudaLaunchKernelEx(&lc, igemm::k_igemm3_mc<256>, tmA, tmB_half, tmOut16, tmSkip, tmOut32, p));
+      CZ_CUDA(cudaGetLastError());
+      return 0;
+    }
+  }
+  const int clusters = items < num_sms() / 2 ? items : num_sms() / 2;
   if (pdl) {
-    cudaLaunchConfig_t lc;
-    memset(&lc, 0, sizeof(lc));
-    lc.gridDim = dim3(2 * PAIRS * clusters); lc.blockDim = dim3(igemm::kThreads2);
-    lc.dynamicSmemBytes = C::smem_bytes(p.stages, p.fbytes, p.nf); lc.stream = st;
-    cudaLaunchAttribute at[1];
-    at[0].id = cudaLaunchAttributeProgrammaticStreamSerialization;
-    at[0].val.programmaticStreamSerializationAllowed = 1;
-    lc.attrs = at; lc.numAttrs = 1;
-    CZ_CUDA(cudaLaunchKernelEx(&lc, igemm::k_igemm3<N_TILE, MT, PAIRS>, tmA, tmB_half, tmOut16, tmSkip, tmOut32, p));
+    lc.gridDim = dim3(2 * clusters);
+    lc.attrs = at; lc.numAttrs = n_at;
+    CZ_CUDA(cudaLaunchKernelEx(&lc, igemm::k_igemm3<N_TILE, MT>, tmA, tmB_half, tmOut16, tmSkip, tmOut32, p));
   } else {
-    igemm::k_igemm3<N_TILE, MT, PAIRS><<<2 * PAIRS * clusters, igemm::kThreads2, C::smem_bytes(p.stages, p.fbytes, p.nf), st>>>(tmA, tmB_half, tmOut16, tmSkip, tmOut32, p);
+    igemm::k_igemm3<N_TILE, MT><<<2 * clusters, igemm::kThreads2, smem, st>>>(tmA, tmB_half, tmOut16, tmSkip, tmOut32, p);
   }
   CZ_CUDA(cudaGetLastError());
   return 0;
 }
 static int launch_igemm3(int n_tile, const CUtensorMap& tmA, const CUtensorMap& tmB_half, const CUtensorMap& tmOut16, const CUtensorMap& tmSkip,
-                         const CUtensorMap& tmOut32, const igemm::Args& a, int skip_mode, bool out32, cudaStream_t st) {
+                         const CUtensorMap& tmOut32, const igemm::Args& a, int skip_mode, bool out32, cudaStream_t st,
+                         int* sched = nullptr, unsigned long long* diag = nullptr) {
   static int mt2 = -1;
   if (mt2 < 0) { const char* e = getenv("CZ_MT"); mt2 = (e && e[0] == '1') ? 0 : 1; }
   switch (n_tile) {
@@ -225,10 +274,9 @@
     case 128: return mt2 ? launch_igemm3_t<128, 2>(tmA, tmB_half, tmOut16, tmSkip, tmOut32, a, skip_mode, out32, st)
                          : launch_igemm3_t<128, 1>(tmA, tmB_half, tmOut16, tmSkip, tmOut32, a, skip_mode, out32, st);
     case 192: return launch_igemm3_t<192, 1>(tmA, tmB_half, tmOut16, tmSkip, tmOut32, a, skip_mode, out32, st);
-    case 256: {
-      if (g_cluster4) return launch_igemm3_t<256, 1, 2>(tmA, tmB_half, tmOut16, tmSkip, tmOut32, a, skip_mode, out32, st);
+    case 256:
+      if (g_cluster4 && sched) return launch_igemm3_t<256, 1>(tmA, tmB_half, tmOut16, tmSkip, tmOut32, a, skip_mode, out32, st, 1, sched, diag);
       return launch_igemm3_t<256, 1>(tmA, tmB_half, tmOut16, tmSkip, tmOut32, a, skip_mode, out32, st);
-    }
   }
   return cz_fail(CZ_ERR_UNSUPPORTED, "igemm3: unsupported N tile %d", n_tile);
 }
@@ -575,6 +623,8 @@
   float* logits;
   float2* stats;
   int* n_scalar;
+  int* sched;
+  unsigned long long* cluster_diag;
   bool heads_attr;
   bool capturing;
   size_t prof_open;
@@ -641,6 +691,8 @@
   r->logits = (float*)cv.take((size_t)r->max_batch * kPolN * sizeof(float));
   r->stats = (float2*)cv.take((size_t)r->max_batch * (kPolN / 256) * sizeof(float2));
   r->n_scalar = (int*)cv.take(64);
+  r->sched = (int*)cv.take((size_t)2 * r->blocks * 2 * sizeof(int));
+  r->cluster_diag = (unsigned long long*)cv.take(4 * sizeof(unsigned long long));
   r->boards_tmp = (uint8_t*)cv.take((size_t)r->max_batch * 2 * CZ_BOARD_STRIDE);
   for (int net = 0; net < r->n_nets; ++net) {
   r->w_first = (__half*)cv.take((size_t)25 * 28 * c * sizeof(__half));
@@ -695,7 +747,7 @@
   r->in_planes = in_planes == 28 ? 28 : 14;
   r->fp32_skip = fp32_skip_mode == 1 || (fp32_skip_mode == 0 && blocks >= 10);
   { const char* e = getenv("CZ_FP32_SKIP"); if (e && e[0] == '1') r->fp32_skip = true; if (e && e[0] == '0') r->fp32_skip = false; }
-  { const char* e = getenv("CZ_CLUSTER4"); g_cluster4 = (e && e[0] == '1') ? 1 : 0; }
+  { const char* e = getenv("CZ_CLUSTER4"); g_cluster4 = (e && e[0] == '1' && cluster4_resident() > 0) ? 1 : 0; }
   r->profile = false; r->ev_used = 0; r->prof_ms = 0; r->prof_flops = 0; r->prof_launches = 0; r->capturing = false;
   Carver cv{(uint8_t*)workspace, 0, bytes};
   layout(r, cv);
@@ -735,6 +787,8 @@
   cudaMemsetAsync(r->t, 0, (size_t)max_batch * 11 * 9 * c * 2, r->stream);
   cudaMemsetAsync(r->y, 0, (size_t)max_batch * 11 * 9 * c * 2, r->stream);
   cudaMemsetAsync(r->pol_feat, 0, ((size_t)max_batch + 128) * 3 * r->pol_k1 * 2, r->stream);
+  cudaMemsetAsync(r->sched, 0, (size_t)2 * blocks * 2 * sizeof(int), r->stream);
+  cudaMemsetAsync(r->cluster_diag, 0, 4 * sizeof(unsigned long long), r->stream);
   return r;
 }
 
@@ -761,6 +815,14 @@
   return true;
 }
 uint64_t nn_launches(const NnRuntime* r) { return r ? r->launches : 0; }
+int nn_cluster_stats(NnRuntime* r, uint64_t* out) {
+  if (!r) return cz_fail(CZ_ERR_STATE, "no network");
+  unsigned long long v[3];
+  CZ_CUDA(cudaMemcpyAsync(v, r->cluster_diag, sizeof(v), cudaMemcpyDeviceToHost, r->stream));
+  CZ_CUDA(cudaStreamSynchronize(r->stream));
+  for (int k = 0; k < 3; ++k) out[k] = v[k];
+  return 0;
+}
 
 struct WeightSet {
   const cz_tensor_desc* d; int n;
@@ -902,10 +964,10 @@
         if (launch_igemm3_split(c, r->imap_t, r->map_w_32[2 * i + 1], *oy, s32 ? *fx : *ox, *fy, d2, s32 ? 2 : 1, s32, st)) return CZ_ERR_CUDA;
       } else {
       if (epi3 && use_tma_epilogue_for(c, false)) {
-        if (launch_igemm3(c, *ix, r->map_w_half[2 * i], r->omap_t, r->omap_t, r->omap_t, d1, 0, false, st)) return CZ_ERR_CUDA;
+        if (launch_igemm3(c, *ix, r->map_w_half[2 * i], r->omap_t, r->omap_t, r->omap_t, d1, 0, false, st, r->sched + 4 * i, r->cluster_diag)) return CZ_ERR_CUDA;
       } else if (launch_igemm2(c, *ix, r->map_w_half[2 * i], d1, st)) return CZ_ERR_CUDA;
       if (epi3 && use_tma_epilogue_for(c, s32)) {
-        if (launch_igemm3(c, r->imap_t, r->map_w_half[2 * i + 1], *oy, s32 ? *fx : *ox, *fy, d2, s32 ? 2 : 1, s32, st)) return CZ_ERR_CUDA;
+        if (launch_igemm3(c, r->imap_t, r->map_w_half[2 * i + 1], *oy, s32 ? *fx : *ox, *fy, d2, s32 ? 2 : 1, s32, st, r->sched + 4 * i + 2, r->cluster_diag)) return CZ_ERR_CUDA;
       } else if (launch_igemm2(c, r->imap_t, r->map_w_half[2 * i + 1], d2, st)) return CZ_ERR_CUDA;
       }
       CUtensorMap* ti = ix; ix = iy; iy = ti;
diff --git a/chinesechess-alphazero_b200/csrc/cz_nn.cuh b/chinesechess-alphazero_b200/csrc/cz_nn.cuh
--- a/chinesechess-alphazero_b200/csrc/cz_nn.cuh
+++ b/chinesechess-alphazero_b200/csrc/cz_nn.cuh
@@ -27,5 +27,6 @@
 uint64_t nn_launches(const NnRuntime*);
 void nn_profile(NnRuntime*, bool on);
 int nn_profile_read(NnRuntime*, double* ms, uint64_t* launches, double* flops);
+int nn_cluster_stats(NnRuntime*, uint64_t* out);
 
 }
diff --git a/chinesechess-alphazero_b200/csrc/cz_tree_api.cu b/chinesechess-alphazero_b200/csrc/cz_tree_api.cu
--- a/chinesechess-alphazero_b200/csrc/cz_tree_api.cu
+++ b/chinesechess-alphazero_b200/csrc/cz_tree_api.cu
@@ -1061,6 +1061,16 @@
   return launch_ok(e, "cz_noise_sample");
 }
 
+int cz_nn_cluster_stats(cz_engine* e, uint64_t* out) {
+#if defined(CZ_EMUL)
+  (void)e; (void)out;
+  return cz_fail(CZ_ERR_UNSUPPORTED, "cz_nn_cluster_stats: no network in the CPU emulation build");
+#else
+  if (!e || !e->nn || !out) return cz_fail(CZ_ERR_ARG, "cz_nn_cluster_stats: engine has no network or out is NULL");
+  return cznn::nn_cluster_stats(e->nn, out);
+#endif
+}
+
 int cz_nn_profile(cz_engine* e, int enable, double* ms, uint64_t* launches, double* flops) {
 #if defined(CZ_EMUL)
   (void)e; (void)enable; (void)ms; (void)launches; (void)flops;
diff --git a/chinesechess-alphazero_b200/csrc/cz_umma.cuh b/chinesechess-alphazero_b200/csrc/cz_umma.cuh
--- a/chinesechess-alphazero_b200/csrc/cz_umma.cuh
+++ b/chinesechess-alphazero_b200/csrc/cz_umma.cuh
@@ -109,6 +109,17 @@
   asm volatile("mov.u32 %0, %%cluster_ctarank;" : "=r"(r));
   return r;
 }
+__device__ __forceinline__ uint32_t cluster_nctarank() {
+  uint32_t r;
+  asm volatile("mov.u32 %0, %%cluster_nctarank;" : "=r"(r));
+  return r;
+}
+__device__ __forceinline__ void st_cluster_u32(uint32_t cluster_addr, uint32_t v) {
+  asm volatile("st.shared::cluster.u32 [%0], %1;" ::"r"(cluster_addr), "r"(v) : "memory");
+}
+__device__ __forceinline__ void mbar_arrive_release_cluster(uint32_t cluster_addr) {
+  asm volatile("mbarrier.arrive.release.cluster.shared::cluster.b64 _, [%0];" ::"r"(cluster_addr) : "memory");
+}
 __device__ __forceinline__ void griddep_launch_dependents() { asm volatile("griddepcontrol.launch_dependents;" ::: "memory"); }
 __device__ __forceinline__ void griddep_wait() { asm volatile("griddepcontrol.wait;" ::: "memory"); }
 __device__ __forceinline__ void cluster_sync_all() {
diff --git a/chinesechess-alphazero_b200/engine.py b/chinesechess-alphazero_b200/engine.py
--- a/chinesechess-alphazero_b200/engine.py
+++ b/chinesechess-alphazero_b200/engine.py
@@ -271,6 +271,11 @@
         self.lib.call("cz_nn_profile", self._h, int(enable), C.byref(ms), C.byref(n), C.byref(fl))
         return ms.value, n.value, fl.value
 
+    def nn_cluster_stats(self):
+        a = np.zeros(3, dtype=np.uint64)
+        self.lib.call("cz_nn_cluster_stats", self._h, C.c_void_p(a.ctypes.data))
+        return tuple(int(x) for x in a)
+
     def play_move(self):
         f = C.c_int32(0)
         self.lib.call("cz_play_move", self._h, C.byref(f))
diff --git a/chinesechess-alphazero_b200/lib.py b/chinesechess-alphazero_b200/lib.py
--- a/chinesechess-alphazero_b200/lib.py
+++ b/chinesechess-alphazero_b200/lib.py
@@ -112,6 +112,7 @@
     "cz_nn_forward_boards": (C.c_int, [_P, _P, C.c_int32, _P, _P]),
     "cz_launch_count": (C.c_int, [_P, C.POINTER(C.c_uint64)]),
     "cz_nn_profile": (C.c_int, [_P, C.c_int, C.POINTER(C.c_double), C.POINTER(C.c_uint64), C.POINTER(C.c_double)]),
+    "cz_nn_cluster_stats": (C.c_int, [_P, _P]),
     "cz_noise_sample": (C.c_int, [_P, C.c_int, C.c_int, C.c_int, _P]),
     "cz_igemm_conv3x3": (C.c_int, [_P, _P, _P, _P, _P, C.c_int, C.c_int, C.c_int, _P]),
     "cz_igemm_conv3x3_dense": (C.c_int, [_P, _P, _P, _P, _P, C.c_int, C.c_int, C.c_int, _P]),
diff --git a/include/cczero_b200.h b/include/cczero_b200.h
--- a/include/cczero_b200.h
+++ b/include/cczero_b200.h
@@ -163,6 +163,7 @@
 int cz_nn_forward(cz_engine* e, const float* planes_dev, int32_t batch, float* policy_dev, float* value_dev);
 int cz_nn_forward_boards(cz_engine* e, const uint8_t* boards_dev, int32_t batch, float* policy_dev, float* value_dev);
 int cz_nn_profile(cz_engine* e, int enable, double* ms, uint64_t* launches, double* flops);
+int cz_nn_cluster_stats(cz_engine* e, uint64_t* out );
 int cz_launch_count(cz_engine* e, uint64_t* n);
 
 int cz_igemm_conv3x3(const void* act_in_dev, const void* w_dev, const float* bias_dev, const void* residual_dev,
```

Result: no change. 272,600, median of 6 (+0.7%).
